# pauxy-qmc/pauxy

Hardware: AMD Instinct MI355X
Metric: walker_steps_per_sec (higher is better)
Workload: dtype f64; 1 GPU; generic Cholesky AFQMC: Nbasis=100, Nchol=500, RHF trial 25+25 electrons, 256 walkers/GPU, dt=0.005, reortho/10, comb/5, energy/10 (BASELINE configs[2]); walkers_total=256, rng=device-philox, population_control=device comb (one rank)

## Files before the change

include/afqmc_hip.h:

```cpp
#ifndef AFQMC_HIP_H
#define AFQMC_HIP_H

#include <stdint.h>

#ifdef __cplusplus
extern "C" {
#endif

typedef struct afq_handle afq_handle;

#define AFQ_OK            0
#define AFQ_EINVAL       (-1)
#define AFQ_ESTATE       (-2)
#define AFQ_EHIP         (-3)
#define AFQ_ENOMEM       (-4)
#define AFQ_EUNSUPPORTED (-5)
#define AFQ_EWEIGHT      (-6)
#define AFQ_EOVERFLOW    (-7)
#define AFQ_ECOMM        (-8)

#define AFQ_SYS_GENERIC 1
#define AFQ_SYS_HUBBARD 2
#define AFQ_SYS_UEG     3

// ... 66 lines not shown
int afq_local_energy_full_g(afq_handle *h, const double *G, int n, double *E_out);
int afq_ueg_pair_sums(afq_handle *h, const double *G, int n, double *E_out, double *two_rdm_out);
int afq_hubbard_energy_full_g(afq_handle *h, const double *G, int n, double *E_out);
int afq_correlations_full_g(afq_handle *h, const double *G, int n, double *corr_out);
int afq_set_pairing_bonds(afq_handle *h, int nb, const int32_t *nbr);
int afq_pairing_full_g(afq_handle *h, const double *G, int n, double *pair_out);

int afq_bp_configure(afq_handle *h, int nbp);
int afq_bp_steps(afq_handle *h, int32_t *steps_out);
int afq_bp_update(afq_handle *h, const double *phi_bp0, int nstblz, int restore_weights, int eval_energy,
                  int reset, double *est_out);
int afq_bp_observables(afq_handle *h, int two_rdm, int ekt, const double *h1, const double *L, int nL);
int afq_bp_pairing(afq_handle *h, int on);
int afq_bp_ekt_chunks(afq_handle *h, int nc, int ncy);
int afq_bp_update_ext(afq_handle *h, const double *phi_bp0, int nstblz, int restore_weights, int eval_energy,
                      int reset, double *est_out, double *two_rdm_out, double *fock_out);
int afq_bp_update_msd(afq_handle *h, int ndet, const double *dets, const double *coeffs, int nstblz, int restore_weights,
                      int eval_energy, int reset, double *est_out, double *detw_out);

int afq_itcf_configure(afq_handle *h, int nmax, int neqlb, int stable, int restore_weights);
int afq_itcf_update(afq_handle *h, const double *psi_T, int nstblz, double *spgf_out, double *denom_out);

int afq_set_trial_multi(afq_handle *h, int ndet, const double *psi, const double *coeffs, const double *rchol);
int afq_walkers_det_weights(afq_handle *h, double *weights_out);

int afq_set_propagator(afq_handle *h, const double *BH1, const double *mf_shift,
                       double dt, int exp_order, int flags);

int afq_walkers_alloc(afq_handle *h, int nw);
int afq_walkers_set(afq_handle *h, int field, const void *host, int first, int count);
int afq_walkers_get(afq_handle *h, int field, void *host, int first, int count);
int afq_walkers_device_ptr(afq_handle *h, int field, void **dev_ptr, int64_t *bytes_per_walker);

int afq_greens(afq_handle *h, int want_G, double *ovlp_out);
int afq_calc_overlap(afq_handle *h, double *ovlp_out);
int afq_inverse_overlap(afq_handle *h, double *oinv_out, double *ovlp_out);
int afq_propagate(afq_handle *h, const double *xi, double eshift_re, double eshift_im);
int afq_propagate_begin(afq_handle *h, const double *xi);
int afq_propagate_finish(afq_handle *h, double eshift_re, double eshift_im);
int afq_reortho(afq_handle *h, double *detR_out);
int afq_set_log_shift(afq_handle *h, int on, double log_shift, double detR_shift);
int afq_log_ovlp_sums(afq_handle *h, double *sums3);
int afq_local_energy(afq_handle *h, double *E_out);

int afq_set_exchange_algorithm(afq_handle *h, int mode);
int afq_exchange_algorithm(afq_handle *h, int *mode_out);

int afq_set_propagator_closed_form(afq_handle *h, int mode);
int afq_propagator_closed_form(afq_handle *h, int *mode_out);

int afq_set_step_fusion(afq_handle *h, int mode);
int afq_set_step_fusion_scope(afq_handle *h, int scope);
int afq_set_step_tail_overlap(afq_handle *h, int on);

int afq_set_msd_force_bias(afq_handle *h, int mode);
int afq_msd_force_bias(afq_handle *h, int *mode_out);

int afq_force_bias(afq_handle *h, double *xbar_out);
int afq_shift_fields(afq_handle *h, const double *xi, const double *xbar,
                     double *xs_out, double *cmf_out, double *cfb_out);
int afq_vhs(afq_handle *h, const double *xs, double *vhs_out);
int afq_vhs_count(afq_handle *h, int *nv);
int afq_apply_exponential(afq_handle *h, const double *vhs);
int afq_kinetic(afq_handle *h);

int afq_cap_weights(afq_handle *h, double frac, double total_weight);
int afq_set_weight_cap(afq_handle *h, double frac, double total_weight);
int afq_popcontrol_comb(afq_handle *h, double r, double target_weight,
                        int32_t *parent_ix, double *total_weight_out);
#define AFQ_PAIR_BRANCH_MAX_WALKERS 8192
int afq_popcontrol_pair_branch(afq_handle *h, const double *u, int nu, double target_weight,
                               double min_weight, double max_weight, int32_t *mult,
                               int32_t *ndraws_out, double *total_weight_out);

#define AFQ_COMM_ID_BYTES 128
#define AFQ_COMM_NSTATS 12
typedef int (*afq_allgather_fn)(const void *send, void *recv, int bytes, void *user);
int afq_comm_unique_id(void *id_out);
int afq_comm_available(void);
int afq_comm_init(afq_handle *h, const void *unique_id, int rank, int nranks);
int afq_comm_init_ipc(afq_handle *h, int rank, int nranks, afq_allgather_fn allgather, void *user);
int afq_comm_destroy(afq_handle *h);
int afq_comm_set_transport(afq_handle *h, int window);
int afq_comm_set_capacity(afq_handle *h, int max_walkers_per_peer);
int afq_comm_set_timeout(afq_handle *h, double seconds);
int afq_comm_probe(afq_handle *h, int64_t *mismatch_out);
int afq_comm_stats(afq_handle *h, int64_t *out);
int afq_comm_parent_ix(afq_handle *h, int32_t *parent_ix_global);
int afq_estimates_allreduce(afq_handle *h, double *buf, int nest);
int afq_comm_init_local(afq_handle **handles, int n);
int afq_popcontrol_comb_local(afq_handle **handles, int n, double r, double target_weight,
                              int32_t *parent_ix_global, double *total_weight_out);
int afq_estimates_allreduce_local(afq_handle **handles, int n);
int afq_walkers_scale_weights(afq_handle *h, double scale);
int afq_walkers_copy(afq_handle *h, int src, int dst);
int afq_walker_pack_bytes(afq_handle *h, int64_t *bytes);
int afq_walker_pack(afq_handle *h, int iw, void *dev_buf);
int afq_walker_unpack(afq_handle *h, int iw, const void *dev_buf);
int afq_walkers_reset_weights(afq_handle *h);
int afq_estimates_update(afq_handle *h, int eval_energy);
int afq_estimates_rdm(afq_handle *h, int on);
int afq_estimates_sf(afq_handle *h, int on);
int afq_estimates_sf_get(afq_handle *h, double *sf_out , int zero);
int afq_estimates_rdm_get(afq_handle *h, double *rdm_out , int zero);
int afq_estimates_get(afq_handle *h, double *est_out , int zero);
int afq_estimates_fuse_next(afq_handle *h);
// ... 52 lines not shown
```

pauxy_amd/_lib.py:

```python
import ctypes
import os
from ctypes import POINTER, c_char_p, c_double, c_int, c_int32, c_int64, c_uint64, c_void_p

HERE = os.path.dirname(os.path.abspath(__file__))
LIB_PATH = os.environ.get("AFQ_LIBRARY") or os.path.join(HERE, "libafqmc_hip.so")

AFQ_OK = 0
AFQ_EWEIGHT, AFQ_EOVERFLOW, AFQ_ECOMM = -6, -7, -8
AFQ_COMM_NSTATS = 12
ALLGATHER_FN = ctypes.CFUNCTYPE(ctypes.c_int, ctypes.c_void_p, ctypes.c_void_p, ctypes.c_int, ctypes.c_void_p)
AFQ_SYS_GENERIC, AFQ_SYS_HUBBARD, AFQ_SYS_UEG = 1, 2, 3
AFQ_PROP_HYBRID, AFQ_PROP_FORCE_BIAS, AFQ_PROP_FREE_PROJECTION, AFQ_PROP_HUBBARD_SPIN = 1, 2, 4, 8
(F_PHI, F_WEIGHT, F_UNSCALED_WEIGHT, F_OT, F_HYBRID_ENERGY, F_PHASE, F_DETR, F_ELOC, F_GHALF, F_G,
 F_XBAR, F_XSHIFTED, F_ENERGY, F_LOG_DETR, F_THERMAL_G, F_THERMAL_STACK, F_THERMAL_RIGHT, F_THERMAL_M0,
 F_THERMAL_DET, F_CMF, F_CFB) = range(21)
THERMAL_CHARGE, THERMAL_FREE_PROJECTION, THERMAL_LOW_RANK, THERMAL_AVERAGE_GF = 1, 2, 4, 8
THERMAL_STREAMED_GREENS = 16
AFQ_EINVAL, AFQ_ESTATE, AFQ_EUNSUPPORTED = -1, -2, -5

_h = c_void_p
_dp = c_void_p
_ip = c_void_p

SIGNATURES = {
# ... 61 lines not shown
    "afq_propagate_hirsch": [_h, c_double],
    "afq_hirsch_free_projection": [_h, c_int],
    "afq_hirsch_single_site": [_h, c_int],
    "afq_propagate_hirsch_free": [_h, _dp, c_void_p, c_double],
    "afq_hirsch_kinetic": [_h],
    "afq_hirsch_two_body": [_h, _dp, _dp, _dp],
    "afq_hirsch_finish": [_h, c_double],
    "afq_bp_configure": [_h, c_int],
    "afq_bp_steps": [_h, _dp],
    "afq_bp_update": [_h, _dp, c_int, c_int, c_int, c_int, _dp],
    "afq_bp_observables": [_h, c_int, c_int, _dp, _dp, c_int],
    "afq_bp_ekt_chunks": [_h, c_int, c_int],
    "afq_bp_update_ext": [_h, _dp, c_int, c_int, c_int, c_int, _dp, _dp, _dp],
    "afq_bp_update_msd": [_h, c_int, _dp, _dp, c_int, c_int, c_int, c_int, _dp, _dp],
    "afq_itcf_configure": [_h, c_int, c_int, c_int, c_int],
    "afq_itcf_update": [_h, _dp, c_int, _dp, _dp],
    "afq_local_energy_full_g": [_h, _dp, c_int, _dp],
    "afq_ueg_pair_sums": [_h, _dp, c_int, _dp, _dp],
    "afq_correlations_full_g": [_h, _dp, c_int, _dp],
    "afq_set_pairing_bonds": [_h, c_int, _ip],
    "afq_pairing_full_g": [_h, _dp, c_int, _dp],
    "afq_bp_pairing": [_h, c_int],
    "afq_hubbard_energy_full_g": [_h, _dp, c_int, _dp],
    "afq_set_trial_multi": [_h, c_int, _dp, _dp, _dp],
    "afq_walkers_det_weights": [_h, _dp],
    "afq_rng_normal": [_h, _dp, c_int64],
    "afq_rng_philox4x32": [_h, c_void_p, c_void_p, c_int],
    "afq_debug": [_h, c_int, c_int],
    "afq_last_launch": [_h, c_void_p, c_int, POINTER(c_uint64), POINTER(c_uint64)],
    "afq_comm_unique_id": [c_void_p],
    "afq_comm_available": [],
    "afq_comm_init": [_h, c_void_p, c_int, c_int],
    "afq_comm_init_ipc": [_h, c_int, c_int, ALLGATHER_FN, c_void_p],
    "afq_comm_set_transport": [_h, c_int],
    "afq_comm_probe": [_h, c_void_p],
    "afq_comm_destroy": [_h],
    "afq_comm_set_capacity": [_h, c_int],
    "afq_comm_set_timeout": [_h, c_double],
    "afq_launch_trace": [_h, c_int],
    "afq_launch_trace_get": [_h, c_void_p, c_int, c_void_p, c_void_p, c_int, POINTER(c_int)],
    "afq_comm_stats": [_h, c_void_p],
    "afq_comm_parent_ix": [_h, c_void_p],
    "afq_estimates_allreduce": [_h, _dp, c_int],
    "afq_comm_init_local": [POINTER(_h), c_int],
    "afq_popcontrol_comb_local": [POINTER(_h), c_int, c_double, c_double, c_void_p, POINTER(c_double)],
    "afq_estimates_allreduce_local": [POINTER(_h), c_int],
    "afq_set_exchange_algorithm": [_h, c_int],
    "afq_exchange_algorithm": [_h, POINTER(c_int)],
    "afq_set_propagator_closed_form": [_h, c_int],
    "afq_propagator_closed_form": [_h, POINTER(c_int)],
    "afq_set_step_fusion": [_h, c_int],
    "afq_set_step_fusion_scope": [_h, c_int],
    "afq_set_step_tail_overlap": [_h, c_int],
    "afq_set_msd_force_bias": [_h, c_int],
    "afq_msd_force_bias": [_h, POINTER(c_int)],
    "afq_kernel_trace": [_h, c_int],
    "afq_kernel_trace_stride": [_h, c_int, c_int],
    "afq_kernel_trace_get": [_h, c_int, _dp, c_int, POINTER(c_int)],
    "afq_kernel_issued_flops": [_h, c_int, POINTER(c_double)],
    "afq_thermal_configure": [_h, c_int, c_int, c_int, _dp, _dp, _dp, _dp, c_int],
    "afq_thermal_reset": [_h],
    "afq_thermal_propagate": [_h, _dp, c_void_p, c_double],
    "afq_thermal_greens": [_h, c_int],
    "afq_thermal_energy": [_h, _dp, _dp],
    "afq_thermal_state": [_h, c_void_p],
    "afq_thermal_configure_continuous": [_h, c_int, c_int, c_double, _dp, _dp, _dp, _dp, c_double, c_int],
    "afq_thermal_propagate_continuous": [_h, _dp, _dp],
}


class AfqLibraryError(RuntimeError):
    pass


class AfqError(RuntimeError):
    def __init__(self, code, text):
        RuntimeError.__init__(self, "libafqmc_hip error %d: %s" % (code, text))
        self.code = code


_lib = None


def load(path=None):
    global _lib
    if _lib is not None and path is None:
        return _lib
    p = path or LIB_PATH
    if not os.path.exists(p):
        raise AfqLibraryError(
            "%s not found: build it with `python -c 'import __graft_entry__ as g; g.build()'` "
            "(or `make -C pauxy_amd/csrc`).  There is no CPU fallback." % p)
    try:
        lib = ctypes.CDLL(p)
    except OSError as e:
        raise AfqLibraryError("cannot load %s: %s" % (p, e))
    for name, args in SIGNATURES.items():
        try:
            fn = getattr(lib, name)
        except AttributeError:
            raise AfqLibraryError("%s does not export %s" % (p, name))
        fn.argtypes = args
        fn.restype = c_char_p if name == "afq_last_error" else c_int
    if path is None:
        _lib = lib
    return lib
# ... 3 lines not shown
```

pauxy_amd/csrc/afq_api.hip:

```cpp
#include <algorithm>
#include <cmath>
#include <complex>
#include <cstdio>
#include <cstdlib>
#include <cstring>
#include "afq_host.h"
#include "walker_fields.h"

namespace {

void free_dets(afq_handle *h) {
    h->mem.release(LT_TRIAL);
    h->dets.assign(1, afq_handle::DetOps());
    h->ndet = 1;
    select_det(h, 0, true);
    h->msd_fb_gbar = false;
}

void free_system(afq_handle *h) {
    free_dets(h);
    h->mem.release(LT_SYSTEM);
    h->hs_cplx = 0; h->sf_nlong = 0; h->kind = 0; h->pair_nb = 0;
    h->hirsch = false;
}
// ... 29 lines not shown
    }
    int rc = dev_upload(h, LT_TRIAL, &h->dets[h->cur_det].rH1, r.data(), (size_t)nt * M);
    select_det(h, h->cur_det, true);
    return rc;
}

}

struct afq_host_cache {
    std::vector<double> H1, psi;
    std::vector<double> BH1;
};
static afq_host_cache *cache_of(afq_handle *h);

struct afq_handle_full : afq_handle {
    afq_host_cache cache;
};
static afq_host_cache *cache_of(afq_handle *h) { return &static_cast<afq_handle_full *>(h)->cache; }

static int build_psiB(afq_handle *h);

static int upload_psi(afq_handle *h, const double *psi) {
    const size_t n = (size_t)h->M * h->nt;
    afq_handle::DetOps &o = h->dets[h->cur_det];
    int rc = dev_upload(h, LT_TRIAL, &o.psi, psi, n);
    if (rc) return rc;
    cache_of(h)->psi.assign(psi, psi + 2 * n);
    h->psi_real = true;
    for (size_t i = 0; i < n && h->psi_real; ++i) h->psi_real = psi[2 * i + 1] == 0.0;
    h->psi_closed = h->na == h->nb && h->na > 0;
    for (int p_ = 0; p_ < h->M && h->psi_closed; ++p_)
        h->psi_closed = memcmp(psi + 2 * (size_t)p_ * h->nt, psi + 2 * ((size_t)p_ * h->nt + h->na), sizeof(double) * 2 * h->na) == 0;
    std::vector<double> pc(psi, psi + 2 * n);
    for (size_t i = 0; i < n; ++i) pc[2 * i + 1] = -pc[2 * i + 1];
    if (h->ndet <= 1) {
        std::vector<double> pt(2 * n);
        for (int p_ = 0; p_ < h->M; ++p_)
            for (int i = 0; i < h->nt; ++i) {
                pt[2 * ((size_t)i * h->M + p_)] = pc[2 * ((size_t)p_ * h->nt + i)];
                pt[2 * ((size_t)i * h->M + p_) + 1] = pc[2 * ((size_t)p_ * h->nt + i) + 1];
            }
        if ((rc = dev_upload(h, LT_TRIAL, &h->psicT, pt.data(), n))) return rc;
    }
    rc = dev_upload(h, LT_TRIAL, &o.psic, pc.data(), n);
    select_det(h, h->cur_det, true);
    return rc ? rc : build_psiB(h);
}

static int build_psiB(afq_handle *h) {
    afq_host_cache *c = cache_of(h);
    const int M = h->M, nt = h->nt, na = h->na;
    const bool ok = h->have_prop && h->ndet <= 1 && h->psi_stride == 0 && h->psi_real && h->psi_closed &&
                    h->bh1_real && h->bh1_same && c->psi.size() == (size_t)2 * M * nt && c->BH1.size() == (size_t)M * M;
    h->psiB_psi = nullptr; h->psiB_bh1 = nullptr;
    if (!ok) return dev_alloc(h, LT_TRIAL, &h->psiB_cT, 0);
    std::vector<double> pb((size_t)na * M, 0.0);
    for (int m = 0; m < M; ++m)
        for (int i = 0; i < na; ++i) {
            const double p = c->psi[2 * ((size_t)m * nt + i)];
            const double *brow = &c->BH1[(size_t)m * M];
            double *out = &pb[(size_t)i * M];
            for (int k = 0; k < M; ++k) out[k] += p * brow[k];
        }
    const int rc = dev_upload(h, LT_TRIAL, &h->psiB_cT, pb.data(), pb.size());
    if (!rc) { h->psiB_psi = h->dets[h->cur_det].psi; h->psiB_bh1 = h->BH1; }
    return rc;
}

static int maybe_build_rH1(afq_handle *h) {
    afq_host_cache *c = cache_of(h);
    if (h->kind == 0 || !h->have_trial || c->H1.empty()) return AFQ_OK;
    return build_rH1(h, c->H1, c->psi);
}

__global__ void afq_marker_kernel(volatile unsigned long long *retired, unsigned long long n) { *retired = n; }

void afq_launch_trace_mark(afq_handle *h, const char *name) {
    const size_t pairs = h->ltrace_name.size();
    if (name && pairs >= 65536) return;
    auto event_at = [&](size_t i) {
        while (h->ltrace_ev.size() <= i) { hipEvent_t e; hipEventCreate(&e); h->ltrace_ev.push_back(e); }
        return h->ltrace_ev[i];
    };
    if (h->ltrace_open) {
        hipEventRecord(event_at(2 * pairs - 1), h->stream);
        h->ltrace_open = false;
    }
    if (name) {
        hipEventRecord(event_at(2 * pairs), h->stream);
        h->ltrace_name.push_back(name);
        h->ltrace_open = true;
    }
}

hipError_t afq_post_launch(afq_handle *h) {
    hipError_t e = hipGetLastError();
    if (e != hipSuccess) return e;
    if (h->ltrace_open) afq_launch_trace_mark(h, nullptr);
    if (h->debug_markers) {
        unsigned long long *dptr = nullptr;
        if (hipHostGetDevicePointer((void **)&dptr, (void *)h->retired, 0) == hipSuccess)
            hipLaunchKernelGGL(afq_marker_kernel, dim3(1), dim3(1), 0, h->stream, dptr, (unsigned long long)h->n_launch);
    }
    if (h->debug_sync) e = hipStreamSynchronize(h->stream);
    return e;
}

extern "C" {

int afq_version(void) { return 2; }

int afq_create(int device_id, afq_handle **out) {
    if (!out) return AFQ_EINVAL;
    *out = nullptr;
    int ndev = 0;
    if (hipGetDeviceCount(&ndev) != hipSuccess || ndev == 0) return AFQ_EHIP;
    if (device_id < 0 || device_id >= ndev) return AFQ_EINVAL;
    if (hipSetDevice(device_id) != hipSuccess) return AFQ_EHIP;
// ... 42 lines not shown

int afq_sync(afq_handle *h) {
    if (!h) return AFQ_EINVAL;
    AFQ_HIP(h, hipStreamSynchronize(h->stream));
    return AFQ_OK;
}

int afq_stream(afq_handle *h, void **stream) {
    if (!h || !stream) return AFQ_EINVAL;
    *stream = (void *)h->stream;
    return AFQ_OK;
}

static int set_dims(afq_handle *h, int kind, int M, int K, int na, int nb) {
    if (M <= 0 || K <= 0 || na <= 0 || nb < 0 || na > M || nb > M) AFQ_FAIL(h, AFQ_EINVAL, "bad dimensions");
    hipSetDevice(h->device);
    free_system(h);
    free_walkers(h);
    h->have_trial = false; h->have_prop = false;
    h->kind = kind; h->M = M; h->K = K; h->na = na; h->nb = nb; h->nt = na + nb;
    return AFQ_OK;
}

static bool rchol_is_real(const double *rchol, size_t n) {
    for (size_t i = 0; i < n; ++i) if (rchol[2 * i + 1] != 0.0) return false;
    return true;
}

static int upload_rchol(afq_handle *h, const double *rchol, bool real) {
    const size_t nq = (size_t)h->nt * h->M;
    const int K = h->K;
    int rc;
    std::vector<double> re(nq * h->ld_rc, 0.0);
    for (size_t q = 0; q < nq; ++q)
        for (int n = 0; n < K; ++n) re[q * h->ld_rc + n] = rchol[2 * (q * K + n)];
    h->rchol_real = real;
    h->gf.rewritten();
    afq_handle::DetOps &o = h->dets[h->cur_det];
    o.rchol_same = h->na == h->nb && memcmp(rchol, rchol + 2 * (size_t)h->na * h->M * K, sizeof(double) * 2 * (size_t)h->na * h->M * K) == 0;
    h->atil_unavailable = false;
    if ((rc = dev_upload(h, LT_TRIAL, &o.rchol_re, re.data(), re.size()))) return rc;
    if (!real) {
        std::vector<double> im(nq * h->ld_rc, 0.0);
        for (size_t q = 0; q < nq; ++q)
            for (int n = 0; n < K; ++n) im[q * h->ld_rc + n] = rchol[2 * (q * K + n) + 1];
        if ((rc = dev_upload(h, LT_TRIAL, &o.rchol_im, im.data(), im.size()))) return rc;
    }
    select_det(h, h->cur_det, true);
    return k_prepare_energy_operands(h, rchol);
}

int afq_set_system_generic(afq_handle *h, int M, int K, int na, int nb, const double *hs_pot,
                           const double *rchol, const double *H1, double ecore) {
    if (h) h->gf.drop();
    if (!h || !hs_pot || !rchol || !H1) return AFQ_EINVAL;
    int rc = set_dims(h, AFQ_SYS_GENERIC, M, K, na, nb);
    if (rc) return rc;
    h->ecore = ecore;
    const size_t mm = (size_t)M * M, nq = (size_t)h->nt * M;
    {
        bool sym = true;
        for (int p = 0; p < M && sym; ++p)
            for (int q = p + 1; q < M && sym; ++q) {
                const double *a = hs_pot + ((size_t)p * M + q) * K, *b = hs_pot + ((size_t)q * M + p) * K;
                for (int n = 0; n < K; ++n) if (a[n] != b[n]) { sym = false; break; }
            }
        h->hs_sym = sym;
        if (sym) {
            const size_t np = (size_t)M * (M + 1) / 2;
            h->ld_hs = (long)((np + 1) & ~(size_t)1);
            std::vector<double> t((size_t)K * h->ld_hs, 0.0);
            std::vector<int> pq(2 * np);
            size_t c = 0;
            for (int p = 0; p < M; ++p)
                for (int q = p; q < M; ++q, ++c) {
                    pq[2 * c] = p; pq[2 * c + 1] = q;
                    const double *a = hs_pot + ((size_t)p * M + q) * K;
                    for (int n = 0; n < K; ++n) t[(size_t)n * h->ld_hs + c] = a[n];
                }
            if ((rc = dev_upload(h, LT_SYSTEM, &h->hs_pot, t.data(), t.size()))) return rc;
            if ((rc = dev_upload(h, LT_SYSTEM, &h->hs_pair, pq.data(), np))) return rc;
        } else {
            h->ld_hs = (long)((mm + 1) & ~(size_t)1);
            std::vector<double> t((size_t)K * h->ld_hs, 0.0);
            for (size_t r = 0; r < mm; ++r)
                for (int n = 0; n < K; ++n) t[(size_t)n * h->ld_hs + r] = hs_pot[r * K + n];
            if ((rc = dev_upload(h, LT_SYSTEM, &h->hs_pot, t.data(), t.size()))) return rc;
        }
    }
    h->ld_rc = (long)((K + 1) & ~1);
    if ((rc = upload_rchol(h, rchol, rchol_is_real(rchol, nq * K)))) return rc;
    if ((rc = dev_upload(h, LT_SYSTEM, &h->H1, H1, 2 * mm))) return rc;
    cache_of(h)->H1.assign(H1, H1 + 4 * mm);
    return AFQ_OK;
}

int afq_set_system_generic_c128(afq_handle *h, int M, int K, int na, int nb, const double *hs_pot,
                                const double *rchol, const double *H1, double ecore) {
    if (h) h->gf.drop();
    if (!h || !hs_pot || !rchol || !H1) return AFQ_EINVAL;
    if (M <= 0 || K <= 0) AFQ_FAIL(h, AFQ_EINVAL, "bad dimensions");
    const size_t mm = (size_t)M * M, nq = (size_t)(na + nb) * M;
    bool real = true;
    for (size_t e = 0; e < mm * K && real; ++e) real = hs_pot[2 * e + 1] == 0.0;
    if (real) {
        std::vector<double> re(mm * K);
        for (size_t e = 0; e < mm * K; ++e) re[e] = hs_pot[2 * e];
        return afq_set_system_generic(h, M, K, na, nb, re.data(), rchol, H1, ecore);
    }
    int rc = set_dims(h, AFQ_SYS_GENERIC, M, K, na, nb);
    if (rc) return rc;
    h->ecore = ecore;
    auto at = [&](int p, int q, int n, int c) { return hs_pot[2 * (((size_t)p * M + q) * K + n) + c]; };
    bool herm = true;
    for (int p = 0; p < M && herm; ++p)
        for (int q = p; q < M && herm; ++q)
            for (int n = 0; n < K; ++n)
                if (at(p, q, n, 0) != at(q, p, n, 0) || at(p, q, n, 1) != -at(q, p, n, 1)) { herm = false; break; }
    h->hs_sym = false;
    h->hs_cplx = herm ? AFQ_HS_HERMITIAN : AFQ_HS_GENERAL;
    if (herm) {
        const size_t np = (size_t)M * (M + 1) / 2, nu = (size_t)M * (M - 1) / 2;
        h->ld_hs = (long)((np + 1) & ~(size_t)1);
        h->ld_hs_im = (long)((nu + 1) & ~(size_t)1);
        std::vector<double> tr((size_t)K * h->ld_hs, 0.0), ti((size_t)K * h->ld_hs_im, 0.0);
        std::vector<int> pq(2 * np), pqi(2 * (nu ? nu : 1));
        size_t c = 0, ci = 0;
        for (int p = 0; p < M; ++p)
            for (int q = p; q < M; ++q, ++c) {
                pq[2 * c] = p; pq[2 * c + 1] = q;
                for (int n = 0; n < K; ++n) tr[(size_t)n * h->ld_hs + c] = at(p, q, n, 0);
                if (q == p) continue;
                pqi[2 * ci] = p; pqi[2 * ci + 1] = q;
                for (int n = 0; n < K; ++n) ti[(size_t)n * h->ld_hs_im + ci] = at(p, q, n, 1);
                ++ci;
            }
        if ((rc = dev_upload(h, LT_SYSTEM, &h->hs_pot, tr.data(), tr.size()))) return rc;
        if ((rc = dev_upload(h, LT_SYSTEM, &h->hs_pot_im, ti.data(), ti.size()))) return rc;
        if ((rc = dev_upload(h, LT_SYSTEM, &h->hs_pair, pq.data(), np))) return rc;
        if (nu && (rc = dev_upload(h, LT_SYSTEM, &h->hs_pair_im, pqi.data(), nu))) return rc;
    } else {
        h->ld_hs = h->ld_hs_im = (long)((mm + 1) & ~(size_t)1);
        std::vector<double> tr((size_t)K * h->ld_hs, 0.0), ti((size_t)K * h->ld_hs, 0.0);
        for (size_t r = 0; r < mm; ++r)
            for (int n = 0; n < K; ++n) {
                tr[(size_t)n * h->ld_hs + r] = hs_pot[2 * (r * K + n)];
                ti[(size_t)n * h->ld_hs + r] = hs_pot[2 * (r * K + n) + 1];
            }
        if ((rc = dev_upload(h, LT_SYSTEM, &h->hs_pot, tr.data(), tr.size()))) return rc;
        if ((rc = dev_upload(h, LT_SYSTEM, &h->hs_pot_im, ti.data(), ti.size()))) return rc;
    }
    h->ld_rc = (long)((K + 1) & ~1);
    if ((rc = upload_rchol(h, rchol, rchol_is_real(rchol, nq * K)))) return rc;
    if ((rc = dev_upload(h, LT_SYSTEM, &h->H1, H1, 2 * mm))) return rc;
    cache_of(h)->H1.assign(H1, H1 + 4 * mm);
    return AFQ_OK;
}

int afq_set_system_hubbard(afq_handle *h, int M, int na, int nb, double U, const double *T) {
    if (h) h->gf.drop();
    if (!h || !T) return AFQ_EINVAL;
    int rc = set_dims(h, AFQ_SYS_HUBBARD, M, M, na, nb);
    if (rc) return rc;
    h->U = U; h->ecore = 0.0;
    const size_t mm = (size_t)M * M;
    if ((rc = dev_upload(h, LT_SYSTEM, &h->H1, T, 2 * mm))) return rc;
    cache_of(h)->H1.assign(T, T + 4 * mm);
    return AFQ_OK;
}

static int csc_to_csr(afq_handle *h, int nrow, int ncol, const int64_t *cp, const int64_t *row, const double *val,
                      int64_t **rp_d, int64_t **col_d, cplx **val_d) {
    const int64_t nnz = cp[ncol];
    std::vector<int64_t> rp(nrow + 1, 0), col(nnz);
    std::vector<double> v(2 * nnz);
    for (int64_t z = 0; z < nnz; ++z) rp[row[z] + 1]++;
    for (int r = 0; r < nrow; ++r) rp[r + 1] += rp[r];
    std::vector<int64_t> fill(rp.begin(), rp.end() - 1);
    for (int c = 0; c < ncol; ++c)
        for (int64_t z = cp[c]; z < cp[c + 1]; ++z) {
            const int64_t d = fill[row[z]]++;
            col[d] = c; v[2 * d] = val[2 * z]; v[2 * d + 1] = val[2 * z + 1];
        }
    int rc;
    if ((rc = dev_upload(h, LT_SYSTEM, rp_d, rp.data(), rp.size()))) return rc;
    if ((rc = dev_upload(h, LT_SYSTEM, col_d, col.data(), col.size()))) return rc;
    return dev_upload(h, LT_SYSTEM, val_d, v.data(), (size_t)nnz);
}

int afq_set_system_ueg(afq_handle *h, int M, int nq, int na, int nb, const int64_t *iA_colptr,
                       const int64_t *iA_row, const double *iA_val, const int64_t *iB_colptr,
                       const int64_t *iB_row, const double *iB_val, const int64_t *kpq_off,
                       const int64_t *kpq_i, const int64_t *kpq_kpq, const int64_t *pmq_off,
                       const int64_t *pmq_i, const int64_t *pmq_pmq, const double *vqvec, double vol,
                       const double *H1diag, double ecore) {
    if (h) h->gf.drop();
    if (!h || !iA_colptr || !iB_colptr || !kpq_off || !pmq_off || !vqvec || !H1diag) return AFQ_EINVAL;
    int rc = set_dims(h, AFQ_SYS_UEG, M, 2 * nq, na, nb);
    if (rc) return rc;
    h->nq = nq; h->vol = vol; h->ecore = ecore;
    h->nnzA = iA_colptr[nq]; h->nnzB = iB_colptr[nq];
    if ((rc = dev_upload(h, LT_SYSTEM, &h->iA_colptr, iA_colptr, (size_t)nq + 1))) return rc;
    if ((rc = dev_upload(h, LT_SYSTEM, &h->iA_row, iA_row, (size_t)h->nnzA))) return rc;
    if ((rc = dev_upload(h, LT_SYSTEM, &h->iA_val, iA_val, (size_t)h->nnzA))) return rc;
    if ((rc = dev_upload(h, LT_SYSTEM, &h->iB_colptr, iB_colptr, (size_t)nq + 1))) return rc;
    if ((rc = dev_upload(h, LT_SYSTEM, &h->iB_row, iB_row, (size_t)h->nnzB))) return rc;
    if ((rc = dev_upload(h, LT_SYSTEM, &h->iB_val, iB_val, (size_t)h->nnzB))) return rc;
    if ((rc = csc_to_csr(h, M * M, nq, iA_colptr, iA_row, iA_val, &h->iA_rowptr, &h->iA_col, &h->iA_rval))) return rc;
    if ((rc = csc_to_csr(h, M * M, nq, iB_colptr, iB_row, iB_val, &h->iB_rowptr, &h->iB_col, &h->iB_rval))) return rc;
    {
        int L = 0;
        for (int q = 0; q < nq; ++q) {
            L = std::max(L, (int)(iA_colptr[q + 1] - iA_colptr[q]));
            L = std::max(L, (int)(iB_colptr[q + 1] - iB_colptr[q]));
        }
        const size_t nc = (size_t)2 * nq;
        std::vector<int> er(nc * L, 0);
        std::vector<double> ev(2 * nc * L, 0.0);
        for (int c = 0; c < 2 * nq; ++c) {
            const bool isB = c >= nq;
            const int q = isB ? c - nq : c;
            const int64_t *cp = isB ? iB_colptr : iA_colptr, *rw = isB ? iB_row : iA_row;
            const double *vl = isB ? iB_val : iA_val;
            int k = 0;
            for (int64_t z = cp[q]; z < cp[q + 1]; ++z, ++k) {
                er[(size_t)k * nc + c] = (int)rw[z];
                ev[2 * ((size_t)k * nc + c)] = vl[2 * z]; ev[2 * ((size_t)k * nc + c) + 1] = vl[2 * z + 1];
            }
        }
        h->ell_len = L;
        if ((rc = dev_upload(h, LT_SYSTEM, &h->ell_row, er.data(), nc * L))) return rc;
        if ((rc = dev_upload(h, LT_SYSTEM, &h->ell_val, ev.data(), nc * L))) return rc;
    }
    if ((rc = dev_upload(h, LT_SYSTEM, &h->kpq_off, kpq_off, (size_t)nq + 1))) return rc;
    if ((rc = dev_upload(h, LT_SYSTEM, &h->kpq_i, kpq_i, (size_t)kpq_off[nq]))) return rc;
    if ((rc = dev_upload(h, LT_SYSTEM, &h->kpq_kpq, kpq_kpq, (size_t)kpq_off[nq]))) return rc;
    if ((rc = dev_upload(h, LT_SYSTEM, &h->pmq_off, pmq_off, (size_t)nq + 1))) return rc;
    if ((rc = dev_upload(h, LT_SYSTEM, &h->pmq_i, pmq_i, (size_t)pmq_off[nq]))) return rc;
    if ((rc = dev_upload(h, LT_SYSTEM, &h->pmq_pmq, pmq_pmq, (size_t)pmq_off[nq]))) return rc;
    {
        std::vector<int> rmap(M, -1), rows;
        for (int64_t z = 0; z < kpq_off[nq]; ++z) if (rmap[kpq_i[z]] < 0) { rmap[kpq_i[z]] = 1; }
        for (int64_t z = 0; z < pmq_off[nq]; ++z) if (rmap[pmq_i[z]] < 0) { rmap[pmq_i[z]] = 1; }
        for (int i = 0; i < M; ++i) if (rmap[i] > 0) { rmap[i] = (int)rows.size(); rows.push_back(i); }
        h->ueg_nrows = (int)rows.size();
        if ((rc = dev_upload(h, LT_SYSTEM, &h->ueg_rmap, rmap.data(), (size_t)M))) return rc;
        if ((rc = dev_upload(h, LT_SYSTEM, &h->ueg_rows, rows.data(), rows.size()))) return rc;
        if (M < 65536 && kpq_off[nq] < (1LL << 31) && pmq_off[nq] < (1LL << 31)) {
            std::vector<int> kp((size_t)kpq_off[nq]), pm((size_t)pmq_off[nq]), ko((size_t)nq + 1), po((size_t)nq + 1);
            for (int64_t z = 0; z < kpq_off[nq]; ++z) kp[z] = (rmap[kpq_i[z]] << 16) | (int)kpq_kpq[z];
            for (int64_t z = 0; z < pmq_off[nq]; ++z) pm[z] = (rmap[pmq_i[z]] << 16) | (int)pmq_pmq[z];
            for (int q = 0; q <= nq; ++q) { ko[q] = (int)kpq_off[q]; po[q] = (int)pmq_off[q]; }
            if ((rc = dev_upload(h, LT_SYSTEM, &h->ueg_kp, kp.data(), kp.size() ? kp.size() : 1))) return rc;
            if ((rc = dev_upload(h, LT_SYSTEM, &h->ueg_pm, pm.data(), pm.size() ? pm.size() : 1))) return rc;
            if ((rc = dev_upload(h, LT_SYSTEM, &h->ueg_koff, ko.data(), ko.size()))) return rc;
            if ((rc = dev_upload(h, LT_SYSTEM, &h->ueg_poff, po.data(), po.size()))) return rc;
            for (int64_t z = 0; z < kpq_off[nq]; ++z) kp[z] = ((int)kpq_i[z] << 16) | (int)kpq_kpq[z];
            for (int64_t z = 0; z < pmq_off[nq]; ++z) pm[z] = ((int)pmq_i[z] << 16) | (int)pmq_pmq[z];
            std::vector<int> order((size_t)nq);
            std::vector<long> cost((size_t)nq);
            for (int q = 0; q < nq; ++q) { order[q] = q; cost[q] = (long)(ko[q + 1] - ko[q]) * (po[q + 1] - po[q]); }
            std::stable_sort(order.begin(), order.end(), [&](int a, int b) { return cost[a] > cost[b]; });
            h->sf_nlong = 0;
            while (h->sf_nlong < nq && cost[order[h->sf_nlong]] > 64) ++h->sf_nlong;
            if ((rc = dev_upload(h, LT_SYSTEM, &h->sf_kp, kp.data(), kp.size() ? kp.size() : 1))) return rc;
            if ((rc = dev_upload(h, LT_SYSTEM, &h->sf_pm, pm.data(), pm.size() ? pm.size() : 1))) return rc;
            if ((rc = dev_upload(h, LT_SYSTEM, &h->sf_order, order.data(), order.size() ? order.size() : 1))) return rc;
        }
    }
    if ((rc = dev_upload(h, LT_SYSTEM, &h->vqvec, vqvec, (size_t)nq))) return rc;
    if ((rc = dev_upload(h, LT_SYSTEM, &h->H1diag, H1diag, (size_t)2 * M))) return rc;
    cache_of(h)->H1.clear();
    return k_ueg_fast_system(h, M, nq, iA_colptr, iA_row, iA_val, iB_colptr, iB_row, iB_val);
}

int afq_set_trial(afq_handle *h, const double *psi) {
    if (h) h->gf.drop();
    if (!h || !psi) return AFQ_EINVAL;
    if (!h->kind) AFQ_FAIL(h, AFQ_ESTATE, "set the system before the trial");
    if (h->ndet > 1) AFQ_FAIL(h, AFQ_ESTATE, "a multi-determinant trial is set; set the system again first");
    hipSetDevice(h->device);
    int rc = upload_psi(h, psi);
    if (rc) return rc;
    h->have_trial = true;
    if (h->kind == AFQ_SYS_UEG && (rc = k_ueg_fast_trial(h, psi))) return rc;
    return maybe_build_rH1(h);
}

int afq_set_trial_multi(afq_handle *h, int ndet, const double *psi, const double *coeffs, const double *rchol) {
    if (h) h->gf.drop();
    if (!h || !psi || !coeffs || !rchol || ndet < 1) return AFQ_EINVAL;
    if (h->kind != AFQ_SYS_GENERIC) AFQ_FAIL(h, AFQ_EUNSUPPORTED, "multi-determinant trials need a generic system");
    if (h->nw) AFQ_FAIL(h, AFQ_ESTATE, "set the trial before allocating walkers");
    hipSetDevice(h->device);
    free_dets(h);
    const size_t npsi = (size_t)h->M * h->nt, nrc = npsi * h->K;
    const bool real = rchol_is_real(rchol, nrc * ndet);
    h->ndet = ndet;
    h->dets.assign(ndet, afq_handle::DetOps());
    int rc;
    for (int d = 0; d < ndet; ++d) {
        select_det(h, d, true);
        if ((rc = upload_psi(h, psi + 2 * npsi * d))) return rc;
        if ((rc = upload_rchol(h, rchol + 2 * nrc * d, real))) return rc;
        h->have_trial = true;
        if ((rc = maybe_build_rH1(h))) return rc;
    }
    select_det(h, 0);
    if ((rc = dev_upload(h, LT_TRIAL, &h->coeffs, coeffs, (size_t)ndet))) return rc;
    if (ndet > 1) {
        const int M = h->M, nt = h->nt;
        const size_t kkp = ((size_t)ndet * nt + 7) & ~(size_t)7;
        std::vector<double> pt(2 * kkp * M, 0.0);
        for (int d = 0; d < ndet; ++d)
            for (int p_ = 0; p_ < M; ++p_)
                for (int i = 0; i < nt; ++i) {
                    const double *src = psi + 2 * (npsi * d + (size_t)p_ * nt + i);
                    double *dst = &pt[2 * (((size_t)d * nt + i) * M + p_)];
                    dst[0] = src[0]; dst[1] = -src[1];
                }
        if ((rc = dev_upload(h, LT_TRIAL, &h->msd_psicT, pt.data(), kkp * M))) return rc;
        if (h->hs_cplx == AFQ_HS_HERMITIAN) {
            for (double &v : pt) v = -v;
            if ((rc = dev_upload(h, LT_TRIAL, &h->msd_psicT_neg, pt.data(), kkp * M))) return rc;
        }
    }
    return AFQ_OK;
}

int afq_set_propagator(afq_handle *h, const double *BH1, const double *mf_shift, double dt, int exp_order,
                       int flags) {
    if (h) h->gf.drop();
    if (!h || !BH1 || !mf_shift || dt <= 0 || exp_order < 0) return AFQ_EINVAL;
    if (!h->kind) AFQ_FAIL(h, AFQ_ESTATE, "set the system before the propagator");
    hipSetDevice(h->device);
    int rc;
    if ((rc = dev_upload(h, LT_HANDLE, &h->BH1, BH1, (size_t)2 * h->M * h->M))) return rc;
    h->bh1_real = true;
    h->bh1_same = memcmp(BH1, BH1 + (size_t)2 * h->M * h->M, sizeof(double) * 2 * h->M * h->M) == 0;
    for (size_t i = 0, n = (size_t)2 * h->M * h->M; i < n && h->bh1_real; ++i) h->bh1_real = BH1[2 * i + 1] == 0.0;
    {
        std::vector<double> &b = cache_of(h)->BH1;
        b.resize((size_t)h->M * h->M);
        for (size_t i = 0; i < b.size(); ++i) b[i] = BH1[2 * i];
    }
    if ((rc = dev_upload(h, LT_HANDLE, &h->mf_shift, mf_shift, (size_t)h->K))) return rc;
    if (h->kind == AFQ_SYS_UEG && (rc = k_ueg_fast_propagator(h, BH1))) return rc;
    h->dt = dt; h->sqrt_dt = std::pow(dt, 0.5); h->exp_order = exp_order;
    if (flags & AFQ_PROP_FREE_PROJECTION) flags &= ~AFQ_PROP_FORCE_BIAS;
    const int old_nv = h->nv; const bool old_diag = h->vhs_diag;
    h->flags = flags;
    h->vhs_diag = h->kind == AFQ_SYS_HUBBARD;
    h->nv = (h->kind == AFQ_SYS_HUBBARD && (flags & AFQ_PROP_HUBBARD_SPIN)) ? 2 : 1;
    h->have_prop = true;
    if ((rc = build_psiB(h))) return rc;
    if (h->nw && (old_nv != h->nv || old_diag != h->vhs_diag || !h->vhs)) {
        const size_t per = h->vhs_diag ? (size_t)2 * h->nv * h->M : (size_t)h->nv * h->M * h->M;
        if ((rc = dev_alloc(h, LT_WALKERS, &h->vhs, per * h->nw))) return rc;
    }
    return AFQ_OK;
}

int afq_walkers_alloc(afq_handle *h, int nw) {
    if (h) h->gf.drop();
    if (!h || nw <= 0) return AFQ_EINVAL;
    if (!h->kind) AFQ_FAIL(h, AFQ_ESTATE, "set the system before allocating walkers");
    hipSetDevice(h->device);
    free_walkers(h);
    const size_t per = (size_t)h->M * h->nt, K = h->K, n = nw;
    int rc = 0;
    auto walk = [&](auto &slot, size_t cnt) { return rc = dev_alloc(h, LT_WALKERS, &slot, cnt); };
    if (walk(h->phi, per * n) || walk(h->phi_t, per * n) || walk(h->phi_t2, per * n) ||
        walk(h->weight, n) || walk(h->unscaled, n) || walk(h->detR, n) || walk(h->log_detR, n) ||
        walk(h->ot, n) || walk(h->ehyb, n) || walk(h->phase, n) || walk(h->eloc, n) ||
        walk(h->ghalf_all, per * n * h->ndet) || walk(h->ovlp_old, n) || walk(h->ovlp_new, n)) return rc;
    if (h->ndet > 1 && (walk(h->detd, n * h->ndet) || walk(h->detd_a, n * h->ndet) || walk(h->detw, n * h->ndet) ||
                        walk(h->energy_all, 3 * n * h->ndet))) return rc;
    if (walk(h->xi, K * n) || walk(h->xbar, K * n) || walk(h->xs, K * n) || walk(h->cmf, n) || walk(h->cfb, n) ||
        walk(h->energy, 3 * n) || walk(h->alive, n) || walk(h->parent_ix, n)) return rc;
    h->fb_split = 1;
    if (h->kind == AFQ_SYS_GENERIC) {
        const long tiles = (long)((nw + 31) / 32) * ((h->K + 31) / 32) * 2;
        int sp = (int)std::max(1L, std::min(8L, 1024 / std::max(1L, tiles)));
        if (nw > 32) {
            const long wgt = (long)((nw + 63) / 64) * ((h->K + 63) / 64) * 2;
            sp = (int)std::max(1L, std::min(16L, (512 + wgt - 1) / wgt));
        }
        if (h->rchol_same && h->rchol_real && h->ndet == 1 && h->na == h->nb && nw > 32 && sp > 1) sp = (sp + 1) / 2;
        const int nmax = std::max(h->na, h->nb) * h->M;
        while (sp > 1 && nmax / sp < 64) --sp;
        h->fb_split = sp;
        if (walk(h->vbias_all, (size_t)2 * sp * n * K * h->ndet)) return rc;
    } else if (h->kind == AFQ_SYS_UEG) {
        if (walk(h->vbias_all, n * K) || walk(h->G, (size_t)2 * h->M * h->M * n)) return rc;
    }
    {
        const size_t pv = h->kind == AFQ_SYS_HUBBARD ? (size_t)4 * h->M : (size_t)h->M * h->M;
        if (walk(h->vhs, pv * n)) return rc;
    }
    if ((rc = dev_alloc(h, LT_WALKERS, (char **)&h->pack_tmp, std::max((size_t)nw * 2 * sizeof(int), (size_t)4096)))) return rc;
    h->nw = nw;
    select_det(h, h->cur_det, true);
    h->cap_frac = 0.0; h->cap_total = -1.0;
    {
        double sc0[AFQ_NSCAL] = {0};
        sc0[0] = (double)nw * k_comm_size(h);
        AFQ_HIP(h, hipMemcpy(h->scal, sc0, sizeof(sc0), hipMemcpyHostToDevice));
    }
    std::vector<double> one(nw, 1.0), zero2(2 * (size_t)nw, 0.0), one2(2 * (size_t)nw, 0.0);
    for (int i = 0; i < nw; ++i) one2[2 * i] = 1.0;
    AFQ_HIP(h, hipMemcpy(h->weight, one.data(), sizeof(double) * nw, hipMemcpyHostToDevice));
    AFQ_HIP(h, hipMemcpy(h->unscaled, one.data(), sizeof(double) * nw, hipMemcpyHostToDevice));
    AFQ_HIP(h, hipMemcpy(h->detR, one.data(), sizeof(double) * nw, hipMemcpyHostToDevice));
    AFQ_HIP(h, hipMemset(h->log_detR, 0, sizeof(double) * nw));
    AFQ_HIP(h, hipMemcpy(h->ot, one2.data(), sizeof(cplx) * nw, hipMemcpyHostToDevice));
    AFQ_HIP(h, hipMemcpy(h->phase, one2.data(), sizeof(cplx) * nw, hipMemcpyHostToDevice));
    AFQ_HIP(h, hipMemcpy(h->ehyb, zero2.data(), sizeof(cplx) * nw, hipMemcpyHostToDevice));
    AFQ_HIP(h, hipMemcpy(h->eloc, zero2.data(), sizeof(cplx) * nw, hipMemcpyHostToDevice));
    AFQ_HIP(h, hipMemset(h->phi, 0, sizeof(cplx) * per * n));
    AFQ_HIP(h, hipMemset(h->ghalf, 0, sizeof(cplx) * per * n));
    AFQ_HIP(h, hipMemset(h->energy, 0, sizeof(cplx) * 3 * n));
    AFQ_HIP(h, hipMemset(h->xi, 0, sizeof(double) * K * n));
    AFQ_HIP(h, hipMemset(h->xbar, 0, sizeof(cplx) * K * n));
    AFQ_HIP(h, hipMemset(h->xs, 0, sizeof(cplx) * K * n));
    AFQ_HIP(h, hipMemset(h->cmf, 0, sizeof(cplx) * n));
    AFQ_HIP(h, hipMemset(h->cfb, 0, sizeof(cplx) * n));
    return AFQ_OK;
}

static int field_info(afq_handle *h, int field, void **base, size_t *bytes) {
    const size_t per = (size_t)h->M * h->nt;
    switch (field) {
    case AFQ_F_PHI: *base = h->phi; *bytes = per * sizeof(cplx); break;
    case AFQ_F_WEIGHT: *base = h->weight; *bytes = sizeof(double); break;
    case AFQ_F_UNSCALED_WEIGHT: *base = h->unscaled; *bytes = sizeof(double); break;
    case AFQ_F_OT: *base = h->ot; *bytes = sizeof(cplx); break;
    case AFQ_F_HYBRID_ENERGY: *base = h->ehyb; *bytes = sizeof(cplx); break;
    case AFQ_F_PHASE: *base = h->phase; *bytes = sizeof(cplx); break;
    case AFQ_F_DETR: *base = h->detR; *bytes = sizeof(double); break;
    case AFQ_F_ELOC: *base = h->eloc; *bytes = sizeof(cplx); break;
    case AFQ_F_GHALF: *base = h->ghalf; *bytes = per * sizeof(cplx); break;
    case AFQ_F_G: *base = h->G; *bytes = (size_t)2 * h->M * h->M * sizeof(cplx); break;
    case AFQ_F_XBAR: *base = h->xbar; *bytes = (size_t)h->K * sizeof(cplx); break;
    case AFQ_F_XSHIFTED: *base = h->xs; *bytes = (size_t)h->K * sizeof(cplx); break;
    case AFQ_F_ENERGY: *base = h->energy; *bytes = 3 * sizeof(cplx); break;
    case AFQ_F_LOG_DETR: *base = h->log_detR; *bytes = sizeof(double); break;
    case AFQ_F_THERMAL_G:
        if (h->th_on && h->th_cplx) { *base = h->thc_G; *bytes = (size_t)2 * h->M * h->M * sizeof(cplx); break; }
        *base = h->th_G; *bytes = (size_t)2 * h->M * h->M * sizeof(double); break;
    case AFQ_F_THERMAL_STACK:
        if (h->th_on && h->th_cplx) { *base = h->thc_stack; *bytes = (size_t)2 * h->M * h->M * h->th_nbins * sizeof(cplx); break; }
        *base = h->th_stack; *bytes = (size_t)2 * h->M * h->M * h->th_nbins * sizeof(double); break;
    case AFQ_F_THERMAL_RIGHT: *base = h->th_on && h->th_cplx ? h->thc_right : nullptr; *bytes = (size_t)2 * h->M * h->M * sizeof(cplx); break;
    case AFQ_F_THERMAL_M0: *base = h->th_on && h->th_cplx ? h->thc_M0 : nullptr; *bytes = 2 * sizeof(cplx); break;
    case AFQ_F_THERMAL_DET: *base = h->th_on && h->th_cplx ? h->thc_det : nullptr; *bytes = 2 * sizeof(cplx); break;
    case AFQ_F_CMF: *base = h->cmf; *bytes = sizeof(cplx); break;
    case AFQ_F_CFB: *base = h->cfb; *bytes = sizeof(cplx); break;
    default: AFQ_FAIL(h, AFQ_EINVAL, "unknown walker field");
    }
    if (!*base) AFQ_FAIL(h, AFQ_ESTATE, "walker field not allocated (afq_walkers_alloc / afq_greens first)");
    return AFQ_OK;
}

static int ensure_spin_ghalf(afq_handle *h);

int afq_walkers_set(afq_handle *h, int field, const void *host, int first, int count) {
    if (h && (field == AFQ_F_PHI || field == AFQ_F_GHALF)) { h->gf.drop(); h->gf.rewritten(); }
    if (!h || !host) return AFQ_EINVAL;
    if (!h->nw) AFQ_FAIL(h, AFQ_ESTATE, "no walkers allocated");
    if (first < 0 || count < 0 || first + count > h->nw) AFQ_FAIL(h, AFQ_EINVAL, "walker range out of bounds");
    if (field == AFQ_F_THERMAL_DET || field == AFQ_F_CMF || field == AFQ_F_CFB)
        AFQ_FAIL(h, AFQ_EINVAL, "afq_walkers_set: a result of the last kernel, not walker state (get only)");
    hipSetDevice(h->device);
    void *base; size_t bytes;
    int rc = field_info(h, field, &base, &bytes);
    if (rc) return rc;
    AFQ_HIP(h, hipMemcpyAsync((char *)base + bytes * first, host, bytes * count, hipMemcpyHostToDevice, h->stream));
    AFQ_HIP(h, hipStreamSynchronize(h->stream));
    return AFQ_OK;
}

int afq_walkers_get(afq_handle *h, int field, void *host, int first, int count) {
    if (!h || !host) return AFQ_EINVAL;
    if (!h->nw) AFQ_FAIL(h, AFQ_ESTATE, "no walkers allocated");
    if (first < 0 || count < 0 || first + count > h->nw) AFQ_FAIL(h, AFQ_EINVAL, "walker range out of bounds");
    hipSetDevice(h->device);
    void *base; size_t bytes;
    int rc = field_info(h, field, &base, &bytes);
    if (rc) return rc;
    if (field == AFQ_F_GHALF && (rc = ensure_spin_ghalf(h))) return rc;
    AFQ_HIP(h, hipMemcpyAsync(host, (char *)base + bytes * first, bytes * count, hipMemcpyDeviceToHost, h->stream));
    AFQ_HIP(h, hipStreamSynchronize(h->stream));
    return AFQ_OK;
}

int afq_walkers_device_ptr(afq_handle *h, int field, void **dev_ptr, int64_t *bytes_per_walker) {
    if (!h || !dev_ptr) return AFQ_EINVAL;
    void *base; size_t bytes;
    int rc = field_info(h, field, &base, &bytes);
    if (rc) return rc;
    if (field == AFQ_F_GHALF && h->gf.kept == GreensCache::SUM_ONLY) {
        hipSetDevice(h->device);
        if ((rc = ensure_spin_ghalf(h))) return rc;
    }
    h->gf.drop(); h->gf.enabled = false;
    *dev_ptr = base;
    if (bytes_per_walker) *bytes_per_walker = (int64_t)bytes;
    return AFQ_OK;
}

static int greens_any(afq_handle *h, cplx *det_out, bool with_ghalf, GreensRequest req = GreensRequest(),
                      GreensResult *res = nullptr);

static int ensure_spin_ghalf(afq_handle *h) {
    if (h->gf.kept != GreensCache::SUM_ONLY) return AFQ_OK;
    h->gf.drop();
    const int rc = greens_any(h, h->ovlp_new, true);
    if (rc == AFQ_OK) h->gf.keep(GreensCache::FULL);
    return rc;
}

int afq_greens(afq_handle *h, int want_G, double *ovlp_out) {
    AFQ_API(h, "afq_greens");
    if (h) h->gf.drop();
    if (!h) return AFQ_EINVAL;
    int rc = need_ready(h, false);
    if (rc) return rc;
    {
        PhaseTimer t(h, T_GREENS);
        if ((rc = greens_any(h, h->ovlp_old, true))) return rc;
        if (want_G || h->kind == AFQ_SYS_UEG) {
            if ((rc = ensure_G(h))) return rc;
            if ((rc = k_full_G(h))) return rc;
        }
    }
    return copy_out(h, ovlp_out, h->ovlp_old, sizeof(cplx) * h->nw);
}

int afq_inverse_overlap(afq_handle *h, double *oinv_out, double *ovlp_out) {
    if (h) h->gf.drop();
    if (!h || !oinv_out) return AFQ_EINVAL;
    int rc = need_ready(h, false);
    if (rc) return rc;
    if (h->ndet > 1) AFQ_FAIL(h, AFQ_EUNSUPPORTED, "inverse overlaps: single-determinant trials");
    const size_t nmax = h->na > h->nb ? h->na : h->nb, n = (size_t)h->nw * 2 * nmax * nmax;
    DevTemp<cplx> tmp;
    if ((rc = dev_temp(h, tmp, n))) return rc;
    AFQ_HIP(h, hipMemsetAsync(tmp, 0, sizeof(cplx) * n, h->stream));
    if ((rc = k_alive(h))) return rc;
    std::vector<int> ones(h->nw, 1);
    AFQ_HIP(h, hipMemcpyAsync(h->alive, ones.data(), sizeof(int) * h->nw, hipMemcpyHostToDevice, h->stream));
    rc = k_inverse_overlap(h, tmp, h->ovlp_new);
    if (!rc) rc = copy_out(h, oinv_out, tmp, sizeof(cplx) * n);
    if (!rc && ovlp_out) rc = copy_out(h, ovlp_out, h->ovlp_new, sizeof(cplx) * h->nw);
    if (!rc) rc = k_alive(h);
    return rc;
}

// ... 53 lines not shown
    return in_scope && h->step_fusion_mode != 0 && h->gf.enabled && h->ndet == 1 &&
           h->kind == AFQ_SYS_GENERIC && (h->flags & AFQ_PROP_HYBRID) && (h->flags & AFQ_PROP_FORCE_BIAS) &&
           !(h->flags & AFQ_PROP_FREE_PROJECTION) && !h->rdm_on && h->nbp == 0 && h->psi_stride == 0 && !h->hirsch &&
           !k_greens_big_supported(h) && k_fb_use_sum(h) && k_step_fusion_shape(h);
}

int afq_propagate(afq_handle *h, const double *xi, double eshift_re, double eshift_im) {
    if (h) { h->step_one_call = true; h->step_eshift = cmake(eshift_re, eshift_im); }
    const int rc = afq_propagate_begin(h, xi);
    if (h) h->step_one_call = false;
    if (rc && h) h->step_tail_done = false;
    return rc ? rc : afq_propagate_finish(h, eshift_re, eshift_im);
}

int afq_propagate_begin(afq_handle *h, const double *xi) {
    AFQ_API(h, "afq_propagate");
    if (!h) return AFQ_EINVAL;
    int rc = need_ready(h, true);
    if (rc) return rc;
    if (h->hirsch) AFQ_FAIL(h, AFQ_ESTATE, "discrete Hirsch propagator set: use afq_propagate_hirsch");
    const bool hubbard_fused = h->vhs_diag;
    const bool hubbard_fused_fields = hubbard_fused && h->K == h->M;
    if (xi) {
        if ((rc = k_alive(h))) return rc;
        AFQ_HIP(h, hipMemcpyAsync(h->xi, xi, sizeof(double) * (size_t)h->nw * h->K, hipMemcpyHostToDevice, h->stream));
    } else if (k_prop_fused_supported(h) || k_ueg_fast_supported(h) || hubbard_fused_fields) {
        h->rng_inline = true;
        h->rng_inline_counter = h->rng_counter++;
    } else {
        if ((rc = k_rng_normal(h))) return rc;
    }
    const bool fp = (h->flags & AFQ_PROP_FREE_PROJECTION) != 0;
    if (!fp || (h->flags & AFQ_PROP_FORCE_BIAS)) {
        PhaseTimer t(h, T_GREENS);
        const GreensCache::Kept kept = h->gf.kept;
        const bool sum_ok = kept == GreensCache::SUM_ONLY && (h->flags & AFQ_PROP_HYBRID) && !h->rdm_on &&
                            (h->kind == AFQ_SYS_GENERIC ||
                             (h->kind == AFQ_SYS_HUBBARD && h->gdiag && h->gf.gdiag.current(h->gf)));
        if (kept == GreensCache::FULL || sum_ok) std::swap(h->ovlp_old, h->ovlp_new);
        else if ((rc = greens_any(h, h->ovlp_old, true))) return rc;
        h->gf.drop();
        const bool le = !fp && !(h->flags & AFQ_PROP_HYBRID);
        if ((h->kind == AFQ_SYS_UEG && ((h->flags & AFQ_PROP_FORCE_BIAS) || le) && !k_ueg_fast_supported(h)) ||
            (h->rdm_on && h->ndet == 1)) {
            if ((rc = ensure_G(h))) return rc;
            if ((rc = k_full_G(h))) return rc;
        }
        if (le) {
            PhaseTimer te(h, T_ENERGY);
            if (h->ndet > 1) { if ((rc = local_energy_dets(h))) return rc; }
            else if ((rc = local_energy(h))) return rc;
        }
    }
    if (k_ueg_fast_supported(h)) {
        { PhaseTimer t(h, T_EXP); if ((rc = k_ueg_step(h))) return rc; }
        h->prop_pending = true;
        return AFQ_OK;
    }
    if (hubbard_fused) {
        cplx *fac = h->vhs + (size_t)h->nw * h->nv * h->M;
        const bool fields_make_factors = hubbard_fused_fields;
        {
            PhaseTimer t(h, T_FB);
            if ((rc = force_bias(h, false))) return rc;
            if ((rc = k_xbar_fields(h, fields_make_factors ? fac : nullptr))) return rc;
        }
        if (!fields_make_factors) {
            { PhaseTimer t(h, T_VHS); if ((rc = build_vhs(h))) return rc; }
            { PhaseTimer t(h, T_EXP); if ((rc = k_exp_diag_factors(h, h->vhs, fac))) return rc; }
        }
        if (h->rng_inline) AFQ_FAIL(h, AFQ_ESTATE, "internal: the inline field draw of this step was not consumed by the field kernel");
        { PhaseTimer t(h, T_ONEBODY); if ((rc = k_onebody(h, fac))) return rc; }
        { PhaseTimer t(h, T_ONEBODY); if ((rc = k_onebody(h))) return rc; }
        h->prop_pending = true;
        return AFQ_OK;
    }
    const bool fused = k_prop_fused_supported(h);
    h->closed_large = !fused && h->kind == AFQ_SYS_GENERIC && h->nv == 1 && h->bh1_same && h->na == h->nb && h->na > 0 &&
                      h->M > 128 && h->nt > 32 && h->nw >= 64;
    struct ClosedLargeOff { afq_handle *h; ~ClosedLargeOff() { h->closed_large = false; } } closed_large_off{h};
    if (h->closed_large && (rc = k_closed_flags(h))) return rc;
    if (!fused) { PhaseTimer t(h, T_ONEBODY); if ((rc = k_onebody(h))) return rc; }
    {
        PhaseTimer t(h, T_FB);
        if ((rc = force_bias(h, false))) return rc;
        if ((rc = k_xbar_fields(h))) return rc;
    }
    h->vhs_upper = fused && h->hs_sym;
    { PhaseTimer t(h, T_VHS); rc = build_vhs(h); }
    if (rc) { h->vhs_upper = false; return rc; }
    if (fused && step_fuses(h)) {
        PhaseTimer t(h, T_EXP);
        GreensRequest req;
        req.ride_weight = h->step_one_call;
        if (h->step_one_call) req.eshift = h->step_eshift;
        req.may_skip_store = h->fuse_est_req;
        h->step_tail_res = GreensResult();
        rc = k_prop_fused_greens(h, req, &h->step_tail_res, h->step_fusion_mode == 2);
        h->vhs_upper = false;
        if (rc) return rc;
        h->step_tail_done = true;
    } else if (fused) {
        PhaseTimer t(h, T_EXP);
        rc = k_prop_fused(h);
        h->vhs_upper = false;
        if (rc) return rc;
// ... 33 lines not shown
                                 h->nbp == 0 && h->psi_stride == 0;
            if ((rc = greens_any(h, h->ovlp_new, true, req, &res))) return rc;
            h->gf.keep(res.store_skipped ? GreensCache::SUM_ONLY : GreensCache::FULL);
        } else if ((rc = greens_any(h, h->ovlp_new, false, req, &res))) return rc;
        if (h->ndet > 1 && !fp && !(h->flags & AFQ_PROP_HYBRID)) {
            if ((rc = k_msd_energy_combine(h))) return rc;
        }
        if (!res.weight_rode && (rc = k_update_weight(h, req.eshift))) return rc;
        if (h->nbp > 0 && !fp && (rc = k_bp_push(h))) return rc;
    }
    if (h->fuse_est_req) {
        h->fuse_est_req = false;
        h->est_acc_pending = true;
    }
    return AFQ_OK;
}

int afq_estimates_fuse_next(afq_handle *h) {
    if (!h) return AFQ_EINVAL;
    if (!h->nw) AFQ_FAIL(h, AFQ_ESTATE, "no walkers");
    if (h->rdm_on) AFQ_FAIL(h, AFQ_EUNSUPPORTED, "afq_estimates_fuse_next with the one-body RDM accumulation on");
    if (h->hirsch) AFQ_FAIL(h, AFQ_EUNSUPPORTED, "afq_estimates_fuse_next: continuous propagator only");
    hipSetDevice(h->device);
    if (!h->est_acc) {
        int rc = dev_alloc(h, LT_WALKERS, &h->est_acc, (size_t)6 * h->nw);
        if (rc) return rc;
        AFQ_HIP(h, hipMemsetAsync(h->est_acc, 0, sizeof(double) * 6 * h->nw, h->stream));
    }
    h->fuse_est_req = true;
    return AFQ_OK;
}

int afq_set_log_shift(afq_handle *h, int on, double log_shift, double detR_shift) {
    AFQ_API(h, "afq_set_log_shift");
    if (!h) return AFQ_EINVAL;
    if (on && h->ndet > 1) AFQ_FAIL(h, AFQ_EUNSUPPORTED, "use_log_shift: single-determinant walkers only");
    h->log_shift_on = on != 0;
    h->log_shift = on ? log_shift : 0.0;
    h->detR_shift = on ? detR_shift : 0.0;
    return AFQ_OK;
}

int afq_log_ovlp_sums(afq_handle *h, double *sums3) {
    AFQ_API(h, "afq_log_ovlp_sums");
    if (!h || !sums3) return AFQ_EINVAL;
    int rc = need_ready(h, false);
    if (rc) return rc;
    return k_log_ovlp_sums(h, sums3);
}

int afq_reortho(afq_handle *h, double *detR_out) {
    AFQ_API(h, "afq_reortho");
    if (!h) return AFQ_EINVAL;
    int rc = need_ready(h, false);
    if (rc) { h->gf.drop(); return rc; }
    const GreensCache::Kept kept = h->gf.take();
    const bool keep = kept != GreensCache::NOTHING && h->ndet == 1;
    bool scaled = false;
    { PhaseTimer t(h, T_QR); if ((rc = k_reortho(h, keep ? h->ovlp_new : nullptr, &scaled))) return rc; }
    if (keep) {
        if (!scaled && (rc = k_scale_by_inverse(h, h->ovlp_new, h->detR))) return rc;
        h->gf.keep(kept);
    }
    if (h->log_shift_on && (rc = k_log_shift_reortho(h))) return rc;
    return copy_out(h, detR_out, h->detR, sizeof(double) * h->nw);
}

static int local_energy_dets(afq_handle *h) {
    cplx *final_e = h->energy;
    int rc = AFQ_OK;
    for (int d = 0; d < h->ndet && !rc; ++d) {
        select_det(h, d);
        h->energy = h->energy_all + (size_t)d * 3 * h->nw;
        rc = k_energy_generic(h);
    }
    h->energy = final_e;
    select_det(h, 0);
    return rc;
}

static int local_energy(afq_handle *h) {
    if (h->kind == AFQ_SYS_GENERIC && h->ndet > 1) {
        int rc = local_energy_dets(h);
        if (rc) return rc;
        return k_msd_energy_combine(h);
    }
    if (h->kind == AFQ_SYS_GENERIC) return k_energy_generic(h);
    if (h->kind == AFQ_SYS_HUBBARD) return k_energy_hubbard(h);
    if (!h->G) AFQ_FAIL(h, AFQ_ESTATE, "afq_greens must run before afq_local_energy");
    return k_energy_ueg(h);
}

int afq_local_energy(afq_handle *h, double *E_out) {
    AFQ_API(h, "afq_local_energy");
    if (!h) return AFQ_EINVAL;
    int rc = need_ready(h, false);
    if (rc) return rc;
    if (!h->rH1 && h->kind != AFQ_SYS_UEG) AFQ_FAIL(h, AFQ_ESTATE, "half-rotated H1 missing (set trial)");
    if ((rc = ensure_spin_ghalf(h))) return rc;
    { PhaseTimer t(h, T_ENERGY); if ((rc = local_energy(h))) return rc; }
    return copy_out(h, E_out, h->energy, sizeof(cplx) * 3 * h->nw);
}

int afq_set_exchange_algorithm(afq_handle *h, int mode) {
    if (!h || mode < 0 || mode > 2) return AFQ_EINVAL;
    h->exx_mode = mode;
    return AFQ_OK;
}

int afq_set_propagator_closed_form(afq_handle *h, int mode) {
    if (!h || mode < 0 || mode > 2) return AFQ_EINVAL;
    h->prop_closed_mode = mode;
    return AFQ_OK;
}

int afq_set_step_fusion(afq_handle *h, int mode) {
    if (!h || mode < 0 || mode > 2) return AFQ_EINVAL;
    h->step_fusion_mode = mode;
    return AFQ_OK;
}

int afq_set_step_fusion_scope(afq_handle *h, int scope) {
    if (!h || scope < 0 || scope > 1) return AFQ_EINVAL;
    h->step_fusion_scope = scope;
    return AFQ_OK;
}

int afq_set_step_tail_overlap(afq_handle *h, int on) {
    if (!h || on < 0 || on > 1) return AFQ_EINVAL;
    h->step_tail_overlap = on;
    return AFQ_OK;
}

int afq_propagator_closed_form(afq_handle *h, int *mode) {
    if (!h || !mode) return AFQ_EINVAL;
    *mode = k_prop_closed_resident(h) ? 2 : 1;
    return AFQ_OK;
}

int afq_set_msd_force_bias(afq_handle *h, int mode) {
    if (!h || mode < 0 || mode > 2) return AFQ_EINVAL;
    h->msd_fb_mode = mode;
    return AFQ_OK;
}

int afq_msd_force_bias(afq_handle *h, int *mode) {
    if (!h || !mode) return AFQ_EINVAL;
    if (h->kind != AFQ_SYS_GENERIC || !h->have_trial || !h->nw) AFQ_FAIL(h, AFQ_ESTATE, "generic system, trial and walkers must be set");
    *mode = h->ndet <= 1 ? 0 : k_msd_gbar_wanted(h) ? 2 : 1;
    return AFQ_OK;
}

int afq_exchange_algorithm(afq_handle *h, int *mode) {
    if (!h || !mode) return AFQ_EINVAL;
    if (h->kind != AFQ_SYS_GENERIC || !h->have_trial) AFQ_FAIL(h, AFQ_ESTATE, "generic system and trial must be set");
    *mode = k_exchange_uses_quadratic(h) ? 2 : 1;
    return AFQ_OK;
}

int afq_force_bias(afq_handle *h, double *xbar_out) {
    if (!h) return AFQ_EINVAL;
    int rc = need_ready(h, true);
    if (rc) return rc;
    if ((rc = force_bias(h))) return rc;
    return copy_out(h, xbar_out, h->xbar, sizeof(cplx) * (size_t)h->nw * h->K);
}

int afq_shift_fields(afq_handle *h, const double *xi, const double *xbar, double *xs_out, double *cmf_out,
                     double *cfb_out) {
    if (!h || !xi || !xbar) return AFQ_EINVAL;
    int rc = need_ready(h, true);
    if (rc) return rc;
    const size_t n = (size_t)h->nw * h->K;
    AFQ_HIP(h, hipMemcpyAsync(h->xi, xi, sizeof(double) * n, hipMemcpyHostToDevice, h->stream));
    AFQ_HIP(h, hipMemcpyAsync(h->xbar, xbar, sizeof(cplx) * n, hipMemcpyHostToDevice, h->stream));
    if ((rc = k_fields_explicit(h, h->xi, h->xbar, h->xs, h->cmf, h->cfb))) return rc;
    if ((rc = copy_out(h, xs_out, h->xs, sizeof(cplx) * n))) return rc;
    if ((rc = copy_out(h, cmf_out, h->cmf, sizeof(cplx) * h->nw))) return rc;
    return copy_out(h, cfb_out, h->cfb, sizeof(cplx) * h->nw);
}

int afq_vhs_count(afq_handle *h, int *nv) {
    if (!h || !nv) return AFQ_EINVAL;
    *nv = h->nv;
    return AFQ_OK;
}

int afq_vhs(afq_handle *h, const double *xs, double *vhs_out) {
    if (!h || !xs || !vhs_out) return AFQ_EINVAL;
    int rc = need_ready(h, true);
    if (rc) return rc;
    const size_t n = (size_t)h->nw * h->K;
    AFQ_HIP(h, hipMemcpyAsync(h->xs, xs, sizeof(cplx) * n, hipMemcpyHostToDevice, h->stream));
    if ((rc = build_vhs(h))) return rc;
    const size_t mm = (size_t)h->M * h->M;
    if (!h->vhs_diag) return copy_out(h, vhs_out, h->vhs, sizeof(cplx) * mm * h->nv * h->nw);
    std::vector<double> d((size_t)2 * h->nw * h->nv * h->M);
    if ((rc = copy_out(h, d.data(), h->vhs, sizeof(cplx) * (size_t)h->nw * h->nv * h->M))) return rc;
    std::memset(vhs_out, 0, sizeof(cplx) * mm * h->nv * h->nw);
    for (size_t b = 0; b < (size_t)h->nw * h->nv; ++b)
        for (int p = 0; p < h->M; ++p) {
            vhs_out[2 * (b * mm + (size_t)p * h->M + p)] = d[2 * (b * h->M + p)];
            vhs_out[2 * (b * mm + (size_t)p * h->M + p) + 1] = d[2 * (b * h->M + p) + 1];
        }
    return AFQ_OK;
}

int afq_apply_exponential(afq_handle *h, const double *vhs) {
    if (h) h->gf.drop();
    if (!h || !vhs) return AFQ_EINVAL;
    int rc = need_ready(h, true);
    if (rc) return rc;
    if ((rc = k_alive(h))) return rc;
    const size_t mm = (size_t)h->M * h->M;
    if (!h->vhs_diag) {
        AFQ_HIP(h, hipMemcpyAsync(h->vhs, vhs, sizeof(cplx) * mm * h->nv * h->nw, hipMemcpyHostToDevice, h->stream));
    } else {
        std::vector<double> d((size_t)2 * h->nw * h->nv * h->M);
        for (size_t b = 0; b < (size_t)h->nw * h->nv; ++b)
            for (int p = 0; p < h->M; ++p) {
                d[2 * (b * h->M + p)] = vhs[2 * (b * mm + (size_t)p * h->M + p)];
                d[2 * (b * h->M + p) + 1] = vhs[2 * (b * mm + (size_t)p * h->M + p) + 1];
            }
        AFQ_HIP(h, hipMemcpy(h->vhs, d.data(), sizeof(double) * d.size(), hipMemcpyHostToDevice));
    }
    if ((rc = apply_exp(h, h->vhs))) return rc;
    return afq_sync(h);
}

int afq_kinetic(afq_handle *h) {
    if (h) h->gf.drop();
    if (!h) return AFQ_EINVAL;
    int rc = need_ready(h, true);
    if (rc) return rc;
    if ((rc = k_alive(h))) return rc;
    if ((rc = k_onebody(h))) return rc;
    return afq_sync(h);
}

int afq_set_weight_cap(afq_handle *h, double frac, double total_weight) {
    if (!h) return AFQ_EINVAL;
    h->cap_frac = frac > 0.0 ? frac : 0.0;
    h->cap_total = total_weight;
    return AFQ_OK;
}

int afq_cap_weights(afq_handle *h, double frac, double total_weight) {
    if (!h) return AFQ_EINVAL;
    if (h->th_on && h->nw) { hipSetDevice(h->device); return k_cap_weights(h, frac, total_weight); }
    int rc = need_ready(h, false);
    if (rc) return rc;
    return k_cap_weights(h, frac, total_weight);
}

int afq_popcontrol_comb(afq_handle *h, double r, double target_weight, int32_t *parent_ix,
                        double *total_weight_out) {
    if (h) h->scal_cache_valid = false;
    AFQ_API(h, "afq_popcontrol_comb");
    if (!h) return AFQ_EINVAL;
    const bool thermal = h->th_on && h->nw;
    int rc = AFQ_OK;
    if (thermal) {
        h->gf.drop();
        hipSetDevice(h->device);
        if (k_comm_size(h) > 1) AFQ_FAIL(h, AFQ_EUNSUPPORTED, "thermal walkers: one rank only");
    } else if ((rc = need_ready(h, false))) { h->gf.drop(); return rc; }
    const int nranks = k_comm_size(h);
    if (h->nw * nranks == 1) return AFQ_OK;
    const bool keep = h->gf.take() == GreensCache::FULL && h->ndet == 1;
    if ((rc = k_comb(h, r, target_weight, keep))) return rc;
    if (keep) h->gf.keep(GreensCache::FULL);
    if (!parent_ix && !total_weight_out) return AFQ_OK;
    double sc[8];
    if ((rc = copy_out(h, sc, h->scal, sizeof(sc)))) return rc;
    if (total_weight_out) *total_weight_out = sc[0];
    if (sc[1] < 0) AFQ_FAIL(h, AFQ_EWEIGHT, "total walker weight below 1e-8");
    if (sc[3] != 0.0) AFQ_FAIL(h, AFQ_EOVERFLOW, "more walkers moved between two ranks than the exchange slots hold");
    if (sc[6] != 0.0) AFQ_FAIL(h, AFQ_ECOMM, "communicator: a peer rank never signalled (the wait budget of afq_comm_set_timeout ran out on the device)");
    if (!parent_ix) return AFQ_OK;
    if (h->comm) return afq_comm_parent_ix(h, parent_ix);
    return copy_out(h, parent_ix, h->parent_ix, sizeof(int) * h->nw);
}

int afq_popcontrol_pair_branch(afq_handle *h, const double *u, int nu, double target_weight, double min_weight,
                               double max_weight, int32_t *mult, int32_t *ndraws_out, double *total_weight_out) {
    if (h) h->scal_cache_valid = false;
    AFQ_API(h, "afq_popcontrol_pair_branch");
    if (!h) return AFQ_EINVAL;
    if (h->th_on) AFQ_FAIL(h, AFQ_EUNSUPPORTED, "thermal walkers: pair_branch population control is not supported (comb only)");
    int rc = need_ready(h, false);
    if (rc) { h->gf.drop(); return rc; }
    if (k_comm_size(h) > 1) {
        h->gf.drop();
        AFQ_FAIL(h, AFQ_EUNSUPPORTED, "pair branching over the library-owned communicator: it does the comb only");
    }
    if (h->nw == 1) return AFQ_OK;
    if (!u || nu < h->nw / 2 || !(target_weight > 0.0)) {
        h->gf.drop();
        AFQ_FAIL(h, AFQ_EINVAL, "afq_popcontrol_pair_branch: nw / 2 uniforms and a positive target weight are needed");
    }
    if ((rc = dev_grow(h, LT_WALKERS, &h->pb_u, &h->pb_u_n, (size_t)(h->nw / 2), "pair-branch uniforms"))) { h->gf.drop(); return rc; }
    AFQ_HIP(h, hipMemcpyAsync(h->pb_u, u, sizeof(double) * (size_t)(h->nw / 2), hipMemcpyHostToDevice, h->stream));
    const bool keep = h->gf.take() == GreensCache::FULL && h->ndet == 1;
    if ((rc = k_pair_branch(h, h->pb_u, target_weight, min_weight, max_weight, keep))) return rc;
    if (keep) h->gf.keep(GreensCache::FULL);
    if (!mult && !ndraws_out && !total_weight_out) return AFQ_OK;
    double sc[AFQ_NSCAL];
    if ((rc = copy_out(h, sc, h->scal, sizeof(sc)))) return rc;
    if (total_weight_out) *total_weight_out = sc[0];
    if (sc[1] < 0) AFQ_FAIL(h, AFQ_EWEIGHT, "total walker weight below 1e-8");
    if (ndraws_out) *ndraws_out = (int32_t)sc[9];
    if (!mult) return AFQ_OK;
    return copy_out(h, mult, h->parent_ix, sizeof(int) * h->nw);
}

int afq_walkers_scale_weights(afq_handle *h, double scale) {
    if (!h || scale == 0.0) return AFQ_EINVAL;
    int rc = need_ready(h, false);
    if (rc) return rc;
    return k_scale_weights(h, scale);
}

int afq_walkers_reset_weights(afq_handle *h) {
    if (!h) return AFQ_EINVAL;
    int rc = need_ready(h, false);
    if (rc) return rc;
    return k_reset_weights(h);
}

int afq_walker_pack_bytes(afq_handle *h, int64_t *bytes) {
    if (!h || !bytes) return AFQ_EINVAL;
    *bytes = (int64_t)walker_fields(h, WF_WEIGHT).packed_bytes();
    return AFQ_OK;
}

static int pack_io(afq_handle *h, int iw, char *buf, bool pack) {
    const WalkerFields f = walker_fields(h, WF_WEIGHT);
    long off = 0;
    for (int k = 0; k < f.n; ++k) {
        const WalkerFields::Entry &e = f.e[k];
        off = WalkerFields::packed_at(off, e.bytes);
        if (pack) AFQ_HIP(h, hipMemcpyAsync(buf + off, e.base + iw * e.bytes, e.bytes, hipMemcpyDeviceToDevice, h->stream));
        else AFQ_HIP(h, hipMemcpyAsync(e.base + iw * e.bytes, buf + off, e.bytes, hipMemcpyDeviceToDevice, h->stream));
        off += e.bytes;
    }
    return AFQ_OK;
}

int afq_walker_pack(afq_handle *h, int iw, void *dev_buf) {
    if (!h || !dev_buf) return AFQ_EINVAL;
    int rc = need_ready(h, false);
    if (rc) return rc;
    if (iw < 0 || iw >= h->nw) AFQ_FAIL(h, AFQ_EINVAL, "walker index out of range");
    return pack_io(h, iw, (char *)dev_buf, true);
}

int afq_walker_unpack(afq_handle *h, int iw, const void *dev_buf) {
    if (h) h->gf.drop();
    if (!h || !dev_buf) return AFQ_EINVAL;
    int rc = need_ready(h, false);
    if (rc) return rc;
    if (iw < 0 || iw >= h->nw) AFQ_FAIL(h, AFQ_EINVAL, "walker index out of range");
    return pack_io(h, iw, (char *)dev_buf, false);
}

int afq_walkers_copy(afq_handle *h, int src, int dst) {
    if (h) h->gf.drop();
    if (!h) return AFQ_EINVAL;
    int rc = need_ready(h, false);
    if (rc) return rc;
    if (src < 0 || dst < 0 || src >= h->nw || dst >= h->nw) AFQ_FAIL(h, AFQ_EINVAL, "walker index out of range");
    if (src == dst) return AFQ_OK;
    const WalkerFields f = walker_fields(h, WF_WEIGHT);
    for (int k = 0; k < f.n; ++k)
        AFQ_HIP(h, hipMemcpyAsync(f.e[k].base + dst * f.e[k].bytes, f.e[k].base + src * f.e[k].bytes, f.e[k].bytes, hipMemcpyDeviceToDevice, h->stream));
    return AFQ_OK;
}

static int est_publish_args(afq_handle *h, int zero, EstPublish *pub);

static int estimates_update_impl(afq_handle *h, int eval_energy, int publish_zero) {
    int rc = need_ready(h, false);
    if (rc) return rc;
    if (publish_zero >= 0 && h->est_pending) AFQ_FAIL(h, AFQ_ESTATE, "afq_estimates_update_publish: a fetch is already in flight");
    if (eval_energy) {
        {
            PhaseTimer t(h, T_GREENS);
            if (h->gf.kept != GreensCache::FULL) {
                if ((rc = greens_any(h, h->ovlp_new, true))) return rc;
                if (h->gf.enabled && !(h->flags & AFQ_PROP_FREE_PROJECTION) && h->psi_stride == 0) h->gf.keep(GreensCache::FULL);
            }
            if (h->kind == AFQ_SYS_UEG || h->rdm_on) {
                if ((rc = ensure_G(h))) return rc;
                if ((rc = k_full_G(h))) return rc;
            }
        }
        PhaseTimer t(h, T_ENERGY);
        if ((rc = local_energy(h))) return rc;
    }
    if (publish_zero >= 0) {
        EstPublish pub;
        if ((rc = est_publish_args(h, publish_zero, &pub))) return rc;
        if ((rc = k_estimates(h, eval_energy, false, &pub))) return rc;
        h->est_pending = true;
    } else if ((rc = k_estimates(h, eval_energy))) return rc;
    if (eval_energy && h->sf_on) {
        if (h->flags & AFQ_PROP_FREE_PROJECTION) AFQ_FAIL(h, AFQ_EUNSUPPORTED, "mixed structure factor: importance sampling only");
        cplx *two = nullptr, *E = nullptr;
        if ((rc = k_ueg_sf_two(h, h->nw, &two, &E))) return rc;
        if ((rc = k_ueg_pair_sums(h, h->G, h->nw, E, two))) return rc;
        if ((rc = k_ueg_sf_wsum(h, two, h->nw, nullptr, h->weight, nullptr, h->sf_acc))) return rc;
    }
    if (h->rdm_on && !(h->flags & AFQ_PROP_FREE_PROJECTION)) {
        if (!h->G) AFQ_FAIL(h, AFQ_ESTATE, "one_rdm: no Green's function evaluated yet");
        return k_rdm_accumulate(h);
    }
    return AFQ_OK;
}

int afq_estimates_update(afq_handle *h, int eval_energy) {
// ... 197 lines not shown
    txt += " last:";
    for (unsigned long long i = n > 8 ? n - 8 : 0; i < n; ++i)
        txt += std::string(" ") + (h->crumb_name[i & 63] ? h->crumb_name[i & 63] : "?");
    snprintf(buf, (size_t)len, "%s", txt.c_str());
    return AFQ_OK;
}

int afq_counters_ext(afq_handle *h, int64_t *out, int n, int reset) {
    if (!h || !out || n < 0) return AFQ_EINVAL;
    hipSetDevice(h->device);
    unsigned long long c[AFQ_NCOUNTERS];
    int rc = copy_out(h, c, h->counters, sizeof(c));
    if (rc) return rc;
    for (int i = 0; i < n; ++i) out[i] = i < AFQ_NCOUNTERS ? (int64_t)c[i] : 0;
    if (reset) AFQ_HIP(h, hipMemsetAsync(h->counters, 0, sizeof(c), h->stream));
    return AFQ_OK;
}

int afq_counters(afq_handle *h, int64_t *out, int reset) { return afq_counters_ext(h, out, 4, reset); }

int afq_enable_timers(afq_handle *h, int on) {
    if (!h) return AFQ_EINVAL;
    h->timers_on = on != 0;
    return AFQ_OK;
}

int afq_timers(afq_handle *h, double *out_ms, int reset) {
    if (!h || !out_ms) return AFQ_EINVAL;
    for (int i = 0; i < T_COUNT; ++i) { out_ms[i] = h->t_ms[i]; if (reset) h->t_ms[i] = 0.0; }
    return AFQ_OK;
}

static int hirsch_buffers(afq_handle *h) {
    if (h->hs_oinv) return AFQ_OK;
    const size_t n = h->nw, nmax = h->na > h->nb ? h->na : h->nb;
    int rc;
    if ((rc = dev_alloc(h, LT_WALKERS, &h->hs_oinv, n * 2 * nmax * nmax))) return rc;
    if ((rc = dev_alloc(h, LT_WALKERS, &h->hs_u, n * h->M))) return rc;
    if ((rc = dev_alloc(h, LT_WALKERS, &h->hs_fields, n * h->M))) return rc;
    if ((rc = dev_alloc(h, LT_WALKERS, &h->hs_used, n))) return rc;
    if ((rc = dev_alloc(h, LT_WALKERS, &h->hs_alive0, n))) return rc;
    AFQ_HIP(h, hipMemsetAsync(h->hs_alive0, 0, sizeof(int) * n, h->stream));
    return AFQ_OK;
}

static int hirsch_ready(afq_handle *h) {
    int rc = need_ready(h, true);
    if (rc) return rc;
    if (!h->hirsch) AFQ_FAIL(h, AFQ_ESTATE, "the discrete Hirsch propagator is not set");
    return hirsch_buffers(h);
}

int afq_set_propagator_hirsch(afq_handle *h, const double *bt2, double dt, int charge_decomposition) {
    if (h) h->gf.drop();
    if (!h || !bt2 || dt <= 0) return AFQ_EINVAL;
    if (h->kind != AFQ_SYS_HUBBARD) AFQ_FAIL(h, AFQ_ESTATE, "the Hirsch transformation needs a Hubbard system");
    if (h->ndet > 1) AFQ_FAIL(h, AFQ_EUNSUPPORTED, "Hirsch propagator: single-determinant trials");
    hipSetDevice(h->device);
    int rc;
    if ((rc = dev_upload(h, LT_HANDLE, &h->BH1, bt2, (size_t)2 * h->M * h->M))) return rc;
    h->bh1_real = true;
    for (size_t i = 0, n = (size_t)2 * h->M * h->M; i < n && h->bh1_real; ++i) h->bh1_real = bt2[2 * i + 1] == 0.0;
    h->bh1_same = false;
    cache_of(h)->BH1.clear();
    if ((rc = build_psiB(h))) return rc;
    typedef std::complex<double> C;
    C gamma, auxf[2][2], wfac[2];
    const double e = std::exp(-0.5 * dt * h->U);
    if (charge_decomposition) {
        gamma = std::acosh(C(e, 0.0));
        auxf[0][0] = auxf[0][1] = std::exp(gamma);
        auxf[1][0] = auxf[1][1] = std::exp(-gamma);
        wfac[0] = std::exp(0.5 * dt * h->U) * std::exp(-gamma);
        wfac[1] = std::exp(0.5 * dt * h->U) * std::exp(gamma);
    } else {
        gamma = C(std::acosh(std::exp(0.5 * dt * h->U)), 0.0);
        auxf[0][0] = std::exp(gamma); auxf[0][1] = std::exp(-gamma);
        auxf[1][0] = std::exp(-gamma); auxf[1][1] = std::exp(gamma);
        wfac[0] = wfac[1] = C(1.0, 0.0);
    }
    for (int x = 0; x < 2; ++x) {
        h->hs_wfac[x] = cmake(wfac[x].real(), wfac[x].imag());
        for (int sp = 0; sp < 2; ++sp) {
            const C f = auxf[x][sp] * e, d = f - 1.0;
            h->hs_auxf[x][sp] = cmake(f.real(), f.imag());
            h->hs_delta[x][sp] = cmake(d.real(), d.imag());
        }
    }
    h->hs_gamma = cmake(gamma.real(), gamma.imag());
    h->hs_charge = charge_decomposition != 0;
    h->hs_direct = false;
    if (!h->mf_shift) {
        std::vector<double> z(2 * (size_t)h->K, 0.0);
        if ((rc = dev_upload(h, LT_HANDLE, &h->mf_shift, z.data(), (size_t)h->K))) return rc;
    }
    h->dt = dt; h->sqrt_dt = std::sqrt(dt);
    h->flags = 0; h->nv = 1; h->vhs_diag = true;
    h->hirsch = true; h->have_prop = true;
    return AFQ_OK;
}

int afq_hirsch_kinetic(afq_handle *h) {
    if (h) h->gf.drop();
    if (!h) return AFQ_EINVAL;
    int rc = hirsch_ready(h);
    if (rc) return rc;
    if ((rc = k_hirsch_alive(h, 0))) return rc;
    return k_hirsch_kinetic(h);
}

int afq_hirsch_two_body(afq_handle *h, const double *u, int32_t *fields_out, int32_t *used_out) {
    if (h) h->gf.drop();
    if (!h || !u) return AFQ_EINVAL;
    int rc = hirsch_ready(h);
    if (rc) return rc;
    AFQ_HIP(h, hipMemcpyAsync(h->hs_u, u, sizeof(double) * (size_t)h->nw * h->M, hipMemcpyHostToDevice, h->stream));
    if ((rc = k_hirsch_alive(h, 1))) return rc;
    if ((rc = k_hirsch_two_body(h))) return rc;
    if (fields_out && (rc = copy_out(h, fields_out, h->hs_fields, sizeof(int) * (size_t)h->nw * h->M))) return rc;
    if (used_out && (rc = copy_out(h, used_out, h->hs_used, sizeof(int) * (size_t)h->nw))) return rc;
    return AFQ_OK;
}

int afq_hirsch_finish(afq_handle *h, double eshift) {
    if (h) h->gf.drop();
    if (!h) return AFQ_EINVAL;
    int rc = hirsch_ready(h);
    if (rc) return rc;
    if ((rc = k_hirsch_alive(h, 1))) return rc;
    if ((rc = k_hirsch_kinetic(h))) return rc;
    if ((rc = k_hirsch_eshift(h, std::exp(h->dt * eshift)))) return rc;
    return k_alive(h);
}

int afq_propagate_hirsch(afq_handle *h, double eshift) {
    AFQ_API(h, "afq_propagate_hirsch");
    if (h) h->gf.drop();
    if (!h) return AFQ_EINVAL;
    int rc = hirsch_ready(h);
    if (rc) return rc;
    if ((rc = k_hirsch_alive(h, 0))) return rc;
    if ((rc = k_hirsch_kinetic(h))) return rc;
    if ((rc = k_rng_uniform(h, h->hs_u, (long)h->nw * h->M))) return rc;
    if ((rc = k_hirsch_alive(h, 1))) return rc;
    if ((rc = k_hirsch_two_body(h))) return rc;
    if ((rc = k_hirsch_alive(h, 1))) return rc;
    if ((rc = k_hirsch_kinetic(h))) return rc;
    if ((rc = k_hirsch_eshift(h, std::exp(h->dt * eshift)))) return rc;
    return k_alive(h);
}

int afq_hirsch_single_site(afq_handle *h, int on) {
    if (!h) return AFQ_EINVAL;
    if (!h->hirsch) AFQ_FAIL(h, AFQ_ESTATE, "afq_set_propagator_hirsch first");
    if (!on && h->nbp > 0) AFQ_FAIL(h, AFQ_EUNSUPPORTED, "the direct Hirsch update records no field history (hubbard.py:222-275)");
    h->hs_direct = !on;
    return AFQ_OK;
}

int afq_hirsch_free_projection(afq_handle *h, int on) {
    if (!h) return AFQ_EINVAL;
    if (!h->hirsch) AFQ_FAIL(h, AFQ_ESTATE, "afq_set_propagator_hirsch first");
    if (on && h->nbp > 0) AFQ_FAIL(h, AFQ_EUNSUPPORTED, "no field history in free projection");
    if (on) h->flags |= AFQ_PROP_FREE_PROJECTION; else h->flags &= ~AFQ_PROP_FREE_PROJECTION;
    return AFQ_OK;
}

int afq_propagate_hirsch_free(afq_handle *h, const double *u, int32_t *fields_out, double eshift) {
    AFQ_API(h, "afq_propagate_hirsch_free");
    if (h) h->gf.drop();
    if (!h) return AFQ_EINVAL;
    int rc = hirsch_ready(h);
    if (rc) return rc;
    if (!(h->flags & AFQ_PROP_FREE_PROJECTION)) AFQ_FAIL(h, AFQ_ESTATE, "afq_hirsch_free_projection(h, 1) first");
    if ((rc = k_hirsch_alive(h, 0))) return rc;
    if (u) AFQ_HIP(h, hipMemcpyAsync(h->hs_u, u, sizeof(double) * (size_t)h->nw * h->M, hipMemcpyHostToDevice, h->stream));
    else if ((rc = k_rng_uniform(h, h->hs_u, (long)h->nw * h->M))) return rc;
    if ((rc = k_hirsch_free(h, eshift))) return rc;
    if (fields_out && (rc = copy_out(h, fields_out, h->hs_fields, sizeof(int) * (size_t)h->nw * h->M))) return rc;
    return k_alive(h);
}

int afq_walkers_det_weights(afq_handle *h, double *weights_out) {
    if (!h || !weights_out) return AFQ_EINVAL;
    if (!h->nw) AFQ_FAIL(h, AFQ_ESTATE, "no walkers allocated");
    hipSetDevice(h->device);
    if (h->ndet <= 1) AFQ_FAIL(h, AFQ_ESTATE, "single-determinant trial: the overlap is the only weight");
    return copy_out(h, weights_out, h->detw, sizeof(cplx) * (size_t)h->nw * h->ndet);
}

int afq_kernel_trace(afq_handle *h, int on) {
    if (!h) return AFQ_EINVAL;
    h->ktrace_mask = on == 1 ? ~0u : on > 1 ? (unsigned)on >> 1 : 0u;
    if (on) for (int k = 0; k < AFQ_K_COUNT; ++k) { h->ktrace_used[k] = 0; h->ktrace_seen[k] = 0; }
    return AFQ_OK;
}

int afq_kernel_trace_stride(afq_handle *h, int kind, int stride) {
    if (!h || stride < 1 || kind < 0 || kind >= AFQ_K_COUNT) return AFQ_EINVAL;
    h->ktrace_stride[kind] = stride;
    return AFQ_OK;
}

int afq_kernel_trace_get(afq_handle *h, int kind, double *ms_out, int max_n, int *n_out) {
    if (!h || !n_out || kind < 0 || kind >= AFQ_K_COUNT || (max_n > 0 && !ms_out)) return AFQ_EINVAL;
    hipSetDevice(h->device);
    AFQ_HIP(h, hipStreamSynchronize(h->stream));
    const int n = h->ktrace_used[kind] < max_n ? h->ktrace_used[kind] : max_n;
    for (int i = 0; i < n; ++i) {
        float f = 0;
        AFQ_HIP(h, hipEventElapsedTime(&f, h->ktrace_ev[kind][2 * i], h->ktrace_ev[kind][2 * i + 1]));
        ms_out[i] = f;
    }
    *n_out = h->ktrace_used[kind];
    return AFQ_OK;
}

int afq_launch_trace(afq_handle *h, int on) {
    if (!h) return AFQ_EINVAL;
    hipSetDevice(h->device);
    if (h->ltrace_open) afq_launch_trace_mark(h, nullptr);
    if (on) h->ltrace_name.clear();
    h->ltrace_on = on != 0;
// ... 46 lines not shown
```

pauxy_amd/csrc/afq_internal.h:

```cpp
#pragma once
#include <hip/hip_runtime.h>
#include <stdint.h>
#include <cstdlib>
#include <string>
#include <vector>
#include "../../include/afqmc_hip.h"
#include "greens_cache.h"
#include "dev_mem.h"

typedef double2 cplx;

__host__ __device__ inline cplx cmake(double r, double i) { return make_double2(r, i); }
__host__ __device__ inline cplx cadd(cplx a, cplx b) { return cmake(a.x + b.x, a.y + b.y); }
__host__ __device__ inline cplx csub(cplx a, cplx b) { return cmake(a.x - b.x, a.y - b.y); }
__host__ __device__ inline cplx cmul(cplx a, cplx b) {
    return cmake(a.x * b.x - a.y * b.y, a.x * b.y + a.y * b.x);
}
__host__ __device__ inline cplx cconj(cplx a) { return cmake(a.x, -a.y); }
__host__ __device__ inline cplx cscale(cplx a, double s) { return cmake(a.x * s, a.y * s); }
__host__ __device__ inline void cfma(cplx &a, cplx b, cplx c) {
    a.x = fma(b.x, c.x, a.x); a.x = fma(-b.y, c.y, a.x);
    a.y = fma(b.x, c.y, a.y); a.y = fma(b.y, c.x, a.y);
}
__host__ __device__ inline double cabs2(cplx a) { return a.x * a.x + a.y * a.y; }
__device__ inline cplx cdiv(cplx a, cplx b) {
    if (fabs(b.x) >= fabs(b.y)) {
        double r = b.y / b.x, d = b.x + b.y * r;
        return cmake((a.x + a.y * r) / d, (a.y - a.x * r) / d);
    } else {
        double r = b.x / b.y, d = b.x * r + b.y;
        return cmake((a.x * r + a.y) / d, (a.y * r - a.x) / d);
    }
}

#define AFQ_NSCAL 12
enum { AFQ_HS_HERMITIAN = 1, AFQ_HS_GENERAL = 2 };
enum { T_GREENS = 0, T_ONEBODY, T_FB, T_VHS, T_EXP, T_OVLP, T_QR, T_ENERGY, T_COUNT };

#define AFQ_NCOUNTERS 9

struct afq_handle {
    int device = 0;
    hipStream_t stream = nullptr;
    std::string err;
    DevMem mem;

    int kind = 0;
    int M = 0, K = 0, na = 0, nb = 0, nt = 0;
    double ecore = 0.0;
    double *hs_pot = nullptr;
    bool hs_sym = false;
    double *L_full = nullptr;
    int2 *hs_pair = nullptr;
    int hs_cplx = 0;
    double *hs_pot_im = nullptr;
    int2 *hs_pair_im = nullptr;
    long ld_hs_im = 0;
    cplx *L_full_c = nullptr;
    long ld_hs = 0, ld_rc = 0;
    bool rchol_real = true;
    double *rchol_re = nullptr;
    double *rchol_im = nullptr;
    double *rchol_frag[2] = {nullptr, nullptr};
    double *rchol_frag_im[2] = {nullptr, nullptr};
    void *atil[2] = {nullptr, nullptr};
    bool atil_unavailable = false;
    bool rchol_same = false;
    int exx_mode = 0;
    int step_fusion_mode = 2;
    int step_fusion_scope = 0;
    int step_tail_overlap = 1;
    int prop_closed_mode = 0;
    cplx *exq_y = nullptr;
    size_t exq_y_len = 0;
    cplx *H1 = nullptr;
    cplx *rH1 = nullptr;
    double U = 0.0;
    int nq = 0;
    int64_t nnzA = 0, nnzB = 0;
    int64_t *iA_colptr = nullptr, *iA_row = nullptr; cplx *iA_val = nullptr;
    int64_t *iB_colptr = nullptr, *iB_row = nullptr; cplx *iB_val = nullptr;
    int64_t *iA_rowptr = nullptr, *iA_col = nullptr; cplx *iA_rval = nullptr;
    int64_t *iB_rowptr = nullptr, *iB_col = nullptr; cplx *iB_rval = nullptr;
    int ell_len = 0; int *ell_row = nullptr; cplx *ell_val = nullptr;
    int ueg_nrows = 0; int *ueg_rmap = nullptr; int *ueg_rows = nullptr;
    int *ueg_kp = nullptr, *ueg_pm = nullptr, *ueg_koff = nullptr, *ueg_poff = nullptr;
    int64_t *kpq_off = nullptr, *kpq_i = nullptr, *kpq_kpq = nullptr;
    int64_t *pmq_off = nullptr, *pmq_i = nullptr, *pmq_pmq = nullptr;
    double *vqvec = nullptr; double vol = 1.0; double *H1diag = nullptr;
    void *ueg_fast = nullptr;
    int *sf_kp = nullptr, *sf_pm = nullptr, *sf_order = nullptr;
    int sf_nlong = 0;
    cplx *sf_ws = nullptr, *sf_two = nullptr;
    size_t sf_ws_len = 0, sf_two_len = 0;
    cplx *corr_ws = nullptr;
    size_t corr_ws_len = 0;
    int *pair_nbr = nullptr;
    int pair_nb = 0;
    cplx *pair_ws = nullptr;
    size_t pair_ws_len = 0;

    bool have_trial = false;
    cplx *psi = nullptr;
    cplx *psic = nullptr;
    cplx *psicT = nullptr;
    long psi_stride = 0;
    bool psi_real = false;
    bool psi_closed = false;
    double *psiB_cT = nullptr;
    const void *psiB_psi = nullptr, *psiB_bh1 = nullptr;
    unsigned long long *closed_bad = nullptr;
    unsigned long long closed_epoch = 0;
    unsigned long long closed_epoch_pub = 0;
    bool exx_open_hint = false;
    int *closed_w = nullptr;
    size_t closed_w_n = 0;
    bool closed_large = false;

    struct DetOps {
        cplx *psi = nullptr, *psic = nullptr, *rH1 = nullptr;
        double *rchol_re = nullptr, *rchol_im = nullptr;
        double *rchol_frag[2] = {nullptr, nullptr}, *rchol_frag_im[2] = {nullptr, nullptr};
        void *atil[2] = {nullptr, nullptr};
        bool rchol_same = false;
        GreensCache::Stamp vbias_stamp;
    };
    int ndet = 1, cur_det = 0;
    std::vector<DetOps> dets = std::vector<DetOps>(1);
    cplx *coeffs = nullptr;
    cplx *detd = nullptr;
    cplx *detd_a = nullptr;
    cplx *detw = nullptr;
    cplx *ghalf_all = nullptr;
    cplx *vbias_all = nullptr;
    cplx *energy_all = nullptr;
    int msd_fb_mode = 0;
    bool msd_fb_gbar = false;
    cplx *msd_psicT = nullptr;
    cplx *msd_gs = nullptr;
    cplx *msd_S = nullptr;
    double *hs_pk = nullptr;
    cplx *msd_psicT_neg = nullptr;
    cplx *msd_D = nullptr;
    double *hs_pk_im = nullptr;

    int nbp = 0;
    cplx *bp_hist = nullptr;
    int *bp_n = nullptr;
    int *bp_flag = nullptr;
    double *bp_cos = nullptr;
    cplx *bp_ph = nullptr;
    cplx *phi_old = nullptr;
    cplx *phi_bp = nullptr;
    cplx *BH1dag = nullptr;
    cplx *bp_xs = nullptr;
    cplx *bp_est = nullptr;
    cplx *bp_ot = nullptr;
    double *bp_detR = nullptr;
    cplx *bpm_ws = nullptr;
    size_t bpm_ws_len = 0;
    int bpo_two = 0, bpo_ekt = 0;
    int bpo_sf = 0;
    int bpo_corr = 0;
// ... 34 lines not shown
    double *th_G0 = nullptr;
    double *th_stack = nullptr;
    double *th_u = nullptr;
    int *th_fields = nullptr;
    double *th_nav = nullptr;
    bool th_cplx = false;
    cplx *thc_G = nullptr;
    cplx *thc_G0 = nullptr;
    cplx *thc_stack = nullptr;
    cplx *thc_right = nullptr;
    cplx *thc_M0 = nullptr;
    cplx *thc_M00 = nullptr;
    cplx *thc_det = nullptr;
    cplx *thc_mf = nullptr;
    double thc_fb_bound = 1.0;
    double *thc_BTpow = nullptr;
    double *thc_left = nullptr;
    double *thc_bh1 = nullptr;
    bool thc_streamed = false;
    cplx *thc_tscratch = nullptr;

    bool have_prop = false;
    cplx *BH1 = nullptr;
    double cap_frac = 0.0, cap_total = -1.0;
    bool vhs_upper = false;
    bool bh1_same = false;
    bool bh1_real = false;
    cplx *mf_shift = nullptr;
    double dt = 0.0, sqrt_dt = 0.0;
    int exp_order = 6;
    int flags = AFQ_PROP_HYBRID | AFQ_PROP_FORCE_BIAS;
    int nv = 1;
    bool vhs_diag = false;

    int nw = 0;
    cplx *phi = nullptr;
    cplx *phi_t = nullptr;
    cplx *phi_t2 = nullptr;
    double *weight = nullptr, *unscaled = nullptr, *detR = nullptr;
    double *log_detR = nullptr;
    bool log_shift_on = false;
    double log_shift = 0.0, detR_shift = 0.0;
    cplx *ot = nullptr, *ehyb = nullptr, *phase = nullptr, *eloc = nullptr;
    cplx *ghalf = nullptr;
    cplx *G = nullptr;
    cplx *ovlp_old = nullptr, *ovlp_new = nullptr;
    double *xi = nullptr;
    int fb_split = 1;
    cplx *vbias = nullptr;
    cplx *ghalf_sum = nullptr;
    cplx *gdiag = nullptr;
    int gdiag_parts = 0;
    GreensCache gf;
    cplx *xbar = nullptr, *xs = nullptr;
    cplx *cmf = nullptr, *cfb = nullptr;
    cplx *vhs = nullptr;
    cplx *lu_ws = nullptr;
    cplx *big_ws = nullptr;
    cplx *big_ws2 = nullptr;
    cplx *detm = nullptr;
    int *dete = nullptr;
    double *qr_logd = nullptr;
    int *qr_fail = nullptr;
    cplx *energy = nullptr;
    cplx *exx_part = nullptr;
    size_t exx_part_len = 0;
    double *gfrag = nullptr;
    size_t gfrag_len = 0;
    bool prop_pending = false;
    bool step_one_call = false, step_tail_done = false;
    cplx step_eshift = {0.0, 0.0};
    GreensResult step_tail_res;
    double *est_stage = nullptr;
    unsigned long long est_seq = 0;
    double scal_cache[AFQ_NSCAL] = {0};
    bool scal_cache_valid = false;
    bool est_pending = false;
    unsigned ktrace_mask = 0;
    std::vector<hipEvent_t> ktrace_ev[AFQ_K_COUNT];
    double issued_flops[AFQ_K_COUNT] = {0, 0, 0, 0, 0};
    double prop_issued_open = 0.0, prop_issued_closed = 0.0;
    int ktrace_used[AFQ_K_COUNT] = {0, 0, 0, 0, 0};
    int ktrace_stride[AFQ_K_COUNT] = {1, 1, 1, 1, 1}, ktrace_seen[AFQ_K_COUNT] = {0, 0, 0, 0, 0};
    bool ltrace_on = false, ltrace_open = false;
    std::vector<hipEvent_t> ltrace_ev;
    std::vector<const char *> ltrace_name;
    int *gj_flag = nullptr;
    cplx *estimates = nullptr;
    bool rdm_on = false;
    double *rdm_acc = nullptr;
    bool sf_on = false;
    double *sf_acc = nullptr;
    unsigned long long *counters = nullptr;
    int *alive = nullptr;
    int *parent_ix = nullptr;
    double *scal = nullptr;
    void *pack_tmp = nullptr;
    double *pb_u = nullptr;
    size_t pb_u_n = 0;
    void *zero_page = nullptr;
    double *est_acc = nullptr;
    bool fuse_est_req = false, est_acc_pending = false;

    uint64_t rng_seed = 0, rng_stream = 0, rng_counter = 0;
    bool rng_inline = false;
    uint64_t rng_inline_counter = 0;
// ... 283 lines not shown
```

pauxy_amd/csrc/afq_windows.hip:

```cpp
#include <algorithm>
#include <optional>
#include "afq_host.h"

namespace {

struct Carver {
    cplx *base;
    size_t off = 0;
    template <class T = cplx> T *take(size_t n) {
        T *p = base ? reinterpret_cast<T *>(base + off) : nullptr;
        off += (n * sizeof(T) + sizeof(cplx) - 1) / sizeof(cplx);
        return p;
    }
};

struct BpMsdWs {
    cplx *dets, *coeffs, *ot, *ovlp, *detw, *S, *fac, *ghalf, *G, *gsum, *E, *esum, *stack;
    double *logr, *detR;
    size_t len;
};

BpMsdWs bp_msd_carve(afq_handle *h, cplx *base) {
    const size_t n = h->nw, nd = h->ndet, per = (size_t)h->M * h->nt, g2 = (size_t)2 * h->M * h->M * n;
    Carver c{base};
// ... 73 lines not shown
    return k_full_G(h);
}

int bp_backward(afq_handle *h, int nd, int nstblz, cplx *stack, cplx *ot, double *detR, double *logr, cplx *keep, int nkeep) {
    const size_t n = h->nw, per = (size_t)h->M * h->nt, slab = n * per;
    Lent<cplx *> l_phi(h->phi, h->phi_bp), l_xs(h->xs, h->bp_xs), l_BH1(h->BH1, h->BH1dag), l_ot(h->ot, ot);
    Lent<double *> l_detR(h->detR, detR);
    Lent<int> l_flags(h->flags, h->flags & ~AFQ_PROP_FREE_PROJECTION);
    const bool fused = k_prop_fused_supported(h);
    cplx *A = h->phi_bp, *B = stack, *C = h->phi_bp + nd * slab;
    int rc;
    for (int i = 0; i < h->nbp; ++i) {
        if (h->hirsch) {
            if ((rc = k_bp_hirsch_step(h, i))) return rc;
        } else {
            if ((rc = k_bp_fields(h, i))) return rc;
            {
                Lent<bool> l_upper(h->vhs_upper, fused && h->hs_sym);
                if ((rc = build_vhs(h))) return rc;
                for (int d = 0; fused && d < nd; ++d) {
                    Lent<cplx *> l_slab(h->phi, A + d * slab);
                    if ((rc = k_prop_fused(h))) return rc;
                }
            }
            if (!fused && nd == 1) {
                if ((rc = k_onebody(h))) return rc;
                if ((rc = apply_exp(h, h->vhs))) return rc;
                if ((rc = k_onebody(h))) return rc;
            } else if (!fused) {
                if ((rc = k_bp_msd_onebody(h, nd, A, B))) return rc;
                if ((rc = k_bp_msd_taylor(h, nd, h->vhs, B, C, A))) return rc;
                if ((rc = k_bp_msd_onebody(h, nd, B, A))) return rc;
            }
        }
        if (i != 0 && i % nstblz == 0) {
            for (int d = 0; d < nd; ++d)
                if ((rc = reortho_foreign(h, A + d * slab, ot, detR + d * n))) return rc;
            if (logr && (rc = k_bp_msd_logr(h, detR, logr, (long)(nd * n)))) return rc;
        }
        const int t = h->nbp - 1 - i;
        if (keep && t < nkeep)
            AFQ_HIP(h, hipMemcpyAsync(keep + (size_t)t * slab, h->phi_bp, sizeof(cplx) * slab, hipMemcpyDeviceToDevice, h->stream));
    }
    return AFQ_OK;
}

size_t bpo_two_len(const afq_handle *h) {
    const size_t m2 = (size_t)h->M * h->M;
    return h->bpo_sf ? (size_t)4 * h->nq : h->bpo_corr ? 5 * m2 : h->bpo_pair ? (size_t)h->pair_nb * h->pair_nb * m2 : m2 * m2;
}

int bp_update(afq_handle *h, const double *phi_bp0, int nstblz, int restore_weights, int eval_energy,
              int reset, double *est_out, double *two_rdm_out, double *fock_out) {
    if (h) h->gf.drop();
    if (!h || !phi_bp0 || !est_out || nstblz < 1 || restore_weights < 0 || restore_weights > 2) return AFQ_EINVAL;
    int rc = need_ready(h, true);
    if (rc) return rc;
    if (!h->nbp) AFQ_FAIL(h, AFQ_ESTATE, "back-propagation is not configured");
    if (h->hirsch && restore_weights)
        AFQ_FAIL(h, AFQ_EUNSUPPORTED, "restore_weights with discrete fields: FieldConfig.push records no weight factors (walkers/stack.py:35-49)");
    const size_t per = (size_t)h->M * h->nt, n = h->nw;
    if ((rc = window_begin(h, phi_bp0))) return rc;
    if ((rc = bp_backward(h, 1, nstblz, nullptr, h->bp_ot, h->bp_detR, nullptr, nullptr, 0))) return rc;
    cplx *conj_bp = h->phi_bp + per * n;
    if ((rc = k_conj_copy(h, h->phi_bp, conj_bp, (long)(per * n)))) return rc;
    if ((rc = ensure_G(h))) return rc;
    if ((rc = greens_with_trial(h, h->phi_old, h->phi_bp, conj_bp, h->ovlp_old, h->ghalf, h->G, false))) return rc;
    AFQ_HIP(h, hipMemsetAsync(h->bp_est, 0, sizeof(cplx) * ((size_t)4 + 2 * h->M * h->M), h->stream));
    if (eval_energy) {
        if (h->kind == AFQ_SYS_GENERIC) { if ((rc = k_energy_full_g(h, h->G, h->nw, h->energy))) return rc; }
        else if (h->kind == AFQ_SYS_HUBBARD) { if ((rc = k_energy_hubbard_full_g(h, h->G, h->nw, h->energy))) return rc; }
    }
    const bool sf = two_rdm_out && h->bpo_sf;
    cplx *sf_two = nullptr, *sf_E = nullptr;
    if (h->kind == AFQ_SYS_UEG && (eval_energy || sf)) {
        if ((rc = k_ueg_sf_two(h, h->nw, &sf_two, &sf_E))) return rc;
        if ((rc = k_ueg_pair_sums(h, h->G, h->nw, eval_energy ? h->energy : sf_E, sf_two))) return rc;
    }
    if ((rc = k_bp_accumulate(h, restore_weights, eval_energy))) return rc;
    const bool corr = two_rdm_out && h->bpo_corr, pair = two_rdm_out && h->bpo_pair;
    const size_t m2 = (size_t)h->M * h->M, m4 = bpo_two_len(h);
    if (two_rdm_out || fock_out) {
        if ((rc = k_bp_observables(h, restore_weights, two_rdm_out && !sf && !corr && !pair ? h->bpo_out : nullptr,
                                   fock_out ? h->bpo_out + (h->bpo_two ? m4 : 0) : nullptr))) return rc;
        if (sf && (rc = k_ueg_sf_wsum(h, sf_two, h->nw, h->bpo_wt, nullptr, h->bpo_out, nullptr))) return rc;
        if (corr && (rc = k_corr_wsum(h, h->G, h->nw, h->bpo_wt, h->bpo_out))) return rc;
        if (pair && (rc = k_pair_wsum(h, h->G, h->nw, h->bpo_wt, h->bpo_out))) return rc;
    }
    if ((rc = window_end(h, reset != 0))) return rc;
    if (two_rdm_out && (rc = copy_out(h, two_rdm_out, h->bpo_out, sizeof(cplx) * m4))) return rc;
    if (fock_out && (rc = copy_out(h, fock_out, h->bpo_out + (h->bpo_two ? m4 : 0), sizeof(cplx) * 2 * m2))) return rc;
    return copy_out(h, est_out, h->bp_est, sizeof(cplx) * ((size_t)4 + 2 * h->M * h->M));
}

int itcf_greens(afq_handle *h, const ItcfWs &w, cplx *psiR, cplx *psiL) {
    int rc;
    if ((rc = k_conj_copy(h, psiL, w.psiLc, (long)h->M * h->nt * h->nw))) return rc;
    if ((rc = greens_with_trial(h, psiR, psiL, w.psiLc, w.ovlp, w.ghalf, w.G, true))) return rc;
    return k_itcf_projectors(h, w.G, w.P, w.Q);
}

template <class F> int full_g_call(afq_handle *h, const double *G, int n, double *E_out, size_t tsz, double *T_out, F launch) {
    hipSetDevice(h->device);
    DevTemp<cplx> Gd, Ed, Td;
    int rc = dev_temp(h, Gd, (size_t)2 * h->M * h->M * n, G);
    if (!rc) rc = dev_temp(h, Ed, (size_t)3 * n);
    if (!rc) rc = dev_temp(h, Td, tsz);
// ... 36 lines not shown
    }
    if ((rc = dev_alloc(h, LT_WALKERS, &h->bp_hist, n * nbp * h->K))) return rc;
    if ((rc = dev_alloc(h, LT_WALKERS, &h->bp_n, n))) return rc;
    if ((rc = dev_alloc(h, LT_WALKERS, &h->bp_flag, n))) return rc;
    if ((rc = dev_alloc(h, LT_WALKERS, &h->bp_cos, n))) return rc;
    if ((rc = dev_alloc(h, LT_WALKERS, &h->bp_ph, n))) return rc;
    if ((rc = dev_alloc(h, LT_WALKERS, &h->phi_old, per * n))) return rc;
    if ((rc = dev_alloc(h, LT_WALKERS, &h->phi_bp, 2 * per * n * nd))) return rc;
    if ((rc = dev_alloc(h, LT_WALKERS, &h->bp_ot, n))) return rc;
    if ((rc = dev_alloc(h, LT_WALKERS, &h->bp_detR, n))) return rc;
    if (nd > 1) {
        if ((rc = dev_alloc(h, LT_WALKERS, &h->bpm_ws, msd_ws, "multi-determinant window", &h->bpm_ws_len))) return rc;
        h->bpm_ws_len = msd_ws;
    }
    if ((rc = dev_alloc(h, LT_WALKERS, &h->BH1dag, (size_t)2 * h->M * h->M))) return rc;
    if ((rc = dev_alloc(h, LT_WALKERS, &h->bp_xs, n * h->K))) return rc;
    if ((rc = dev_alloc(h, LT_WALKERS, &h->bp_est, (size_t)4 + 2 * h->M * h->M))) return rc;
    h->nbp = nbp;
    AFQ_HIP(h, hipMemsetAsync(h->bp_hist, 0, sizeof(cplx) * n * nbp * h->K, h->stream));
    AFQ_HIP(h, hipMemsetAsync(h->bp_flag, 0, sizeof(int) * n, h->stream));
    if ((rc = k_bp_reset(h, true))) return rc;
    if ((rc = k_conj_transpose(h, h->BH1, h->BH1dag))) return rc;
    AFQ_HIP(h, hipMemcpyAsync(h->phi_old, h->phi, sizeof(cplx) * per * n, hipMemcpyDeviceToDevice, h->stream));
    return AFQ_OK;
}

int afq_bp_steps(afq_handle *h, int32_t *steps_out) {
    if (!h || !steps_out) return AFQ_EINVAL;
    if (!h->nbp) AFQ_FAIL(h, AFQ_ESTATE, "back-propagation is not configured");
    hipSetDevice(h->device);
    int rc = copy_out(h, steps_out, h->bp_n, sizeof(int) * h->nw);
    if (!rc && h->hirsch) for (int i = 0; i < h->nw; ++i) steps_out[i] /= h->M;
    return rc;
}

int afq_bp_update(afq_handle *h, const double *phi_bp0, int nstblz, int restore_weights, int eval_energy,
                  int reset, double *est_out) {
    AFQ_API(h, "afq_bp_update");
    return bp_update(h, phi_bp0, nstblz, restore_weights, eval_energy, reset, est_out, nullptr, nullptr);
}

int afq_bp_update_ext(afq_handle *h, const double *phi_bp0, int nstblz, int restore_weights, int eval_energy,
                      int reset, double *est_out, double *two_rdm_out, double *fock_out) {
    AFQ_API(h, "afq_bp_update_ext");
    if (h && two_rdm_out && !h->bpo_two) AFQ_FAIL(h, AFQ_ESTATE, "two-body RDM: afq_bp_observables(h, 1, 2 or 3, ...) or afq_bp_pairing(h, 1) first");
    if (h && fock_out && !h->bpo_ekt) AFQ_FAIL(h, AFQ_ESTATE, "EKT Fock matrices: afq_bp_observables(h, ., 1, ...) first");
    return bp_update(h, phi_bp0, nstblz, restore_weights, eval_energy, reset, est_out, two_rdm_out, fock_out);
}

int afq_bp_update_msd(afq_handle *h, int ndet, const double *dets, const double *coeffs, int nstblz, int restore_weights,
                      int eval_energy, int reset, double *est_out, double *detw_out) {
    AFQ_API(h, "afq_bp_update_msd");
    GreensCache::ReadOnly read_only(h ? &h->gf : nullptr);
    if (!h || !dets || !coeffs || !est_out || ndet < 1 || nstblz < 1 || restore_weights < 0 || restore_weights > 2)
        return AFQ_EINVAL;
    int rc = need_ready(h, true);
    if (rc) return rc;
    if (!h->nbp) AFQ_FAIL(h, AFQ_ESTATE, "back-propagation is not configured");
    if (h->ndet <= 1 || !h->bpm_ws)
        AFQ_FAIL(h, AFQ_ESTATE, "afq_bp_update_msd: the handle holds a single-determinant trial (afq_bp_update)");
    if (ndet != h->ndet)
        AFQ_FAIL(h, AFQ_EINVAL, "afq_bp_update_msd: " + std::to_string(ndet) + " determinants, the history was configured for " +
                                    std::to_string(h->ndet));
    const size_t per = (size_t)h->M * h->nt, n = h->nw, nd = ndet, slab = n * per, gsz = (size_t)2 * h->M * h->M;
    const BpMsdWs ws = bp_msd_carve(h, h->bpm_ws);
    AFQ_HIP(h, hipMemcpyAsync(ws.dets, dets, sizeof(cplx) * nd * per, hipMemcpyHostToDevice, h->stream));
    AFQ_HIP(h, hipMemcpyAsync(ws.coeffs, coeffs, sizeof(cplx) * nd, hipMemcpyHostToDevice, h->stream));
    AFQ_HIP(h, hipMemsetAsync(ws.logr, 0, sizeof(double) * nd * n, h->stream));
    for (size_t d = 0; d < nd; ++d) {
        Lent<cplx *> l_slab(h->phi_bp, h->phi_bp + d * slab);
        if ((rc = k_bp_init(h, ws.dets + d * per))) return rc;
    }
    if ((rc = bp_backward(h, ndet, nstblz, ws.stack, ws.ot, ws.detR, ws.logr, nullptr, 0))) return rc;
    cplx *conj_bp = h->phi_bp + nd * slab;
    if ((rc = k_conj_copy(h, h->phi_bp, conj_bp, (long)(nd * slab)))) return rc;
    if (eval_energy && h->kind != AFQ_SYS_GENERIC) AFQ_FAIL(h, AFQ_EUNSUPPORTED, "back-propagated energies: generic systems only");
    for (size_t d = 0; d < nd; ++d) {
        if ((rc = greens_with_trial(h, h->phi_old, h->phi_bp + d * slab, conj_bp + d * slab, ws.ovlp + d * n, ws.ghalf, ws.G, true)))
            return rc;
        if (eval_energy && (rc = k_energy_full_g(h, ws.G, h->nw, ws.E))) return rc;
        if ((rc = k_bp_msd_detw(h, ndet, (int)d, ws.coeffs, ws.logr, ws.ovlp, ws.detw, ws.S))) return rc;
        if ((rc = k_bp_msd_gsum(h, ndet, (int)d, ws.detw, ws.G, ws.gsum, eval_energy ? ws.E : nullptr, ws.esum))) return rc;
    }
    AFQ_HIP(h, hipMemsetAsync(h->bp_est, 0, sizeof(cplx) * (4 + gsz), h->stream));
    if ((rc = k_bp_msd_finish(h, ndet, restore_weights, ws.detw, ws.S, ws.fac))) return rc;
    if ((rc = k_bp_msd_accumulate(h, ws.gsum, ws.fac, eval_energy ? ws.esum : nullptr, h->bp_est))) return rc;
    if ((rc = window_end(h, reset != 0))) return rc;
    read_only.succeeded();
    if ((rc = copy_out(h, detw_out, ws.detw, sizeof(cplx) * n * nd))) return rc;
    return copy_out(h, est_out, h->bp_est, sizeof(cplx) * (4 + gsz));
}

int afq_bp_ekt_chunks(afq_handle *h, int nc, int ncy) {
    if (!h || nc < 0 || ncy < 0) return AFQ_EINVAL;
    h->bpo_nc = nc; h->bpo_ncy = ncy;
    return AFQ_OK;
}

#define AFQ_BPO_MEM_SHARE 0.5

int afq_bp_observables(afq_handle *h, int two_rdm, int ekt, const double *h1, const double *L, int nL) {
    if (!h || (ekt && (!h1 || nL < 1 || (L == nullptr && nL != h->K)))) return AFQ_EINVAL;
    int rc = need_ready(h, true);
    if (rc) return rc;
    if (h->ndet > 1 && (two_rdm || ekt))
        AFQ_FAIL(h, AFQ_EUNSUPPORTED, "back-propagated two-body RDM / EKT with a multi-determinant trial (sum_d w_d f[G_d] of quartic / cubic forms)");
// ... 47 lines not shown
        int rc = dev_alloc(h, LT_WALKERS, &h->bpo_out, h->bpo_ekt ? 2 * M * M : 0);
        if (rc) return rc;
    }
    h->pair_nb = 0;
    int rc = dev_upload(h, LT_SYSTEM, &h->pair_nbr, nbr, nb * M);
    if (rc) return rc;
    h->pair_nb = nb;
    return AFQ_OK;
}

int afq_bp_pairing(afq_handle *h, int on) {
    if (!h) return AFQ_EINVAL;
    int rc = need_ready(h, true);
    if (rc) return rc;
    if (h->ndet > 1 && on)
        AFQ_FAIL(h, AFQ_EUNSUPPORTED, "back-propagated pairing correlations with a multi-determinant trial (sum_d w_d f[G_d] of a quadratic form)");
    if (!h->nbp) AFQ_FAIL(h, AFQ_ESTATE, "back-propagation is not configured: afq_bp_configure first");
    if (on && !h->pair_nb) AFQ_FAIL(h, AFQ_ESTATE, "pairing correlations: no bond table (afq_set_pairing_bonds first)");
    if (!on && !h->bpo_pair) return AFQ_OK;
    const size_t m2 = (size_t)h->M * h->M, m4 = on ? (size_t)h->pair_nb * h->pair_nb * m2 : 0;
    hipSetDevice(h->device);
    AFQ_HIP(h, hipStreamSynchronize(h->stream));
    h->bpo_two = h->bpo_sf = h->bpo_corr = h->bpo_pair = 0;
    if ((rc = dev_alloc(h, LT_WALKERS, &h->bpo_out, m4 + (h->bpo_ekt ? 2 * m2 : 0), "pairing correlations"))) {
        h->bpo_ekt = 0;
        return rc;
    }
    h->bpo_two = h->bpo_pair = on ? 1 : 0;
    return AFQ_OK;
}

int afq_itcf_configure(afq_handle *h, int nmax, int neqlb, int stable, int restore_weights) {
    if (!h || nmax < 1 || neqlb < 0) return AFQ_EINVAL;
    if (h->th_on) AFQ_FAIL(h, AFQ_EUNSUPPORTED, "thermal walkers: no ITCF window");
    int rc = need_ready(h, true);
    if (rc) return rc;
    if (h->M > 128) AFQ_FAIL(h, AFQ_EUNSUPPORTED, "ITCF: M > 128 (the batched Gauss-Jordan inverse)");
    if (h->kind == AFQ_SYS_UEG) AFQ_FAIL(h, AFQ_EUNSUPPORTED, "ITCF: no propagator matrix for the UEG (itcf.py:114-122)");
    if (h->hirsch && restore_weights)
        AFQ_FAIL(h, AFQ_EUNSUPPORTED, "restore_weights with discrete fields: FieldConfig.push records no weight factors (walkers/stack.py:35-49)");
    if (h->ndet > 1) AFQ_FAIL(h, AFQ_EUNSUPPORTED, "ITCF: multi-determinant trials");
    const int n = nmax + neqlb;
    if (h->nbp && h->nbp != n)
        AFQ_FAIL(h, AFQ_ESTATE, "ITCF: a field history of " + std::to_string(h->nbp) + " steps is configured, the window needs " +
                                    std::to_string(n));
    if (!h->nbp && (rc = afq_bp_configure(h, n))) return rc;
    h->it_nmax = nmax; h->it_neqlb = neqlb; h->it_stable = stable ? 1 : 0; h->it_restore = restore_weights ? 1 : 0;
    return AFQ_OK;
}

int afq_itcf_update(afq_handle *h, const double *psi_T, int nstblz, double *spgf_out, double *denom_out) {
    AFQ_API(h, "afq_itcf_update");
    GreensCache::ReadOnly read_only(h ? &h->gf : nullptr);
    if (!h || !psi_T || !spgf_out || !denom_out || nstblz < 1) return AFQ_EINVAL;
    int rc = need_ready(h, true);
    if (rc) return rc;
    if (!h->it_nmax) AFQ_FAIL(h, AFQ_ESTATE, "ITCF is not configured: afq_itcf_configure first");
    if (h->nbp != h->it_nmax + h->it_neqlb) AFQ_FAIL(h, AFQ_ESTATE, "ITCF: the field history changed length");
    const int M = h->M, nw = h->nw, nmax = h->it_nmax;
    const size_t per = (size_t)M * h->nt, mm = (size_t)M * M, g2 = 2 * mm * nw, nspgf = (size_t)(nmax + 1) * 4 * mm;
    const bool stable = h->it_stable != 0;
    const int nkeep = stable ? nmax : 1;
    const bool gen = !h->hirsch;
    {
        size_t fr = 0, tot = 0;
        AFQ_HIP(h, hipMemGetInfo(&fr, &tot));
        const double need = 16.0 * (double)nw * nkeep * per;
        const double avail = (double)fr + 16.0 * (double)h->it_ws_len;
        if (need > 0.5 * avail)
            AFQ_FAIL(h, AFQ_ENOMEM, "ITCF: the stored psi_L take " + std::to_string((unsigned long long)need) +
                                        " bytes, more than half of the free device memory (" +
                                        std::to_string((unsigned long long)avail) + " bytes)");
    }
    cplx *base;
    if ((rc = itcf_scratch(h, itcf_carve(h, nullptr, nkeep).len, &base))) return rc;
    const ItcfWs w = itcf_carve(h, base, nkeep);
    cplx *psiR = w.psiR, *psiR2 = w.psiR2, *Ggr = w.Ggr, *Gls = w.Gls, *T = w.T;
    AFQ_HIP(h, hipMemcpyAsync(w.BT2inv, h->BH1, sizeof(cplx) * 2 * mm, hipMemcpyDeviceToDevice, h->stream));
    if ((rc = k_gj_inverse(h, w.BT2inv, M, 2, w.detm, w.dete))) return rc;
    if ((rc = window_begin(h, psi_T))) return rc;
    if ((rc = bp_backward(h, 1, nstblz, nullptr, h->bp_ot, h->bp_detR, nullptr, w.psiL, nkeep))) return rc;
    AFQ_HIP(h, hipMemsetAsync(w.est, 0, sizeof(cplx) * (1 + nspgf), h->stream));
    if ((rc = k_itcf_weights(h, h->it_restore, w.wfac, w.est))) return rc;
    AFQ_HIP(h, hipMemcpyAsync(psiR, h->phi_old, sizeof(cplx) * nw * per, hipMemcpyDeviceToDevice, h->stream));
    for (int tau = 0; tau < nmax; ++tau) {
        if (stable || tau == 0) {
            if ((rc = itcf_greens(h, w, psiR, w.psiL + (size_t)tau * nw * per))) return rc;
        }
        if (tau == 0) {
            AFQ_HIP(h, hipMemcpyAsync(Ggr, w.Q, sizeof(cplx) * g2, hipMemcpyDeviceToDevice, h->stream));
            AFQ_HIP(h, hipMemcpyAsync(Gls, w.P, sizeof(cplx) * g2, hipMemcpyDeviceToDevice, h->stream));
            if ((rc = k_itcf_accumulate(h, Ggr, Gls, w.wfac, w.est + 1))) return rc;
        }
        if (gen) {
            {
                Lent<cplx *> l_xs(h->xs, w.xs);
                if ((rc = k_itcf_fields(h, w.xs, tau))) return rc;
                if ((rc = build_vhs(h))) return rc;
            }
            if ((rc = k_itcf_generic_b(h, h->vhs, h->BH1, w.BT2inv, w.B, w.Binv, w.ws, w.detm, w.dete))) return rc;
        } else {
            if ((rc = k_itcf_hirsch_b(h, tau, h->BH1, w.BT2inv, w.B, w.Binv, w.f))) return rc;
        }
        if (stable) {
            if ((rc = k_itcf_mul(h, w.Q, Ggr, T)) || (rc = k_itcf_mul(h, w.B, T, Ggr))) return rc;
            if ((rc = k_itcf_mul(h, Gls, w.P, T)) || (rc = k_itcf_mul(h, T, w.Binv, Gls))) return rc;
// ... 55 lines not shown
```

pauxy_amd/csrc/k_comm.hip:

```cpp
#include <dlfcn.h>
#include <rccl/rccl.h>

#include <algorithm>
#include <cstring>
#include <vector>

#include "block_scan.h"
#include "walker_fields.h"

namespace {

constexpr int MAX_RANKS = 16;
constexpr double WAIT_SECONDS_DEFAULT = 300.0;
__device__ unsigned long long g_wait_ticks = (unsigned long long)(WAIT_SECONDS_DEFAULT * 1e8);

struct RcclApi {
    void *lib = nullptr;
    decltype(&ncclGetUniqueId) GetUniqueId = nullptr;
    decltype(&ncclCommInitRank) CommInitRank = nullptr;
    decltype(&ncclCommDestroy) CommDestroy = nullptr;
    decltype(&ncclAllGather) AllGather = nullptr;
    decltype(&ncclAllReduce) AllReduce = nullptr;
    decltype(&ncclSend) Send = nullptr;
    decltype(&ncclRecv) Recv = nullptr;
// ... 470 lines not shown
    if (c->win_collectives)
        AFQ_LAUNCH(h, comm_prep_kernel, dim3(c->nranks), dim3(256), 0, h->stream, h->weight, h->nw, r, c->sendw, 1, c->pw, c->wl,
                   c->rank, c->seq_g);
    else
        AFQ_LAUNCH(h, comm_prep_kernel, dim3((h->nw + 1 + 255) / 256), dim3(256), 0, h->stream, h->weight, h->nw, r, c->sendw, 0,
                   c->pw, c->wl, c->rank, c->seq_g);
    AFQ_POST(h);
    return AFQ_OK;
}

void fill_pack(afq_handle *h, PackArgs &p, bool with_greens, bool send) {
    afq_comm_state *c = cs_of(h);
    p.f = walker_fields(h, with_greens ? WF_GREENS : 0);
    p.cap = c->cap; p.nranks = c->nranks; p.rank = c->rank;
    p.count = c->lists + (send ? 0 : c->nranks);
    p.idx = c->lists + 2 * c->nranks + (send ? 0 : c->nranks * c->cap);
    p.slot = (long)c->slot;
    p.window = c->window ? 1 : 0; p.pw = c->pw; p.wl = c->wl; p.seq = c->seq_x; p.tickets = c->tickets;
    p.scal = h->scal;
    p.buf = c->window ? (send ? nullptr : c->wl.rbuf(c->win)) : (send ? c->sbuf : c->rbuf);
    p.closed_bad = h->closed_bad; p.closed_epoch = h->closed_epoch; p.closed_half = 0;
}

int stage_plan_pack(afq_handle *h, double target, bool with_greens, bool fused_prep = false, double r = 0.0, bool pack_now = true) {
    afq_comm_state *c = cs_of(h);
    const long N = (long)c->nranks * h->nw;
    const size_t lds = (sizeof(double) + 3 * sizeof(int)) * (size_t)N;
    if (lds > 160 * 1024 - 256) AFQ_FAIL(h, AFQ_EUNSUPPORTED, "device comb: more than 8000 walkers in total");
    static size_t lds_set[AFQ_MAX_DEVICES] = {0};
    AFQ_HIP(h, afq_raise_lds((const void *)comb_plan_global_kernel, lds, lds_set));
    PlanArgs a;
    a.gw = c->win_collectives ? c->wl.gw(c->win, (int)(c->seq_g & 1)) : c->gw;
    a.gflag = c->win_collectives ? c->wl.flag_g(c->win) : nullptr; a.seq = c->seq_g;
    a.R = c->nranks; a.nw = h->nw; a.rank = c->rank; a.cap = c->cap; a.target = target;
    a.weight = h->weight; a.unscaled = h->unscaled; a.pix_global = c->pix; a.parent_ix = h->parent_ix;
    a.pairs = (int *)h->pack_tmp; a.lists = c->lists; a.scal = h->scal;
    a.prep_R = fused_prep ? c->nranks : 0; a.prep_r = r; a.pw = c->pw; a.wl = c->wl;
    AFQ_LAUNCH(h, comb_plan_global_kernel, dim3(1 + a.prep_R), dim3(256), lds, h->stream, a);
    AFQ_POST(h);
    int rc = k_clone_pairs(h, with_greens, true);
    if (rc) return rc;
    if (c->nranks > 1 && pack_now) {
        PackArgs p;
        fill_pack(h, p, with_greens, true);
        AFQ_LAUNCH(h, comm_pack_kernel<true>, dim3(4, std::min(c->cap, COMM_GRID_Y), c->nranks), dim3(256), 0, h->stream, p);
        AFQ_POST(h);
    }
    return AFQ_OK;
}

int stage_unpack(afq_handle *h, bool with_greens, bool pack_too = false) {
    const bool closed_too = with_greens && h->closed_bad && h->gf.closed.current(h->gf) && h->na == h->nb;
    h->gf.cloned(closed_too ? GreensCache::CLOSED : 0);
    afq_comm_state *c = cs_of(h);
    if (c->nranks > 1) {
        PackArgs p;
        fill_pack(h, p, with_greens, false);
        if (closed_too) p.closed_half = (long)h->na * h->M;
        if (pack_too) {
            PackArgs ps;
            fill_pack(h, ps, with_greens, true);
            AFQ_LAUNCH(h, comm_exchange_kernel, dim3(4, std::min(c->cap, COMM_GRID_Y), 2 * c->nranks), dim3(256), 0, h->stream, ps, p);
        } else {
            AFQ_LAUNCH(h, comm_pack_kernel<false>, dim3(4, std::min(c->cap, COMM_GRID_Y), c->nranks), dim3(256), 0, h->stream, p);
        }
        AFQ_POST(h);
    }
    c->events += 1;
    return AFQ_OK;
}

int check_group(afq_handle **hs, int n, std::string *err) {
    if (!hs || n < 1) return AFQ_EINVAL;
    for (int i = 0; i < n; ++i) {
        afq_comm_state *c = hs[i] ? cs_of(hs[i]) : nullptr;
        if (!c || c->mode != COMM_LOCAL || c->nranks != n || c->rank != i || c->peers.size() != (size_t)n || c->peers[0] != hs[0]) {
            if (err) *err = "the handles are not the ranks 0..n-1 of one afq_comm_init_local communicator";
            return AFQ_ESTATE;
        }
        if (hs[i]->nw != hs[0]->nw || !hs[i]->nw) { if (err) *err = "every rank needs the same number of walkers"; return AFQ_ESTATE; }
    }
    return AFQ_OK;
}

int ensure_group(afq_handle **hs, int n) {
    bool fresh = false;
    for (int i = 0; i < n; ++i) {
        afq_comm_state *c = cs_of(hs[i]);
        hipSetDevice(hs[i]->device);
        const bool had = c->lists && c->nw == hs[i]->nw && c->nbp == hs[i]->nbp && c->slot == (size_t)max_slot(hs[i]);
        const int rc = ensure_buffers(hs[i]);
        if (rc) return rc;
        fresh = fresh || !had;
    }
    if (!fresh) return AFQ_OK;
    for (int i = 0; i < n; ++i) {
        afq_comm_state *c = cs_of(hs[i]);
        hipSetDevice(hs[i]->device);
        for (int j = 0; j < n; ++j) {
            if (cs_of(hs[j])->cap != c->cap || cs_of(hs[j])->slot != c->slot) AFQ_FAIL(hs[i], AFQ_ESTATE, "ranks disagree on the slot layout");
            c->pw.base[j] = cs_of(hs[j])->win;
            if (hs[j]->device != hs[i]->device) {
                const hipError_t e = hipDeviceEnablePeerAccess(hs[j]->device, 0);
                if (e != hipSuccess && e != hipErrorPeerAccessAlreadyEnabled) AFQ_HIP(hs[i], e);
                (void)hipGetLastError();
            }
// ... 299 lines not shown
    c->window = window != 0;
    return AFQ_OK;
}

int afq_comm_set_capacity(afq_handle *h, int max_walkers_per_peer) {
    if (!h || max_walkers_per_peer < 1) return AFQ_EINVAL;
    afq_comm_state *c = cs_of(h);
    if (!c) AFQ_FAIL(h, AFQ_ESTATE, "no communicator");
    if (c->cap == max_walkers_per_peer) return AFQ_OK;
    hipSetDevice(h->device);
    AFQ_HIP(h, hipStreamSynchronize(h->stream));
    free_buffers(c);
    c->cap = max_walkers_per_peer;
    return AFQ_OK;
}

int afq_comm_stats(afq_handle *h, int64_t *out) {
    if (!h || !out) return AFQ_EINVAL;
    afq_comm_state *c = cs_of(h);
    if (!c) AFQ_FAIL(h, AFQ_ESTATE, "no communicator");
    hipSetDevice(h->device);
    double sc[AFQ_NSCAL];
    if (h->scal_cache_valid) {
        memcpy(sc, h->scal_cache, sizeof(sc));
    } else {
        AFQ_HIP(h, hipMemcpyAsync(sc, h->scal, sizeof(sc), hipMemcpyDeviceToHost, h->stream));
        AFQ_HIP(h, hipStreamSynchronize(h->stream));
    }
    out[0] = (int64_t)sc[4];
    out[1] = (int64_t)sc[5];
    out[2] = c->cap > 0 ? c->cap : default_cap(h->nw);
    out[3] = (int64_t)sc[3];
    out[4] = c->rank; out[5] = c->nranks;
    out[6] = c->window ? (int64_t)sc[7] : -1;
    out[7] = c->window ? (int64_t)sc[8] : (int64_t)c->sendrecv_bytes;
    out[8] = c->window ? 1 : 0;
    out[9] = (int64_t)sc[6];
    out[10] = (int64_t)c->mode;
    out[11] = c->win ? c->win_kind : 0;
    return AFQ_OK;
}

int afq_popcontrol_comb_local(afq_handle **hs, int n, double r, double target, int32_t *parent_ix, double *total_out) {
    std::string err;
    int rc = check_group(hs, n, &err);
    if (rc) { if (hs && n > 0 && hs[0]) hs[0]->err = err; return rc; }
    const int nw = hs[0]->nw;
    std::vector<char> keep(n);
    for (int i = 0; i < n; ++i) {
        afq_handle *h = hs[i];
        hipSetDevice(h->device);
        h->scal_cache_valid = false;
        keep[i] = h->gf.take() == GreensCache::FULL && h->ndet == 1;
    }
    bool with_greens = true;
    for (int i = 0; i < n; ++i) with_greens = with_greens && keep[i];
    if ((rc = ensure_group(hs, n))) return rc;
    for (int i = 0; i < n; ++i) {
        hipSetDevice(hs[i]->device);
        if ((rc = stage_prep(hs[i], i == 0 ? r : 0.0))) return rc;
        AFQ_HIP(hs[i], hipEventRecord(cs_of(hs[i])->ev, hs[i]->stream));
    }
    for (int i = 0; i < n; ++i) {
        afq_handle *h = hs[i];
        hipSetDevice(h->device);
        for (int j = 0; j < n; ++j) if (j != i) AFQ_HIP(h, hipStreamWaitEvent(h->stream, cs_of(hs[j])->ev, 0));
        if ((rc = stage_plan_pack(h, target, with_greens))) return rc;
        AFQ_HIP(h, hipEventRecord(cs_of(h)->ev2, h->stream));
    }
    for (int i = 0; i < n; ++i) {
        afq_handle *h = hs[i];
        hipSetDevice(h->device);
        for (int j = 0; j < n; ++j) if (j != i) AFQ_HIP(h, hipStreamWaitEvent(h->stream, cs_of(hs[j])->ev2, 0));
        if ((rc = stage_unpack(h, with_greens))) return rc;
        h->gf.keep(with_greens ? GreensCache::FULL : GreensCache::NOTHING);
    }
    if (!parent_ix && !total_out) return AFQ_OK;
    afq_handle *h0 = hs[0];
    hipSetDevice(h0->device);
    double sc[8];
    AFQ_HIP(h0, hipMemcpyAsync(sc, h0->scal, sizeof(sc), hipMemcpyDeviceToHost, h0->stream));
    if (parent_ix)
        AFQ_HIP(h0, hipMemcpyAsync(parent_ix, cs_of(h0)->pix, sizeof(int) * (size_t)n * nw, hipMemcpyDeviceToHost, h0->stream));
    for (int i = 0; i < n; ++i) { hipSetDevice(hs[i]->device); AFQ_HIP(hs[i], hipStreamSynchronize(hs[i]->stream)); }
    if (total_out) *total_out = sc[0];
    if (sc[1] < 0) AFQ_FAIL(h0, AFQ_EWEIGHT, "total walker weight below 1e-8");
    if (sc[3] != 0.0) AFQ_FAIL(h0, AFQ_EOVERFLOW, "more walkers moved between two ranks than the exchange slots hold");
    if (sc[6] != 0.0) AFQ_FAIL(h0, AFQ_ECOMM, "communicator: a rank never signalled (the wait budget of afq_comm_set_timeout ran out on the device)");
    return AFQ_OK;
}

int afq_comm_parent_ix(afq_handle *h, int32_t *parent_ix_global) {
    if (!h || !parent_ix_global) return AFQ_EINVAL;
    afq_comm_state *c = cs_of(h);
    if (!c || !c->pix) AFQ_FAIL(h, AFQ_ESTATE, "no population control on a communicator yet");
    hipSetDevice(h->device);
    AFQ_HIP(h, hipMemcpyAsync(parent_ix_global, c->pix, sizeof(int) * (size_t)c->nranks * h->nw, hipMemcpyDeviceToHost, h->stream));
    AFQ_HIP(h, hipStreamSynchronize(h->stream));
    return AFQ_OK;
}

int afq_estimates_allreduce(afq_handle *h, double *buf, int nest) {
    if (!h || (buf && nest < 1)) return AFQ_EINVAL;
    afq_comm_state *c = cs_of(h);
    if (!c) AFQ_FAIL(h, AFQ_ESTATE, "no communicator");
    if (c->mode == COMM_LOCAL) AFQ_FAIL(h, AFQ_ESTATE, "in-process communicator: use afq_estimates_allreduce_local");
// ... 163 lines not shown
```

pauxy_amd/csrc/k_fused.hip:

```cpp
#include <cstdlib>
#include <type_traits>

#include "mfma_gemm_wg.h"
#include "greens_small.h"

#define PF_D 3
#ifndef PF_NW
#define PF_NW 8
#endif
#define PF_NT (64 * PF_NW)
#ifndef PF_LW
#define PF_LW PF_NW
#endif
#define PF_FPW (16 / PF_LW)

struct PropFusedArgs {
    int M, na, nb, nt, order;
    int vhs_upper;
    int same_b;
    int b_real;
    int rem4;
    int hyb;
    int symcols;
    int closed_try;
// ... 1 lines not shown
    const cplx *BH1;
    const cplx *vhs;
    cplx *phi;
    const int *alive;
    const void *zero16;
    unsigned long long *n_closed;
    int resident;
};

__device__ inline d2_t lds_read_c(unsigned addr) { return lds_read_b128(addr); }

template <int OFF> __device__ inline d2_t lds_read_off(unsigned addr) {
    d2_t v;
    asm volatile("ds_read_b128 %0, %1 offset:%2" : "=v"(v) : "v"(addr), "n"(OFF));
    return v;
}
__device__ __attribute__((always_inline)) inline d2_t lds_read_frag(unsigned base, int idx) {
    switch (idx) {
    case 0: return lds_read_off<0>(base);
    case 1: return lds_read_off<1024>(base);
    case 2: return lds_read_off<2048>(base);
    case 3: return lds_read_off<3072>(base);
    case 4: return lds_read_off<4096>(base);
    case 5: return lds_read_off<5120>(base);
    case 6: return lds_read_off<6144>(base);
    default: return lds_read_off<7168>(base);
    }
}

template <int OFF> __device__ inline double lds_read_re_off(unsigned addr) {
    double v;
    asm volatile("ds_read_b64 %0, %1 offset:%2" : "=v"(v) : "v"(addr), "n"(OFF));
    return v;
}
__device__ __attribute__((always_inline)) inline double lds_read_frag_re(unsigned base, int idx) {
    switch (idx) {
    case 0: return lds_read_re_off<0>(base);
    case 1: return lds_read_re_off<1024>(base);
    case 2: return lds_read_re_off<2048>(base);
    case 3: return lds_read_re_off<3072>(base);
    case 4: return lds_read_re_off<4096>(base);
    case 5: return lds_read_re_off<5120>(base);
    case 6: return lds_read_re_off<6144>(base);
    default: return lds_read_re_off<7168>(base);
    }
}

__device__ inline void lds_barrier() {
    asm volatile("s_waitcnt lgkmcnt(0)" ::: "memory");
    __builtin_amdgcn_s_barrier();
    asm volatile("" ::: "memory");
}

#include "k_fused_closed.h"

template <bool NARROW, int FULL>
__global__ __launch_bounds__(PF_NT) void prop_fused_kernel(PropFusedArgs a) {
    extern __shared__ __align__(16) unsigned char smem[];
    constexpr bool MUL3 = false;
#define PF_LEAVE(stored_closed_) return
#define PF_RESIDENT(KS_) prop_closed_resident<KS_, MUL3>(a, smem, phi, vhs)
#include "k_fused_body.h"
#undef PF_RESIDENT
#undef PF_LEAVE
}

template <bool NARROW, int FULL, bool TAIL, bool MUL3>
__global__ __launch_bounds__(PF_NT) void prop_fused_kernel(PropFusedArgs a, GreensArgs ga, WeightArgs wa, const double *psiB) {
    static_assert(TAIL && !NARROW && FULL == 7, "the tail rides on the full wide deal only");
    extern __shared__ __align__(16) unsigned char smem[];
    bool stored_closed = false;
    EarlyTail early;
    early.on = false;
    do {
#define PF_LEAVE(stored_closed_) { stored_closed = (stored_closed_); break; }
#define PF_RESIDENT(KS_)                                                                                      \
    do {                                                                                                      \
        if constexpr (MUL3) {                                                                                 \
            if (psiB) prop_closed_resident<KS_, true, true>(a, smem, phi, vhs, psiB, &early);                 \
            else prop_closed_resident<KS_, true>(a, smem, phi, vhs);                                          \
        } else prop_closed_resident<KS_, false>(a, smem, phi, vhs);                                           \
    } while (0)
#include "k_fused_body.h"
#undef PF_RESIDENT
#undef PF_LEAVE
    } while (0);
    asm volatile("s_waitcnt vmcnt(0) lgkmcnt(0)" ::: "memory");
    __syncthreads();
    int w = blockIdx.x;
    asm volatile("" : "+s"(w));
    if constexpr (MUL3) greens_small_body<true, true, true>(ga, wa, w, smem, stored_closed, &early);
    else greens_small_body<true, true>(ga, wa, w, smem, stored_closed);
}

int k_prop_fused_supported(afq_handle *h) {
    return !h->vhs_diag && h->nv == 1 && h->M <= 104 && h->na <= 32 && h->nb <= 32 && h->nb > 0;
}

int k_prop_closed_resident(afq_handle *h) {
    return PF_NW == 8 && k_prop_fused_supported(h) && h->prop_closed_mode != 1 && h->bh1_same && h->bh1_real &&
           h->na == h->nb && h->na > 16 && h->na <= 32 && h->M > 96 && h->M <= 104 && h->exp_order > 0;
}

int k_step_fusion_shape(afq_handle *h) {
    if (!k_prop_closed_resident(h)) return 0;
    const size_t nmax = h->na, NCH = (h->M + 7) / 8;
    const size_t tail = sizeof(cplx) * (2 * (nmax * nmax + 2 * nmax) + ((2 * nmax + 3) / 4 + 1) + (size_t)h->M * h->nt);
    return tail <= NCH * 8192 + (size_t)PF_D * 16384;
}

int k_prop_fused(afq_handle *h, const GreensLaunch *tail, bool mul3) {
    PropFusedArgs a;
    a.M = h->M; a.na = h->na; a.nb = h->nb; a.nt = h->nt; a.order = h->exp_order;
    a.vhs_upper = h->vhs_upper ? 1 : 0;
    a.same_b = h->bh1_same ? 1 : 0;
    a.b_real = h->bh1_real ? 1 : 0;
    a.rem4 = (h->M > 96 && h->M <= 100) ? 1 : 0;
    a.hyb = 0;
    a.contig = 0; a.symcols = 0;
    if (a.rem4 && a.same_b && h->na > 16 && h->nb > 16 && h->nt > 48 && h->nt <= 56 && PF_NW == 8) {
        a.contig = 1;
        a.hyb = (h->nt - 48 + 3) / 4;
    }
    a.symcols = (a.contig && h->na == h->nb) ? 1 : 0;
    a.closed_try = 0;
    a.BH1 = h->BH1; a.vhs = h->vhs; a.phi = h->phi; a.alive = h->alive; a.zero16 = h->zero_page;
    a.n_closed = h->counters + 3;
    const int NCH = (h->M + 7) / 8;
    const size_t lds = (size_t)NCH * 8192 + (size_t)PF_D * 16384;
    static size_t lds_set[8][AFQ_MAX_DEVICES] = {{0}, {0}, {0}, {0}, {0}, {0}, {0}, {0}};
    const bool narrow = h->na <= 16 && h->nb <= 16;
    const bool early = tail && mul3 && h->step_tail_overlap && h->psiB_cT && k_prop_closed_resident(h) &&
                       tail->a.psi_real && tail->a.psi_closed && tail->a.psi_stride == 0 &&
                       (const void *)tail->a.psi == h->psiB_psi && (const void *)h->BH1 == h->psiB_bh1 &&
                       tail->a.gsum && tail->a.ghalf && !tail->a.oinv;
    KernelTrace kt(h, AFQ_K_PROPAGATOR);
    {
        const int nrt_ = (h->M + 15) / 16, ct = (h->na + 15) / 16 + (h->nb + 15) / 16;
        const double ksteps = 2.0 * NCH;
        const double per_pass = ksteps * (2048.0 * (a.rem4 ? nrt_ - 1 : nrt_) * ct + 512.0 * (a.rem4 ? ct : 0));
        const double taylor_pass = a.contig ? ksteps * (2048.0 * (nrt_ - 1) * 3 + 512.0 * (nrt_ - 1) * a.hyb + 512.0 * 4) : per_pass;
        h->issued_flops[AFQ_K_PROPAGATOR] = (3.0 * h->exp_order * taylor_pass + 2.0 * (a.b_real ? 2.0 : 3.0) * per_pass) * h->nw;
        h->prop_issued_open = h->issued_flops[AFQ_K_PROPAGATOR] / h->nw;
        const int cta = (h->na + 15) / 16;
        const double closed_pass = ksteps * (2048.0 * (a.rem4 ? nrt_ - 1 : nrt_) * cta + 512.0 * (a.rem4 ? cta : 0));
        h->prop_issued_closed = 3.0 * h->exp_order * closed_pass + 2.0 * (a.b_real ? 2.0 : 3.0) * per_pass;
        if (k_prop_closed_resident(h))
            h->prop_issued_closed = ((tail && mul3 ? 3.0 : 4.0) * h->exp_order + 2.0 * 2.0) * ((h->M + 3) / 4) * 2048.0 * 7 * 2;
        if (tail) {
            const double t16 = (h->na + 15) / 16, m16 = (h->M + 15) / 16;
            const double ks1 = 4.0 * (((h->M + 3) / 4 + 3) / 4), ks3 = (h->na + 3) / 4;
            const double spin = 2048.0 * (t16 * t16 * ks1 * (tail->a.psi_real ? 2.0 : 3.0) + t16 * m16 * ks3 * 3.0);
            h->prop_issued_open += 2.0 * spin;
            h->prop_issued_closed += (tail->a.psi_closed ? 1.0 : 2.0) * spin;
            if (early) h->prop_issued_closed += 2048.0 * (4.0 * ((h->M + 3) / 4) * 2.0 - t16 * t16 * ks1 * 2.0);
            h->issued_flops[AFQ_K_PROPAGATOR] = h->prop_issued_open * h->nw;
        }
    }
    const int nrt = (h->M + 15) / 16;
    const bool nofull = PF_NW != 8;
    const int full = nofull ? 0 : narrow ? (nrt == 6 ? 6 : 0) : (nrt >= 5 && h->na > 16 && h->nb > 16 ? nrt : 0);
    a.closed_try = (a.same_b && h->na == h->nb && h->exp_order > 0 && full != 0 && PF_NW == 8 &&
                    (!a.contig || a.symcols)) ? 1 : 0;
    a.resident = (a.closed_try && full == 7 && k_prop_closed_resident(h)) ? 1 : 0;
#define PF_LAUNCH_(NARROW_, FULL_, SLOT_)                                                                     \
    do {                                                                                                      \
        AFQ_HIP(h, afq_raise_lds((const void *)prop_fused_kernel<NARROW_, FULL_>, lds, lds_set[SLOT_]));      \
        AFQ_LAUNCH(h, (prop_fused_kernel<NARROW_, FULL_>), dim3(h->nw), dim3(PF_NT), lds, h->stream, a);      \
    } while (0)
    if (tail) {
        if (full != 7 || !a.resident || tail->lds > lds)
            AFQ_FAIL(h, AFQ_ESTATE, "internal: a Green's function tail on a propagator launch outside its shape class");
        if (mul3) {
            AFQ_HIP(h, afq_raise_lds((const void *)prop_fused_kernel<false, 7, true, true>, lds, lds_set[6]));
            const double *psiB = early ? h->psiB_cT : nullptr;
            AFQ_LAUNCH(h, (prop_fused_kernel<false, 7, true, true>), dim3(h->nw), dim3(PF_NT), lds, h->stream, a, tail->a, tail->wa, psiB);
        } else {
            const double *psiB = nullptr;
            AFQ_HIP(h, afq_raise_lds((const void *)prop_fused_kernel<false, 7, true, false>, lds, lds_set[7]));
            AFQ_LAUNCH(h, (prop_fused_kernel<false, 7, true, false>), dim3(h->nw), dim3(PF_NT), lds, h->stream, a, tail->a, tail->wa, psiB);
        }
    }
    else if (narrow && full) PF_LAUNCH_(true, 6, 0);
    else if (narrow) PF_LAUNCH_(true, 0, 1);
    else if (full == 7) PF_LAUNCH_(false, 7, 2);
    else if (full == 6) PF_LAUNCH_(false, 6, 3);
    else if (full == 5) PF_LAUNCH_(false, 5, 4);
    else PF_LAUNCH_(false, 0, 5);
#undef PF_LAUNCH_
    AFQ_POST(h);
    return AFQ_OK;
}
```

pauxy_amd/csrc/k_fused_body.h:

```cpp
    const int w = blockIdx.x;
    if (!a.alive[w]) PF_LEAVE(false);
    const int tid = threadIdx.x, lane = tid & 63, wave = __builtin_amdgcn_readfirstlane(tid >> 6);
    const int lr = lane & 15, lk = lane >> 4;
    const int M = a.M, nt = a.nt;
    const int NCH = (M + 7) >> 3;
    const int nrt = (M + 15) >> 4;
    unsigned char *Tf = smem;
    unsigned char *ring = smem + (size_t)NCH * 8192;
    const unsigned tf_l = lds_addr(Tf), ring_l = lds_addr(ring);
    cplx *phi = a.phi + (long)w * M * nt;
    const cplx *vhs = a.vhs + (long)w * M * M;

    const int nob = a.same_b ? 1 : 2;
    const int nphase = 2 * nob + a.order;
    const int G = nphase * NCH;
    const long MM = (long)M * M;
    int gi = 0, gi_phase = 0, gi_c = 0, gi_slot = 0;
    const void *nsrc[PF_FPW];
    bool prepared = false;
    const bool refills = wave >= PF_NW - PF_LW;
    const int lw = wave - (PF_NW - PF_LW);
    const int p_row0 = (lw >> 1) * 16 + lr;
    const int p_kl = 2 * lk + (lw & 1);
    auto prepare = [&]() __attribute__((always_inline)) {
        if (!refills) { prepared = true; return; }
        const bool in_v = gi_phase >= nob && gi_phase < nob + a.order;
        const int spin = gi_phase < nob ? gi_phase : gi_phase - nob - a.order;
        const cplx *A = in_v ? vhs : a.BH1 + (spin == 1 ? MM : 0L);
        const bool sym_phase = a.vhs_upper && in_v;
        const bool live = gi < G;
        const int k = gi_c * 8 + p_kl;
#pragma unroll
        for (int t = 0; t < PF_FPW; ++t) {
            const int row = p_row0 + t * (PF_LW / 2) * 16;
            const int off = (sym_phase && k < row) ? k * M + row : row * M + k;
            nsrc[t] = (live && row < M && k < M) ? (const void *)(A + off) : a.zero16;
            asm volatile("" : "+v"(nsrc[t]));
        }
        ++gi;
        const bool wrap = gi_c + 1 == NCH;
        gi_c = wrap ? 0 : gi_c + 1;
        gi_phase += wrap ? 1 : 0;
        prepared = true;
    };
    auto issueA = [&]() __attribute__((always_inline)) {
        if (!refills) return;
        if (!prepared) prepare();
        unsigned char *dst = ring + (size_t)gi_slot * 16384;
#pragma unroll
        for (int t = 0; t < PF_FPW; ++t) glds16(nsrc[t], dst + (lw + t * PF_LW) * 1024);
        if (++gi_slot == PF_D) gi_slot = 0;
        prepared = false;
    };
    issueA(); issueA();
    prepare();
    bool closed = false;
    if (a.closed_try) {
        bool same = true;
        for (int p = tid >> 5; p < M; p += PF_NT / 32) {
            const int c = tid & 31;
            if (c < a.na) {
                const cplx x = phi[p * nt + c], y = phi[p * nt + a.na + c];
                same = same && __double_as_longlong(x.x) == __double_as_longlong(y.x) &&
                       __double_as_longlong(x.y) == __double_as_longlong(y.y);
            }
        }
        closed = __builtin_amdgcn_readfirstlane(__syncthreads_and(same ? 1 : 0)) != 0;
        if (closed && tid == 0) atomicAdd(a.n_closed, 1ULL);
    }
    if constexpr (!NARROW && FULL == 7 && PF_NW == 8) {
        if (closed && a.resident) {
            if (M <= 100) PF_RESIDENT(25);
            else PF_RESIDENT(26);
            PF_LEAVE(true);
        }
    }
    const bool relayout = closed && a.contig;
    const int contig = relayout ? 0 : a.contig, hyb = relayout ? 0 : a.hyb;
    const int sym_n = (a.symcols && !relayout) ? a.na : 0;
    auto wcol = [&](const int c) -> int {
        if (!sym_n) return c;
        if (c < 16) return c;
        if (c < 32) return sym_n + (c - 16);
        if (c < 40) return 16 + (c - 32);
        if (c < 48) return sym_n + 16 + (c - 40);
        const int e = c - 48, extra = sym_n - 24;
        return e < extra ? 24 + e : sym_n + 24 + (e - extra);
    };

    for (int e = tid; e < NCH * 512; e += PF_NT) {
        const int j = e & 15, kk = (e >> 4) & 3, pb = (e >> 6) & 1, slot = (e >> 7) & 3, ch = e >> 9;
        const int p = ch * 8 + 2 * kk + pb, sp = contig ? 0 : slot >> 1, col = (contig ? slot : slot & 1) * 16 + j;
        const int ns_ = contig ? nt : sp ? a.nb : a.na, off_ = sp ? a.na : 0;
        const bool ok = p < M && col < ns_;
        const cplx v = phi[ok ? p * nt + off_ + wcol(col) : 0];
        ((d2_t *)Tf)[e] = ok ? (d2_t){v.x, v.y} : (d2_t){0.0, 0.0};
    }
    __syncthreads();

    auto t_ok = [&](int ti, int r) -> bool { return 2 * ti + (r >> 1) < NCH; };
    const unsigned t_lane = (unsigned)((lk & 1) * 1024 + ((lk >> 1) * 16 + lr) * 16);
    auto t_addr = [&](int ti, int r, int cs) -> unsigned {
        unsigned base = t_lane;
        asm volatile("" : "+v"(base));
        return base + (unsigned)(((2 * ti * 4 + cs) * 2) * 1024) + (unsigned)((r >> 1) * 8192 + (r & 1) * 512);
    };

    int ring_slot = 0;
    auto next_chunk = [&]() __attribute__((always_inline)) -> unsigned {
        asm volatile("s_waitcnt vmcnt(%0)" ::"n"((PF_D - 2) * PF_FPW) : "memory");
// ... 776 lines not shown
```

pauxy_amd/csrc/k_fused_closed.h:

```cpp
#pragma once

#define PCR_LDS(p) ((__attribute__((address_space(3))) unsigned char *)(p))

template <int KS, bool MUL3, bool EARLY = false>
__device__ __attribute__((always_inline)) inline void prop_closed_resident(const PropFusedArgs &a, unsigned char *smem_,
                                                                           cplx *phi, const cplx *vhs,
                                                                           const double *psiB = nullptr, EarlyTail *et = nullptr) {
    auto *smem = PCR_LDS(smem_);
    typedef __attribute__((address_space(3))) d2_t lds_d2;
    typedef __attribute__((address_space(3))) double lds_f64;
    const int tid = threadIdx.x, wave = __builtin_amdgcn_readfirstlane(tid >> 6);
    const int M = a.M, nt = a.nt, na = a.na;
    constexpr unsigned TB = KS * 2048;
    const bool mul = wave < 7;
    auto lane_id = [&]() __attribute__((always_inline)) -> int {
        int t = tid;
        asm volatile("" : "+v"(t));
        return t & 63;
    };

    const unsigned base0 = (EARLY && (a.order & 1)) ? TB : 0u;
    for (int e = tid; e < KS * 128; e += PF_NT) {
        const int k = 4 * (e >> 7) + ((e >> 4) & 3), col = 16 * ((e >> 6) & 1) + (e & 15);
        const bool ok = k < M && col < na;
        const cplx v = phi[ok ? k * nt + col : 0];
        ((lds_d2 *)(smem + base0))[e] = ok ? (d2_t){v.x, v.y} : (d2_t){0.0, 0.0};
    }
    __syncthreads();

    auto load_b = [&](double (&bh)[KS]) __attribute__((always_inline)) {
        const int lane = lane_id(), lk = lane >> 4, row = wave * 16 + (lane & 15);
#pragma unroll
        for (int s = 0; s < KS; ++s) {
            const int k = 4 * s + lk;
            const double *p = (row < M && k < M) ? &a.BH1[row * M + k].x : (const double *)a.zero16;
            bh[s] = *p;
        }
    };
    auto one_body = [&](const unsigned src, const double (&bh)[KS], d4_t (&P1)[2], d4_t (&P2)[2]) __attribute__((always_inline)) {
#pragma unroll
        for (int j = 0; j < 2; ++j) { P1[j] = (d4_t){0, 0, 0, 0}; P2[j] = (d4_t){0, 0, 0, 0}; }
        const auto *tb = smem + src + lane_id() * 16;
#pragma unroll
        for (int s = 0; s < KS; ++s) {
#pragma unroll
            for (int j = 0; j < 2; ++j) {
                const d2_t b = *(const lds_d2 *)(tb + (s * 2 + j) * 1024);
                P1[j] = mfma16(bh[s], b[0], P1[j]);
                P2[j] = mfma16(bh[s], b[1], P2[j]);
            }
        }
    };
    auto put = [&](const unsigned dst, const d4_t (&re)[2], const d4_t (&im)[2]) __attribute__((always_inline)) {
        auto *tb = smem + dst + lane_id() * 16;
#pragma unroll
        for (int q = 0; q < 4; ++q)
            if (4 * wave + q < KS) {
#pragma unroll
                for (int j = 0; j < 2; ++j) *(lds_d2 *)(tb + ((4 * wave + q) * 2 + j) * 1024) = (d2_t){re[j][q], im[j][q]};
            }
    };

    d2_t av[KS];
    d4_t SR[2], SI[2];
    if (mul) {
        double bh[KS];
        load_b(bh);
        const int lane = lane_id(), lk = lane >> 4, row = wave * 16 + (lane & 15);
#pragma unroll
        for (int s = 0; s < KS; ++s) {
            const int k = 4 * s + lk;
            const int off = (a.vhs_upper && k < row) ? k * M + row : row * M + k;
            const d2_t *p = (row < M && k < M) ? (const d2_t *)(vhs + off) : (const d2_t *)a.zero16;
            av[s] = *p;
        }
        one_body(base0, bh, SR, SI);
        put(base0 ^ TB, SR, SI);
    }
    constexpr unsigned PB = 2 * TB;
    if constexpr (EARLY) {
        if (!mul) {
            const int lane = lane_id(), lk = lane >> 4, lr = lane & 15;
            double pv[2][KS];
#pragma unroll
            for (int t = 0; t < 2; ++t)
#pragma unroll
                for (int s = 0; s < KS; ++s) {
                    const int j = 16 * t + lr, k = 4 * s + lk;
                    const double *p = (j < na && k < M) ? psiB + j * M + k : (const double *)a.zero16;
                    pv[t][s] = *p;
                }
            auto *pb = smem + PB + lane * 8;
#pragma unroll
            for (int t = 0; t < 2; ++t)
#pragma unroll
                for (int s = 0; s < KS; ++s) *(lds_f64 *)(pb + (t * KS + s) * 512) = pv[t][s];
        }
    }
    lds_barrier();

    unsigned cur = base0 ^ TB;
    for (int n = 1; n <= a.order; ++n) {
        if (mul) {
            double inv_n = 1.0 / n;
            asm volatile("" : "+v"(inv_n));
            d4_t P1[2], P2[2], P3[2];
#pragma unroll
            for (int j = 0; j < 2; ++j) { P1[j] = (d4_t){0, 0, 0, 0}; P2[j] = (d4_t){0, 0, 0, 0}; P3[j] = (d4_t){0, 0, 0, 0}; }
            const auto *tb = smem + cur + lane_id() * 16;
#pragma unroll
            for (int s = 0; s < KS; ++s) {
                asm volatile("" : "+v"(av[s]));
#pragma unroll
                for (int j = 0; j < 2; ++j) {
                    const d2_t b = *(const lds_d2 *)(tb + (s * 2 + j) * 1024);
                    if constexpr (MUL3) {
                        P1[j] = mfma16(av[s][0], b[0], P1[j]);
                        P2[j] = mfma16(av[s][1], b[1], P2[j]);
                        P3[j] = mfma16(av[s][0] + av[s][1], b[0] + b[1], P3[j]);
                    } else {
                        P3[j] = mfma16(av[s][0], b[1], P3[j]);
                        P1[j] = mfma16(av[s][0], b[0], P1[j]);
                        P2[j] = mfma16(av[s][1], b[1], P2[j]);
                        P3[j] = mfma16(av[s][1], b[0], P3[j]);
                    }
                }
            }
            d4_t re[2], im[2];
#pragma unroll
            for (int j = 0; j < 2; ++j)
#pragma unroll
                for (int q = 0; q < 4; ++q) {
                    re[j][q] = (P1[j][q] - P2[j][q]) * inv_n;
                    im[j][q] = (MUL3 ? P3[j][q] - P1[j][q] - P2[j][q] : P3[j][q]) * inv_n;
                    SR[j][q] += re[j][q]; SI[j][q] += im[j][q];
                }
            if (n == a.order) put(cur ^ TB, SR, SI);
            else put(cur ^ TB, re, im);
        }
        lds_barrier();
        cur ^= TB;
    }

    if constexpr (EARLY) {
        const int nn = na, nsq = nn * nn + 2 * nn;
        cplx *O = (cplx *)smem_;
        cplx *phi_l = (cplx *)smem_ + 2L * nsq + ((2 * nn + 3) / 4 + 1);
        {
            const int t = wave >> 2, j = (wave >> 1) & 1, part = wave & 1;
            const auto *pa = smem + PB + t * (KS * 512) + lane_id() * 8;
            const auto *tb = smem + cur + j * 1024 + part * 8 + lane_id() * 16;
            d4_t acc0 = {0, 0, 0, 0}, acc1 = {0, 0, 0, 0};
#pragma unroll
            for (int s = 0; s < KS; ++s) {
                const double x = *(const lds_f64 *)(pa + s * 512), y = *(const lds_f64 *)(tb + s * 2048);
                if (s & 1) acc1 = mfma16(x, y, acc1);
                else acc0 = mfma16(x, y, acc0);
            }
            const int lane = lane_id(), lr = lane & 15, lk = lane >> 4;
#pragma unroll
            for (int q = 0; q < 4; ++q) {
                const int i = 16 * j + lr, jj = 16 * t + 4 * q + lk;
                if (i < nn && jj < nn) ((double *)&O[i * nn + jj])[part] = acc0[q] + acc1[q];
            }
        }
        lds_barrier();
        d4_t P1[2], P2[2];
        if (mul) {
            double bh[KS];
            load_b(bh);
            one_body(cur, bh, P1, P2);
            const int lane = lane_id(), lr = lane & 15, lk = lane >> 4;
#pragma unroll
            for (int j = 0; j < 2; ++j)
#pragma unroll
                for (int q = 0; q < 4; ++q) {
                    const int orow = wave * 16 + lk + 4 * q, col = 16 * j + lr;
                    if (orow < M && col < na) {
                        const cplx v = cmake(P1[j][q], P2[j][q]);
                        phi[(long)orow * nt + col] = v;
                        phi[(long)orow * nt + na + col] = v;
                    }
                }
        } else {
            cplx *scr = O + nsq;
            gj_wave32(O, nn, lane_id(), true, scr, scr + 32, (int *)(scr + 64), et->ph, et->la);
        }
        lds_barrier();
        if (mul) {
            const int lane = lane_id(), lr = lane & 15, lk = lane >> 4;
#pragma unroll
            for (int j = 0; j < 2; ++j)
#pragma unroll
                for (int q = 0; q < 4; ++q) {
                    const int orow = wave * 16 + lk + 4 * q, col = 16 * j + lr;
                    if (orow < M && col < na) {
                        const cplx v = cmake(P1[j][q], P2[j][q]);
                        phi_l[orow * nt + col] = v;
                        phi_l[orow * nt + na + col] = v;
                    }
                }
        }
        et->on = true;
        return;
    }
    if (mul) {
        d4_t P1[2], P2[2];
        double bh[KS];
        load_b(bh);
        one_body(cur, bh, P1, P2);
        const int lane = lane_id(), lr = lane & 15, lk = lane >> 4;
#pragma unroll
        for (int j = 0; j < 2; ++j)
#pragma unroll
            for (int q = 0; q < 4; ++q) {
                const int orow = wave * 16 + lk + 4 * q, col = 16 * j + lr;
                if (orow < M && col < na) {
                    const cplx v = cmake(P1[j][q], P2[j][q]);
                    phi[(long)orow * nt + col] = v;
                    phi[(long)orow * nt + na + col] = v;
                }
            }
    }
}
```

pauxy_amd/device.py:

```python
import ctypes

import numpy

from pauxy_amd import _lib as L


def _c128(a, shape=None):
    a = numpy.ascontiguousarray(a, dtype=numpy.complex128)
    if shape is not None:
        assert a.shape == tuple(shape), (a.shape, shape)
    return a


def _f64(a, shape=None):
    a = numpy.ascontiguousarray(a, dtype=numpy.float64)
    if shape is not None:
        assert a.shape == tuple(shape), (a.shape, shape)
    return a


def _i64(a):
    return numpy.ascontiguousarray(a, dtype=numpy.int64)


# ... 641 lines not shown
        out = numpy.zeros(max_n, dtype=numpy.float64)
        n = ctypes.c_int()
        self._ck(self.lib.afq_kernel_trace_get(self.h, int(kind), _p(out), max_n, ctypes.byref(n)))
        return out[:min(n.value, max_n)]

    def launch_trace(self, on=True):
        self._ck(self.lib.afq_launch_trace(self.h, int(bool(on))))

    def launch_trace_get(self):
        cap = 256
        names = ctypes.create_string_buffer(cap * 96)
        ms = numpy.zeros(cap, dtype=numpy.float64)
        cnt = numpy.zeros(cap, dtype=numpy.int64)
        n = ctypes.c_int()
        self._ck(self.lib.afq_launch_trace_get(self.h, ctypes.cast(names, ctypes.c_void_p), len(names), _p(ms), _p(cnt),
                                               cap, ctypes.byref(n)))
        out, at = {}, 0
        for k in range(min(n.value, cap)):
            end = names.raw.index(b'\0', at)
            out[names.raw[at:end].decode()] = (int(cnt[k]), float(ms[k]))
            at = end + 1
        return out

    def kernel_issued_flops(self, kind):
        out = ctypes.c_double(0.0)
        self._ck(self.lib.afq_kernel_issued_flops(self.h, int(kind), ctypes.byref(out)))
        return float(out.value)

    def propagator_issued_flops(self):
        a, b = ctypes.c_double(0.0), ctypes.c_double(0.0)
        self._ck(self.lib.afq_propagator_issued_flops(self.h, ctypes.byref(a), ctypes.byref(b)))
        return float(a.value), float(b.value)

    def set_exchange_algorithm(self, mode):
        self._ck(self.lib.afq_set_exchange_algorithm(self.h, int(mode)))

    def exchange_algorithm(self):
        m = ctypes.c_int()
        self._ck(self.lib.afq_exchange_algorithm(self.h, ctypes.byref(m)))
        return m.value

    def set_propagator_closed_form(self, mode):
        self._ck(self.lib.afq_set_propagator_closed_form(self.h, int(mode)))

    def set_step_fusion(self, mode):
        self._ck(self.lib.afq_set_step_fusion(self.h, int(mode)))

    def set_step_fusion_scope(self, scope):
        self._ck(self.lib.afq_set_step_fusion_scope(self.h, int(scope)))

    def set_step_tail_overlap(self, on):
        self._ck(self.lib.afq_set_step_tail_overlap(self.h, int(on)))

    def propagator_closed_form(self):
        m = ctypes.c_int()
        self._ck(self.lib.afq_propagator_closed_form(self.h, ctypes.byref(m)))
        return m.value

    def set_msd_force_bias(self, mode):
        self._ck(self.lib.afq_set_msd_force_bias(self.h, int(mode)))

    def msd_force_bias(self):
        m = ctypes.c_int()
        self._ck(self.lib.afq_msd_force_bias(self.h, ctypes.byref(m)))
        return m.value


def _handle_array(devs):
    return (ctypes.c_void_p * len(devs))(*[d.h.value for d in devs])


def comm_init_local(devs):
    lib = devs[0].lib
    rc = lib.afq_comm_init_local(_handle_array(devs), len(devs))
    if rc != 0:
        raise L.AfqError(rc, lib.afq_last_error(devs[0].h).decode())
    for i, d in enumerate(devs):
        d.comm_rank, d.comm_size = i, len(devs)


def popcontrol_comb_local(devs, r, target, fetch=True):
    lib = devs[0].lib
    n = len(devs)
    if not fetch:
        rc = lib.afq_popcontrol_comb_local(_handle_array(devs), n, float(r), float(target), None, None)
        pix = tw = None
    else:
        pix = numpy.zeros(n * devs[0].nw, dtype=numpy.int32)
        tw = ctypes.c_double(0.0)
        rc = lib.afq_popcontrol_comb_local(_handle_array(devs), n, float(r), float(target), _p(pix), ctypes.byref(tw))
        tw = tw.value
    if rc != 0:
        raise L.AfqError(rc, lib.afq_last_error(devs[0].h).decode())
    return pix, tw


def estimates_allreduce_local(devs):
    lib = devs[0].lib
    rc = lib.afq_estimates_allreduce_local(_handle_array(devs), len(devs))
    if rc != 0:
        raise L.AfqError(rc, lib.afq_last_error(devs[0].h).decode())
```

Before: 1.186 million walker-steps/s.

## Hand over next step's first one-body product from the fused propagate kernel

```diff
diff --git a/include/afqmc_hip.h b/include/afqmc_hip.h
--- a/include/afqmc_hip.h
+++ b/include/afqmc_hip.h
@@ -142,6 +142,7 @@
 int afq_set_step_fusion(afq_handle *h, int mode);
 int afq_set_step_fusion_scope(afq_handle *h, int scope);
 int afq_set_step_tail_overlap(afq_handle *h, int on);
+int afq_set_step_handover(afq_handle *h, int on);
 
 int afq_set_msd_force_bias(afq_handle *h, int mode);
 int afq_msd_force_bias(afq_handle *h, int *mode_out);
diff --git a/pauxy_amd/_lib.py b/pauxy_amd/_lib.py
--- a/pauxy_amd/_lib.py
+++ b/pauxy_amd/_lib.py
@@ -137,6 +137,7 @@
     "afq_set_step_fusion": [_h, c_int],
     "afq_set_step_fusion_scope": [_h, c_int],
     "afq_set_step_tail_overlap": [_h, c_int],
+    "afq_set_step_handover": [_h, c_int],
     "afq_set_msd_force_bias": [_h, c_int],
     "afq_msd_force_bias": [_h, POINTER(c_int)],
     "afq_kernel_trace": [_h, c_int],
diff --git a/pauxy_amd/csrc/afq_api.hip b/pauxy_amd/csrc/afq_api.hip
--- a/pauxy_amd/csrc/afq_api.hip
+++ b/pauxy_amd/csrc/afq_api.hip
@@ -105,8 +105,12 @@
     const int M = h->M, nt = h->nt, na = h->na;
     const bool ok = h->have_prop && h->ndet <= 1 && h->psi_stride == 0 && h->psi_real && h->psi_closed &&
                     h->bh1_real && h->bh1_same && c->psi.size() == (size_t)2 * M * nt && c->BH1.size() == (size_t)M * M;
-    h->psiB_psi = nullptr; h->psiB_bh1 = nullptr;
-    if (!ok) return dev_alloc(h, LT_TRIAL, &h->psiB_cT, 0);
+    h->psiB_psi = nullptr; h->psiB_bh1 = nullptr; h->b2_bh1 = nullptr;
+    h->handover.drop();
+    if (!ok) {
+        const int rc0 = dev_alloc(h, LT_TRIAL, &h->B2, 0);
+        return rc0 ? rc0 : dev_alloc(h, LT_TRIAL, &h->psiB_cT, 0);
+    }
     std::vector<double> pb((size_t)na * M, 0.0);
     for (int m = 0; m < M; ++m)
         for (int i = 0; i < na; ++i) {
@@ -115,8 +119,22 @@
             double *out = &pb[(size_t)i * M];
             for (int k = 0; k < M; ++k) out[k] += p * brow[k];
         }
-    const int rc = dev_upload(h, LT_TRIAL, &h->psiB_cT, pb.data(), pb.size());
+    int rc = dev_upload(h, LT_TRIAL, &h->psiB_cT, pb.data(), pb.size());
     if (!rc) { h->psiB_psi = h->dets[h->cur_det].psi; h->psiB_bh1 = h->BH1; }
+    if (rc) return rc;
+    std::vector<double> b2((size_t)M * M);
+    std::vector<long double> acc(M);
+    for (int m = 0; m < M; ++m) {
+        std::fill(acc.begin(), acc.end(), 0.0L);
+        for (int j = 0; j < M; ++j) {
+            const long double x = c->BH1[(size_t)m * M + j];
+            const double *brow = &c->BH1[(size_t)j * M];
+            for (int k = 0; k < M; ++k) acc[k] += x * (long double)brow[k];
+        }
+        for (int k = 0; k < M; ++k) b2[(size_t)m * M + k] = (double)acc[k];
+    }
+    rc = dev_upload(h, LT_TRIAL, &h->B2, b2.data(), b2.size());
+    if (!rc) h->b2_bh1 = h->BH1;
     return rc;
 }
 
@@ -265,7 +283,7 @@
 
 int afq_set_system_generic(afq_handle *h, int M, int K, int na, int nb, const double *hs_pot,
                            const double *rchol, const double *H1, double ecore) {
-    if (h) h->gf.drop();
+    if (h) { h->gf.drop(); h->handover.drop(); }
     if (!h || !hs_pot || !rchol || !H1) return AFQ_EINVAL;
     int rc = set_dims(h, AFQ_SYS_GENERIC, M, K, na, nb);
     if (rc) return rc;
@@ -310,7 +328,7 @@
 
 int afq_set_system_generic_c128(afq_handle *h, int M, int K, int na, int nb, const double *hs_pot,
                                 const double *rchol, const double *H1, double ecore) {
-    if (h) h->gf.drop();
+    if (h) { h->gf.drop(); h->handover.drop(); }
     if (!h || !hs_pot || !rchol || !H1) return AFQ_EINVAL;
     if (M <= 0 || K <= 0) AFQ_FAIL(h, AFQ_EINVAL, "bad dimensions");
     const size_t mm = (size_t)M * M, nq = (size_t)(na + nb) * M;
@@ -371,7 +389,7 @@
 }
 
 int afq_set_system_hubbard(afq_handle *h, int M, int na, int nb, double U, const double *T) {
-    if (h) h->gf.drop();
+    if (h) { h->gf.drop(); h->handover.drop(); }
     if (!h || !T) return AFQ_EINVAL;
     int rc = set_dims(h, AFQ_SYS_HUBBARD, M, M, na, nb);
     if (rc) return rc;
@@ -407,7 +425,7 @@
                        const int64_t *kpq_i, const int64_t *kpq_kpq, const int64_t *pmq_off,
                        const int64_t *pmq_i, const int64_t *pmq_pmq, const double *vqvec, double vol,
                        const double *H1diag, double ecore) {
-    if (h) h->gf.drop();
+    if (h) { h->gf.drop(); h->handover.drop(); }
     if (!h || !iA_colptr || !iB_colptr || !kpq_off || !pmq_off || !vqvec || !H1diag) return AFQ_EINVAL;
     int rc = set_dims(h, AFQ_SYS_UEG, M, 2 * nq, na, nb);
     if (rc) return rc;
@@ -488,7 +506,7 @@
 }
 
 int afq_set_trial(afq_handle *h, const double *psi) {
-    if (h) h->gf.drop();
+    if (h) { h->gf.drop(); h->handover.drop(); }
     if (!h || !psi) return AFQ_EINVAL;
     if (!h->kind) AFQ_FAIL(h, AFQ_ESTATE, "set the system before the trial");
     if (h->ndet > 1) AFQ_FAIL(h, AFQ_ESTATE, "a multi-determinant trial is set; set the system again first");
@@ -501,7 +519,7 @@
 }
 
 int afq_set_trial_multi(afq_handle *h, int ndet, const double *psi, const double *coeffs, const double *rchol) {
-    if (h) h->gf.drop();
+    if (h) { h->gf.drop(); h->handover.drop(); }
     if (!h || !psi || !coeffs || !rchol || ndet < 1) return AFQ_EINVAL;
     if (h->kind != AFQ_SYS_GENERIC) AFQ_FAIL(h, AFQ_EUNSUPPORTED, "multi-determinant trials need a generic system");
     if (h->nw) AFQ_FAIL(h, AFQ_ESTATE, "set the trial before allocating walkers");
@@ -543,7 +561,7 @@
 
 int afq_set_propagator(afq_handle *h, const double *BH1, const double *mf_shift, double dt, int exp_order,
                        int flags) {
-    if (h) h->gf.drop();
+    if (h) { h->gf.drop(); h->handover.drop(); }
     if (!h || !BH1 || !mf_shift || dt <= 0 || exp_order < 0) return AFQ_EINVAL;
     if (!h->kind) AFQ_FAIL(h, AFQ_ESTATE, "set the system before the propagator");
     hipSetDevice(h->device);
@@ -575,7 +593,7 @@
 }
 
 int afq_walkers_alloc(afq_handle *h, int nw) {
-    if (h) h->gf.drop();
+    if (h) { h->gf.drop(); h->handover.drop(); }
     if (!h || nw <= 0) return AFQ_EINVAL;
     if (!h->kind) AFQ_FAIL(h, AFQ_ESTATE, "set the system before allocating walkers");
     hipSetDevice(h->device);
@@ -679,6 +697,7 @@
 
 int afq_walkers_set(afq_handle *h, int field, const void *host, int first, int count) {
     if (h && (field == AFQ_F_PHI || field == AFQ_F_GHALF)) { h->gf.drop(); h->gf.rewritten(); }
+    if (h && field == AFQ_F_PHI) h->handover.drop();
     if (!h || !host) return AFQ_EINVAL;
     if (!h->nw) AFQ_FAIL(h, AFQ_ESTATE, "no walkers allocated");
     if (first < 0 || count < 0 || first + count > h->nw) AFQ_FAIL(h, AFQ_EINVAL, "walker range out of bounds");
@@ -717,6 +736,7 @@
         if ((rc = ensure_spin_ghalf(h))) return rc;
     }
     h->gf.drop(); h->gf.enabled = false;
+    if (field == AFQ_F_PHI) { h->handover.drop(); h->handover.enabled = false; }
     *dev_ptr = base;
     if (bytes_per_walker) *bytes_per_walker = (int64_t)bytes;
     return AFQ_OK;
@@ -876,6 +896,7 @@
             else if ((rc = local_energy(h))) return rc;
         }
     }
+    if (k_ueg_fast_supported(h) || hubbard_fused || !k_prop_fused_supported(h)) h->handover.drop();
     if (k_ueg_fast_supported(h)) {
         { PhaseTimer t(h, T_EXP); if ((rc = k_ueg_step(h))) return rc; }
         h->prop_pending = true;
@@ -1015,6 +1036,7 @@
 int afq_reortho(afq_handle *h, double *detR_out) {
     AFQ_API(h, "afq_reortho");
     if (!h) return AFQ_EINVAL;
+    h->handover.drop();
     int rc = need_ready(h, false);
     if (rc) { h->gf.drop(); return rc; }
     const GreensCache::Kept kept = h->gf.take();
@@ -1074,24 +1096,35 @@
 int afq_set_propagator_closed_form(afq_handle *h, int mode) {
     if (!h || mode < 0 || mode > 2) return AFQ_EINVAL;
     h->prop_closed_mode = mode;
+    h->handover.drop();
     return AFQ_OK;
 }
 
 int afq_set_step_fusion(afq_handle *h, int mode) {
     if (!h || mode < 0 || mode > 2) return AFQ_EINVAL;
     h->step_fusion_mode = mode;
+    h->handover.drop();
     return AFQ_OK;
 }
 
 int afq_set_step_fusion_scope(afq_handle *h, int scope) {
     if (!h || scope < 0 || scope > 1) return AFQ_EINVAL;
     h->step_fusion_scope = scope;
+    h->handover.drop();
     return AFQ_OK;
 }
 
 int afq_set_step_tail_overlap(afq_handle *h, int on) {
     if (!h || on < 0 || on > 1) return AFQ_EINVAL;
     h->step_tail_overlap = on;
+    h->handover.drop();
+    return AFQ_OK;
+}
+
+int afq_set_step_handover(afq_handle *h, int on) {
+    if (!h || on < 0 || on > 1) return AFQ_EINVAL;
+    h->step_handover = on;
+    h->handover.drop();
     return AFQ_OK;
 }
 
@@ -1170,7 +1203,7 @@
 }
 
 int afq_apply_exponential(afq_handle *h, const double *vhs) {
-    if (h) h->gf.drop();
+    if (h) { h->gf.drop(); h->handover.drop(); }
     if (!h || !vhs) return AFQ_EINVAL;
     int rc = need_ready(h, true);
     if (rc) return rc;
@@ -1192,7 +1225,7 @@
 }
 
 int afq_kinetic(afq_handle *h) {
-    if (h) h->gf.drop();
+    if (h) { h->gf.drop(); h->handover.drop(); }
     if (!h) return AFQ_EINVAL;
     int rc = need_ready(h, true);
     if (rc) return rc;
@@ -1221,6 +1254,7 @@
     if (h) h->scal_cache_valid = false;
     AFQ_API(h, "afq_popcontrol_comb");
     if (!h) return AFQ_EINVAL;
+    h->handover.drop();
     const bool thermal = h->th_on && h->nw;
     int rc = AFQ_OK;
     if (thermal) {
@@ -1250,6 +1284,7 @@
     if (h) h->scal_cache_valid = false;
     AFQ_API(h, "afq_popcontrol_pair_branch");
     if (!h) return AFQ_EINVAL;
+    h->handover.drop();
     if (h->th_on) AFQ_FAIL(h, AFQ_EUNSUPPORTED, "thermal walkers: pair_branch population control is not supported (comb only)");
     int rc = need_ready(h, false);
     if (rc) { h->gf.drop(); return rc; }
@@ -1319,7 +1354,7 @@
 }
 
 int afq_walker_unpack(afq_handle *h, int iw, const void *dev_buf) {
-    if (h) h->gf.drop();
+    if (h) { h->gf.drop(); h->handover.drop(); }
     if (!h || !dev_buf) return AFQ_EINVAL;
     int rc = need_ready(h, false);
     if (rc) return rc;
@@ -1328,7 +1363,7 @@
 }
 
 int afq_walkers_copy(afq_handle *h, int src, int dst) {
-    if (h) h->gf.drop();
+    if (h) { h->gf.drop(); h->handover.drop(); }
     if (!h) return AFQ_EINVAL;
     int rc = need_ready(h, false);
     if (rc) return rc;
@@ -1632,7 +1667,7 @@
 }
 
 int afq_set_propagator_hirsch(afq_handle *h, const double *bt2, double dt, int charge_decomposition) {
-    if (h) h->gf.drop();
+    if (h) { h->gf.drop(); h->handover.drop(); }
     if (!h || !bt2 || dt <= 0) return AFQ_EINVAL;
     if (h->kind != AFQ_SYS_HUBBARD) AFQ_FAIL(h, AFQ_ESTATE, "the Hirsch transformation needs a Hubbard system");
     if (h->ndet > 1) AFQ_FAIL(h, AFQ_EUNSUPPORTED, "Hirsch propagator: single-determinant trials");
@@ -1681,7 +1716,7 @@
 }
 
 int afq_hirsch_kinetic(afq_handle *h) {
-    if (h) h->gf.drop();
+    if (h) { h->gf.drop(); h->handover.drop(); }
     if (!h) return AFQ_EINVAL;
     int rc = hirsch_ready(h);
     if (rc) return rc;
@@ -1690,7 +1725,7 @@
 }
 
 int afq_hirsch_two_body(afq_handle *h, const double *u, int32_t *fields_out, int32_t *used_out) {
-    if (h) h->gf.drop();
+    if (h) { h->gf.drop(); h->handover.drop(); }
     if (!h || !u) return AFQ_EINVAL;
     int rc = hirsch_ready(h);
     if (rc) return rc;
@@ -1703,7 +1738,7 @@
 }
 
 int afq_hirsch_finish(afq_handle *h, double eshift) {
-    if (h) h->gf.drop();
+    if (h) { h->gf.drop(); h->handover.drop(); }
     if (!h) return AFQ_EINVAL;
     int rc = hirsch_ready(h);
     if (rc) return rc;
@@ -1715,7 +1750,7 @@
 
 int afq_propagate_hirsch(afq_handle *h, double eshift) {
     AFQ_API(h, "afq_propagate_hirsch");
-    if (h) h->gf.drop();
+    if (h) { h->gf.drop(); h->handover.drop(); }
     if (!h) return AFQ_EINVAL;
     int rc = hirsch_ready(h);
     if (rc) return rc;
@@ -1748,7 +1783,7 @@
 
 int afq_propagate_hirsch_free(afq_handle *h, const double *u, int32_t *fields_out, double eshift) {
     AFQ_API(h, "afq_propagate_hirsch_free");
-    if (h) h->gf.drop();
+    if (h) { h->gf.drop(); h->handover.drop(); }
     if (!h) return AFQ_EINVAL;
     int rc = hirsch_ready(h);
     if (rc) return rc;
diff --git a/pauxy_amd/csrc/afq_internal.h b/pauxy_amd/csrc/afq_internal.h
--- a/pauxy_amd/csrc/afq_internal.h
+++ b/pauxy_amd/csrc/afq_internal.h
@@ -37,7 +37,14 @@
 enum { AFQ_HS_HERMITIAN = 1, AFQ_HS_GENERAL = 2 };
 enum { T_GREENS = 0, T_ONEBODY, T_FB, T_VHS, T_EXP, T_OVLP, T_QR, T_ENERGY, T_COUNT };
 
-#define AFQ_NCOUNTERS 9
+#define AFQ_NCOUNTERS 10
+
+struct StepHandover {
+    bool current = false;
+    bool enabled = true;
+    void drop() { current = false; }
+    void produced() { current = enabled; }
+};
 
 struct afq_handle {
     int device = 0;
@@ -70,6 +77,7 @@
     int step_fusion_mode = 2;
     int step_fusion_scope = 0;
     int step_tail_overlap = 1;
+    int step_handover = 1;
     int prop_closed_mode = 0;
     cplx *exq_y = nullptr;
     size_t exq_y_len = 0;
@@ -109,6 +117,8 @@
     bool psi_closed = false;
     double *psiB_cT = nullptr;
     const void *psiB_psi = nullptr, *psiB_bh1 = nullptr;
+    double *B2 = nullptr;
+    const void *b2_bh1 = nullptr;
     unsigned long long *closed_bad = nullptr;
     unsigned long long closed_epoch = 0;
     unsigned long long closed_epoch_pub = 0;
@@ -249,6 +259,9 @@
     cplx *gdiag = nullptr;
     int gdiag_parts = 0;
     GreensCache gf;
+    unsigned char *t0_next = nullptr;
+    int *t0_ready = nullptr;
+    StepHandover handover;
     cplx *xbar = nullptr, *xs = nullptr;
     cplx *cmf = nullptr, *cfb = nullptr;
     cplx *vhs = nullptr;
diff --git a/pauxy_amd/csrc/afq_windows.hip b/pauxy_amd/csrc/afq_windows.hip
--- a/pauxy_amd/csrc/afq_windows.hip
+++ b/pauxy_amd/csrc/afq_windows.hip
@@ -149,7 +149,7 @@
 
 int bp_update(afq_handle *h, const double *phi_bp0, int nstblz, int restore_weights, int eval_energy,
               int reset, double *est_out, double *two_rdm_out, double *fock_out) {
-    if (h) h->gf.drop();
+    if (h) { h->gf.drop(); h->handover.drop(); }
     if (!h || !phi_bp0 || !est_out || nstblz < 1 || restore_weights < 0 || restore_weights > 2) return AFQ_EINVAL;
     int rc = need_ready(h, true);
     if (rc) return rc;
@@ -292,6 +292,7 @@
                       int eval_energy, int reset, double *est_out, double *detw_out) {
     AFQ_API(h, "afq_bp_update_msd");
     GreensCache::ReadOnly read_only(h ? &h->gf : nullptr);
+    if (h) h->handover.drop();
     if (!h || !dets || !coeffs || !est_out || ndet < 1 || nstblz < 1 || restore_weights < 0 || restore_weights > 2)
         return AFQ_EINVAL;
     int rc = need_ready(h, true);
@@ -445,6 +446,7 @@
 int afq_itcf_update(afq_handle *h, const double *psi_T, int nstblz, double *spgf_out, double *denom_out) {
     AFQ_API(h, "afq_itcf_update");
     GreensCache::ReadOnly read_only(h ? &h->gf : nullptr);
+    if (h) h->handover.drop();
     if (!h || !psi_T || !spgf_out || !denom_out || nstblz < 1) return AFQ_EINVAL;
     int rc = need_ready(h, true);
     if (rc) return rc;
diff --git a/pauxy_amd/csrc/k_comm.hip b/pauxy_amd/csrc/k_comm.hip
--- a/pauxy_amd/csrc/k_comm.hip
+++ b/pauxy_amd/csrc/k_comm.hip
@@ -546,6 +546,7 @@
 int stage_unpack(afq_handle *h, bool with_greens, bool pack_too = false) {
     const bool closed_too = with_greens && h->closed_bad && h->gf.closed.current(h->gf) && h->na == h->nb;
     h->gf.cloned(closed_too ? GreensCache::CLOSED : 0);
+    h->handover.drop();
     afq_comm_state *c = cs_of(h);
     if (c->nranks > 1) {
         PackArgs p;
@@ -951,6 +952,7 @@
         hipSetDevice(h->device);
         h->scal_cache_valid = false;
         keep[i] = h->gf.take() == GreensCache::FULL && h->ndet == 1;
+        h->handover.drop();
     }
     bool with_greens = true;
     for (int i = 0; i < n; ++i) with_greens = with_greens && keep[i];
diff --git a/pauxy_amd/csrc/k_fused.hip b/pauxy_amd/csrc/k_fused.hip
--- a/pauxy_amd/csrc/k_fused.hip
+++ b/pauxy_amd/csrc/k_fused.hip
@@ -77,6 +77,15 @@
     asm volatile("" ::: "memory");
 }
 
+struct StepHandoverArgs {
+    unsigned char *t0_next;
+    int *ready;
+    const double *B2;
+    unsigned long long *n_handed;
+    int consume;
+    int produce;
+};
+
 #include "k_fused_closed.h"
 
 template <bool NARROW, int FULL>
@@ -84,38 +93,67 @@
     extern __shared__ __align__(16) unsigned char smem[];
     constexpr bool MUL3 = false;
 #define PF_LEAVE(stored_closed_) return
+#define PF_HANDOVER
 #define PF_RESIDENT(KS_) prop_closed_resident<KS_, MUL3>(a, smem, phi, vhs)
 #include "k_fused_body.h"
 #undef PF_RESIDENT
+#undef PF_HANDOVER
 #undef PF_LEAVE
 }
 
 template <bool NARROW, int FULL, bool TAIL, bool MUL3>
 __global__ __launch_bounds__(PF_NT) void prop_fused_kernel(PropFusedArgs a, GreensArgs ga, WeightArgs wa, const double *psiB) {
     static_assert(TAIL && !NARROW && FULL == 7, "the tail rides on the full wide deal only");
+    static_assert(!MUL3, "the 3-multiplication tail kernel takes the step hand-over: the overload below");
+    extern __shared__ __align__(16) unsigned char smem[];
+    bool stored_closed = false;
+    do {
+#define PF_LEAVE(stored_closed_) { stored_closed = (stored_closed_); break; }
+#define PF_HANDOVER
+#define PF_RESIDENT(KS_) prop_closed_resident<KS_, false>(a, smem, phi, vhs)
+#include "k_fused_body.h"
+#undef PF_RESIDENT
+#undef PF_HANDOVER
+#undef PF_LEAVE
+    } while (0);
+    asm volatile("s_waitcnt vmcnt(0) lgkmcnt(0)" ::: "memory");
+    __syncthreads();
+    int w = blockIdx.x;
+    asm volatile("" : "+s"(w));
+    greens_small_body<true, true>(ga, wa, w, smem, stored_closed);
+}
+
+template <bool NARROW, int FULL, bool TAIL, bool MUL3>
+__global__ __launch_bounds__(PF_NT) void prop_fused_kernel(PropFusedArgs a, GreensArgs ga, WeightArgs wa, const double *psiB,
+                                                           StepHandoverArgs ho) {
+    static_assert(TAIL && !NARROW && FULL == 7 && MUL3, "the tail rides on the full wide deal only");
     extern __shared__ __align__(16) unsigned char smem[];
     bool stored_closed = false;
     EarlyTail early;
     early.on = false;
     do {
 #define PF_LEAVE(stored_closed_) { stored_closed = (stored_closed_); break; }
+#define PF_HANDOVER                                                                                           \
+    if (ho.consume) {                                                                                         \
+        handed = __builtin_amdgcn_readfirstlane(ho.ready[w]) != 0;                                            \
+        if (handed && threadIdx.x == 0) { atomicAdd(a.n_closed, 1ULL); atomicAdd(ho.n_handed, 1ULL); }        \
+    }
 #define PF_RESIDENT(KS_)                                                                                      \
     do {                                                                                                      \
-        if constexpr (MUL3) {                                                                                 \
-            if (psiB) prop_closed_resident<KS_, true, true>(a, smem, phi, vhs, psiB, &early);                 \
-            else prop_closed_resident<KS_, true>(a, smem, phi, vhs);                                          \
-        } else prop_closed_resident<KS_, false>(a, smem, phi, vhs);                                           \
+        if (psiB) prop_closed_resident<KS_, true, true>(a, smem, phi, vhs, psiB, &early, &ho, handed);        \
+        else prop_closed_resident<KS_, true>(a, smem, phi, vhs);                                              \
     } while (0)
 #include "k_fused_body.h"
 #undef PF_RESIDENT
+#undef PF_HANDOVER
 #undef PF_LEAVE
     } while (0);
+    if (ho.ready && threadIdx.x == 0) ho.ready[blockIdx.x] = (early.on && ho.produce) ? 1 : 0;
     asm volatile("s_waitcnt vmcnt(0) lgkmcnt(0)" ::: "memory");
     __syncthreads();
     int w = blockIdx.x;
     asm volatile("" : "+s"(w));
-    if constexpr (MUL3) greens_small_body<true, true, true>(ga, wa, w, smem, stored_closed, &early);
-    else greens_small_body<true, true>(ga, wa, w, smem, stored_closed);
+    greens_small_body<true, true, true>(ga, wa, w, smem, stored_closed, &early);
 }
 
 int k_prop_fused_supported(afq_handle *h) {
@@ -159,6 +197,13 @@
                        tail->a.psi_real && tail->a.psi_closed && tail->a.psi_stride == 0 &&
                        (const void *)tail->a.psi == h->psiB_psi && (const void *)h->BH1 == h->psiB_bh1 &&
                        tail->a.gsum && tail->a.ghalf && !tail->a.oinv;
+    const bool consumes = early && h->handover.current && h->handover.enabled && h->t0_next && h->t0_ready;
+    h->handover.drop();
+    const bool produces = early && h->step_handover && h->handover.enabled && h->B2 && (const void *)h->BH1 == h->b2_bh1;
+    if (produces && (!h->t0_next || !h->t0_ready)) {
+        AFQ_TRY(dev_alloc(h, LT_WALKERS, &h->t0_next, (size_t)h->nw * ((h->M + 3) / 4) * 2048, "step hand-over image"));
+        AFQ_TRY(dev_alloc(h, LT_WALKERS, &h->t0_ready, (size_t)h->nw, "step hand-over flags"));
+    }
     KernelTrace kt(h, AFQ_K_PROPAGATOR);
     {
         const int nrt_ = (h->M + 15) / 16, ct = (h->na + 15) / 16 + (h->nb + 15) / 16;
@@ -170,8 +215,10 @@
         const int cta = (h->na + 15) / 16;
         const double closed_pass = ksteps * (2048.0 * (a.rem4 ? nrt_ - 1 : nrt_) * cta + 512.0 * (a.rem4 ? cta : 0));
         h->prop_issued_closed = 3.0 * h->exp_order * closed_pass + 2.0 * (a.b_real ? 2.0 : 3.0) * per_pass;
-        if (k_prop_closed_resident(h))
-            h->prop_issued_closed = ((tail && mul3 ? 3.0 : 4.0) * h->exp_order + 2.0 * 2.0) * ((h->M + 3) / 4) * 2048.0 * 7 * 2;
+        if (k_prop_closed_resident(h)) {
+            const double passes = (consumes ? 0.0 : 1.0) + 1.0 + (produces ? 1.0 : 0.0);
+            h->prop_issued_closed = ((tail && mul3 ? 3.0 : 4.0) * h->exp_order + passes * 2.0) * ((h->M + 3) / 4) * 2048.0 * 7 * 2;
+        }
         if (tail) {
             const double t16 = (h->na + 15) / 16, m16 = (h->M + 15) / 16;
             const double ks1 = 4.0 * (((h->M + 3) / 4 + 3) / 4), ks3 = (h->na + 3) / 4;
@@ -197,12 +244,18 @@
         if (full != 7 || !a.resident || tail->lds > lds)
             AFQ_FAIL(h, AFQ_ESTATE, "internal: a Green's function tail on a propagator launch outside its shape class");
         if (mul3) {
-            AFQ_HIP(h, afq_raise_lds((const void *)prop_fused_kernel<false, 7, true, true>, lds, lds_set[6]));
+            void (*const kern)(PropFusedArgs, GreensArgs, WeightArgs, const double *, StepHandoverArgs) =
+                prop_fused_kernel<false, 7, true, true>;
+            AFQ_HIP(h, afq_raise_lds((const void *)kern, lds, lds_set[6]));
             const double *psiB = early ? h->psiB_cT : nullptr;
-            AFQ_LAUNCH(h, (prop_fused_kernel<false, 7, true, true>), dim3(h->nw), dim3(PF_NT), lds, h->stream, a, tail->a, tail->wa, psiB);
+            StepHandoverArgs ho;
+            ho.t0_next = h->t0_next; ho.ready = h->t0_ready; ho.B2 = h->B2; ho.n_handed = h->counters + 9;
+            ho.consume = consumes ? 1 : 0; ho.produce = produces ? 1 : 0;
+            AFQ_LAUNCH(h, (prop_fused_kernel<false, 7, true, true>), dim3(h->nw), dim3(PF_NT), lds, h->stream, a, tail->a, tail->wa, psiB, ho);
         } else {
             const double *psiB = nullptr;
-            AFQ_HIP(h, afq_raise_lds((const void *)prop_fused_kernel<false, 7, true, false>, lds, lds_set[7]));
+            void (*const kern)(PropFusedArgs, GreensArgs, WeightArgs, const double *) = prop_fused_kernel<false, 7, true, false>;
+            AFQ_HIP(h, afq_raise_lds((const void *)kern, lds, lds_set[7]));
             AFQ_LAUNCH(h, (prop_fused_kernel<false, 7, true, false>), dim3(h->nw), dim3(PF_NT), lds, h->stream, a, tail->a, tail->wa, psiB);
         }
     }
@@ -214,5 +267,6 @@
     else PF_LAUNCH_(false, 0, 5);
 #undef PF_LAUNCH_
     AFQ_POST(h);
+    if (produces) h->handover.produced();
     return AFQ_OK;
 }
diff --git a/pauxy_amd/csrc/k_fused_body.h b/pauxy_amd/csrc/k_fused_body.h
--- a/pauxy_amd/csrc/k_fused_body.h
+++ b/pauxy_amd/csrc/k_fused_body.h
@@ -52,10 +52,14 @@
         if (++gi_slot == PF_D) gi_slot = 0;
         prepared = false;
     };
+    bool handed = false;
+    PF_HANDOVER
+    if (!handed) {
     issueA(); issueA();
     prepare();
-    bool closed = false;
-    if (a.closed_try) {
+    }
+    bool closed = handed;
+    if (!handed && a.closed_try) {
         bool same = true;
         for (int p = tid >> 5; p < M; p += PF_NT / 32) {
             const int c = tid & 31;
diff --git a/pauxy_amd/csrc/k_fused_closed.h b/pauxy_amd/csrc/k_fused_closed.h
--- a/pauxy_amd/csrc/k_fused_closed.h
+++ b/pauxy_amd/csrc/k_fused_closed.h
@@ -5,8 +5,10 @@
 template <int KS, bool MUL3, bool EARLY = false>
 __device__ __attribute__((always_inline)) inline void prop_closed_resident(const PropFusedArgs &a, unsigned char *smem_,
                                                                            cplx *phi, const cplx *vhs,
-                                                                           const double *psiB = nullptr, EarlyTail *et = nullptr) {
+                                                                           const double *psiB = nullptr, EarlyTail *et = nullptr,
+                                                                           const StepHandoverArgs *ho = nullptr, const bool handed_ = false) {
     auto *smem = PCR_LDS(smem_);
+    const bool handed = EARLY && handed_;
     typedef __attribute__((address_space(3))) d2_t lds_d2;
     typedef __attribute__((address_space(3))) double lds_f64;
     const int tid = threadIdx.x, wave = __builtin_amdgcn_readfirstlane(tid >> 6);
@@ -20,13 +22,24 @@
     };
 
     const unsigned base0 = (EARLY && (a.order & 1)) ? TB : 0u;
-    for (int e = tid; e < KS * 128; e += PF_NT) {
-        const int k = 4 * (e >> 7) + ((e >> 4) & 3), col = 16 * ((e >> 6) & 1) + (e & 15);
-        const bool ok = k < M && col < na;
-        const cplx v = phi[ok ? k * nt + col : 0];
-        ((lds_d2 *)(smem + base0))[e] = ok ? (d2_t){v.x, v.y} : (d2_t){0.0, 0.0};
-    }
-    __syncthreads();
+    constexpr int NCP = (KS * 128 + PF_NT - 1) / PF_NT;
+    d2_t cp[NCP];
+    if (handed) {
+        const d2_t *t0 = (const d2_t *)(ho->t0_next + (size_t)blockIdx.x * TB);
+#pragma unroll
+        for (int i = 0; i < NCP; ++i) {
+            const int e = tid + i * PF_NT;
+            cp[i] = t0[e < KS * 128 ? e : 0];
+        }
+    } else {
+        for (int e = tid; e < KS * 128; e += PF_NT) {
+            const int k = 4 * (e >> 7) + ((e >> 4) & 3), col = 16 * ((e >> 6) & 1) + (e & 15);
+            const bool ok = k < M && col < na;
+            const cplx v = phi[ok ? k * nt + col : 0];
+            ((lds_d2 *)(smem + base0))[e] = ok ? (d2_t){v.x, v.y} : (d2_t){0.0, 0.0};
+        }
+        __syncthreads();
+    }
 
     auto load_b = [&](double (&bh)[KS]) __attribute__((always_inline)) {
         const int lane = lane_id(), lk = lane >> 4, row = wave * 16 + (lane & 15);
@@ -65,7 +78,18 @@
     d4_t SR[2], SI[2];
     if (mul) {
         double bh[KS];
-        load_b(bh);
+        if (handed) {
+            const d2_t *t0 = (const d2_t *)(ho->t0_next + (size_t)blockIdx.x * TB) + lane_id();
+#pragma unroll
+            for (int q = 0; q < 4; ++q)
+#pragma unroll
+                for (int j = 0; j < 2; ++j) {
+                    const d2_t v = 4 * wave + q < KS ? t0[((4 * wave + q) * 2 + j) * 64] : (d2_t){0.0, 0.0};
+                    SR[j][q] = v[0]; SI[j][q] = v[1];
+                }
+        } else {
+            load_b(bh);
+        }
         const int lane = lane_id(), lk = lane >> 4, row = wave * 16 + (lane & 15);
 #pragma unroll
         for (int s = 0; s < KS; ++s) {
@@ -74,8 +98,10 @@
             const d2_t *p = (row < M && k < M) ? (const d2_t *)(vhs + off) : (const d2_t *)a.zero16;
             av[s] = *p;
         }
-        one_body(base0, bh, SR, SI);
-        put(base0 ^ TB, SR, SI);
+        if (!handed) {
+            one_body(base0, bh, SR, SI);
+            put(base0 ^ TB, SR, SI);
+        }
     }
     constexpr unsigned PB = 2 * TB;
     if constexpr (EARLY) {
@@ -95,6 +121,13 @@
             for (int t = 0; t < 2; ++t)
 #pragma unroll
                 for (int s = 0; s < KS; ++s) *(lds_f64 *)(pb + (t * KS + s) * 512) = pv[t][s];
+        }
+    }
+    if (handed) {
+#pragma unroll
+        for (int i = 0; i < NCP; ++i) {
+            const int e = tid + i * PF_NT;
+            if (e < KS * 128) ((lds_d2 *)(smem + (base0 ^ TB)))[e] = cp[i];
         }
     }
     lds_barrier();
@@ -182,6 +215,53 @@
                         phi[(long)orow * nt + na + col] = v;
                     }
                 }
+            if (ho->produce && wave != 3) {
+                const bool third = wave == 4 || wave == 5;
+                auto load_b2 = [&](const int rt, double (&bf)[KS]) __attribute__((always_inline)) {
+                    const int ln = lane_id(), hk = ln >> 4, hrow = rt * 16 + (ln & 15);
+#pragma unroll
+                    for (int s = 0; s < KS; ++s) {
+                        const int k = 4 * s + hk;
+                        const double *p = (hrow < M && k < M) ? ho->B2 + hrow * M + k : (const double *)a.zero16;
+                        bf[s] = *p;
+                    }
+                };
+                auto store_t0 = [&](const int rt, const int j, const d4_t &re, const d4_t &im) __attribute__((always_inline)) {
+                    d2_t *t0 = (d2_t *)(ho->t0_next + (size_t)blockIdx.x * TB) + lane_id();
+#pragma unroll
+                    for (int q = 0; q < 4; ++q)
+                        if (4 * rt + q < KS) t0[((4 * rt + q) * 2 + j) * 64] = (d2_t){re[q], im[q]};
+                };
+                d4_t Q1[2], Q2[2];
+                load_b2(wave, bh);
+                if (third) {
+                    double b3[KS];
+                    load_b2(3, b3);
+                    const int j3 = wave - 4;
+                    d4_t X1 = {0, 0, 0, 0}, X2 = {0, 0, 0, 0};
+#pragma unroll
+                    for (int j = 0; j < 2; ++j) { Q1[j] = (d4_t){0, 0, 0, 0}; Q2[j] = (d4_t){0, 0, 0, 0}; }
+                    const auto *tb = smem + cur + lane_id() * 16;
+                    const auto *tx = tb + j3 * 1024;
+#pragma unroll
+                    for (int s = 0; s < KS; ++s) {
+#pragma unroll
+                        for (int j = 0; j < 2; ++j) {
+                            const d2_t b = *(const lds_d2 *)(tb + (s * 2 + j) * 1024);
+                            Q1[j] = mfma16(bh[s], b[0], Q1[j]);
+                            Q2[j] = mfma16(bh[s], b[1], Q2[j]);
+                        }
+                        const d2_t b = *(const lds_d2 *)(tx + s * 2048);
+                        X1 = mfma16(b3[s], b[0], X1);
+                        X2 = mfma16(b3[s], b[1], X2);
+                    }
+                    store_t0(3, j3, X1, X2);
+                } else {
+                    one_body(cur, bh, Q1, Q2);
+                }
+#pragma unroll
+                for (int j = 0; j < 2; ++j) store_t0(wave, j, Q1[j], Q2[j]);
+            }
         } else {
             cplx *scr = O + nsq;
             gj_wave32(O, nn, lane_id(), true, scr, scr + 32, (int *)(scr + 64), et->ph, et->la);
diff --git a/pauxy_amd/device.py b/pauxy_amd/device.py
--- a/pauxy_amd/device.py
+++ b/pauxy_amd/device.py
@@ -717,6 +717,9 @@
     def set_step_tail_overlap(self, on):
         self._ck(self.lib.afq_set_step_tail_overlap(self.h, int(on)))
 
+    def set_step_handover(self, on):
+        self._ck(self.lib.afq_set_step_handover(self.h, int(on)))
+
     def propagator_closed_form(self):
         m = ctypes.c_int()
         self._ck(self.lib.afq_propagator_closed_form(self.h, ctypes.byref(m)))
```

Measured after the change: 1.218 million walker-steps/s (median of 6 runs). 2.7% higher.
